# prip-lab/MSU-LatentAFIS

Measured on AMD Instinct MI355X. Metric: latent queries/sec vs 100k rolled gallery, higher is better.
Workload: dtype f32

## Files before the change

### msu-latentafis_amd/csrc/afis_api.cpp

```cpp
#include "afis_ctx.h"
#include <algorithm>
#include <vector>

using namespace afis;

namespace afis {
thread_local std::string g_create_error;
}

extern "C" {

int afis_create(afis_ctx** out, const float* codewords, int M, int K, int dsub, int device_id)
{
    if (!out || !codewords) return fail(nullptr, AFIS_EINVAL, "afis_create: null argument");
    *out = nullptr;
    if (M != kM || K != kK || dsub != kDsub) return fail(nullptr, AFIS_EINVAL, "afis_create: only the M=16, K=256, dsub=6 codebook geometry is supported");
    int n_dev = 0;
    if (hipGetDeviceCount(&n_dev) != hipSuccess || n_dev <= 0) return fail(nullptr, AFIS_EDEVICE, "afis_create: no HIP device (this library has no CPU fallback)");
    if (device_id < 0 || device_id >= n_dev) return fail(nullptr, AFIS_EINVAL, "afis_create: device_id out of range");
    hipDeviceProp_t prop;
    if (hipGetDeviceProperties(&prop, device_id) != hipSuccess) return fail(nullptr, AFIS_EDEVICE, "afis_create: hipGetDeviceProperties failed");
    if (strncmp(prop.gcnArchName, "gfx950", 6) != 0)
        return fail(nullptr, AFIS_EDEVICE, std::string("afis_create: kernels are built for gfx950 only, device is ") + prop.gcnArchName);
    afis_ctx* c = new afis_ctx();
    c->device = device_id;
    c->n_cus = prop.multiProcessorCount;
#define CRCHK(call) do { hipError_t e_ = (call); if (e_ != hipSuccess) { g_create_error = std::string(#call) + ": " + hipGetErrorString(e_); afis_destroy(c); return AFIS_EDEVICE; } } while (0)
    CRCHK(hipSetDevice(device_id));
    if (const char* cm = getenv("AFIS_CU_MASK")) {
        std::vector<uint32_t> words;
        for (const char* p = cm; *p;) { words.push_back((uint32_t)strtoul(p, nullptr, 16)); const char* q = strchr(p, ','); if (!q) break; p = q + 1; }
        CRCHK(hipExtStreamCreateWithCUMask(&c->stream, (uint32_t)words.size(), words.data()));
    } else
    CRCHK(hipStreamCreateWithFlags(&c->stream, hipStreamNonBlocking));
    std::vector<float> cw(codewords, codewords + (size_t)M * K * dsub);
    CRCHK(upload(c->codewords, cw, c->stream));
    std::vector<float> table((size_t)kDistN * kDistN);
    for (int i = 0; i < kDistN; ++i)
        for (int j = i; j < kDistN; ++j) {
            table[i * kDistN + j] = (float)sqrt((i * 16.0) * (i * 16.0) + (j * 16.0) * (j * 16.0));
            table[j * kDistN + i] = table[i * kDistN + j];
        }
    CRCHK(upload(c->table, table, c->stream));
    CRCHK(hipStreamSynchronize(c->stream));
#undef CRCHK
    *out = c;
    register_context(c);
    {
        if (const char* r = getenv("AFIS_OVERLAP_CELL_RATIO")) c->overlap_cell_ratio = atof(r);
        if (const char* r = getenv("AFIS_SEARCH_TIMEOUT_S")) c->search_timeout_s = atof(r);
        const char* e = getenv("AFIS_BOUND_CUS");
        const int64_t n = e ? atoll(e) : (c->n_cus == 256 ? 128 : 0);
        if (afis_set_option(c, "bound_cus", n) != AFIS_OK) { c->bound_cus = 0; c->err.clear(); }
    }
    return AFIS_OK;
}

int afis_device_info(int device_id, char* name, size_t name_cap, char* pci_bus_id, size_t pci_cap, char* uuid_hex, size_t uuid_cap, int* n_cus)
{
    int n_dev = 0;
    if (hipGetDeviceCount(&n_dev) != hipSuccess || device_id < 0 || device_id >= n_dev) return AFIS_EINVAL;
    hipDeviceProp_t prop;
    if (hipGetDeviceProperties(&prop, device_id) != hipSuccess) return AFIS_EDEVICE;
    if (name && name_cap) snprintf(name, name_cap, "%s (%s)", prop.name, prop.gcnArchName);
    if (pci_bus_id && pci_cap) { if (hipDeviceGetPCIBusId(pci_bus_id, (int)pci_cap, device_id) != hipSuccess) pci_bus_id[0] = 0; }
    if (uuid_hex && uuid_cap) {
        uuid_hex[0] = 0;
        hipUUID u;
        if (uuid_cap >= 33 && hipDeviceGetUuid(&u, device_id) == hipSuccess)
            for (int i = 0; i < 16; ++i) snprintf(uuid_hex + 2 * i, 3, "%02x", (unsigned)(unsigned char)u.bytes[i]);
    }
    if (n_cus) *n_cus = prop.multiProcessorCount;
    return AFIS_OK;
}

int afis_create_from_codebook(afis_ctx** out, const void* bytes, size_t len, int device_id)
{
    HostCodebook cb;
    if (!bytes || !parse_codebook(bytes, len, cb)) return fail(nullptr, AFIS_EFORMAT, "codebook is empty!");
    return afis_create(out, cb.words.data(), cb.M, cb.K, cb.dsub, device_id);
}

void afis_destroy(afis_ctx* c)
{
    if (!c) return;
    unregister_context(c);
    (void)hipSetDevice(c->device);
    static const bool trace = getenv("AFIS_DESTROY_TRACE") != nullptr;
    auto lap = [&](const char* what) { if (trace) { fprintf(stderr, "afis_destroy: %s\n", what); fflush(stderr); } };
    lap("waiting for the side streams");
    for (hipStream_t* ps : {&c->stream_lo, &c->stream_hi}) if (*ps) (void)hipStreamSynchronize(*ps);
    lap("waiting for the context's stream");
    if (c->stream) (void)hipStreamSynchronize(c->stream);
    lap("destroying the side streams");
    for (hipStream_t* ps : {&c->stream_lo, &c->stream_hi}) if (*ps) { (void)hipStreamDestroy(*ps); *ps = nullptr; }
    lap("freeing device memory");
    for (afis_queries* q : c->parked_queries) { for (QueryGroup& g : q->groups) g.release(); delete q; }
    c->parked_queries.clear();
    if (c->h_pin) { (void)hipHostFree(c->h_pin); c->h_pin = nullptr; c->h_pin_bytes = 0; }
    free_gallery_dev(c);
    c->codewords.release(); c->table.release(); c->lut.release(); c->rm_val.release(); c->rm_arg.release(); c->rm_cv.release(); c->rm_n.release();
    c->parts.release(); c->scores.release(); c->scratch.release(); c->cands.release(); c->cand_n.release(); c->minu_fb.release(); c->diag.release(); c->topk_idx.release(); c->topk_score.release(); c->lutq.release(); c->lutq_min.release(); c->lutq_rng.release(); c->lutq_rowc.release(); c->lut32.release();
    c->mf_cw16.release(); c->mf_cwn.release(); c->mf_bfrag.release(); c->mf_rowk.release(); c->mf_rec.release(); c->mf_stats.release();
    lap("destroying events and the context's stream");
    for (auto& e : c->evpool) if (e) (void)hipEventDestroy(e);
    if (c->stream) (void)hipStreamDestroy(c->stream);
    lap("joining the staging thread");
    if (c->staging_reaper.joinable()) c->staging_reaper.join();
    lap("done");
    delete c;
}

const char* afis_last_error(const afis_ctx* ctx) { return ctx ? ctx->err.c_str() : g_create_error.c_str(); }

int afis_get_timing(const afis_ctx* ctx, afis_timing* out)
{
    return afis_get_timing2(ctx, out, offsetof(afis_timing, pairs) + sizeof(int64_t));
}

int afis_get_timing2(const afis_ctx* ctx, afis_timing* out, size_t struct_size)
{
    if (!ctx || !out || struct_size < sizeof(float)) return AFIS_EINVAL;
    memcpy(out, &ctx->timing, std::min(struct_size, sizeof(afis_timing)));
    return AFIS_OK;
}

int afis_rank_list(const float* scores, int64_t n, int ref_order, int k, int64_t* idx, float* sc)
{
    if (n < 0 || k < 0 || (n > 0 && !scores) || (k > 0 && !idx)) return fail(nullptr, AFIS_EINVAL, "afis_rank_list: null argument or negative size");
    if (n > 0x7fffffff) return fail(nullptr, AFIS_EINVAL, "afis_rank_list: more than 2^31 - 1 scores");
    std::vector<int> ind((size_t)n);
    for (int64_t i = 0; i < n; ++i) ind[(size_t)i] = (int)i;
    auto by_score = [scores](const int& a, const int& b) { return scores[a] > scores[b]; };
    if (ref_order) std::sort(ind.begin(), ind.end(), by_score);
    else std::stable_sort(ind.begin(), ind.end(), by_score);
    for (int j = 0; j < k; ++j) {
        const bool in = j < n;
        idx[j] = in ? ind[(size_t)j] : -1;
        if (sc) sc[j] = in ? scores[ind[(size_t)j]] : 0.0f;
    }
    return AFIS_OK;
}


int afis_get_option(const afis_ctx* ctx, const char* name, int64_t* value)
{
    if (!ctx || !name || !value) return AFIS_EINVAL;
    const std::string n(name);
    if (n == "adc_variant") *value = ctx->adc_variant;
    else if (n == "bound_cus") *value = (ctx->stream_lo && !ctx->overlap_failed) ? ctx->bound_cus : 0;
    else if (n == "search_timeout_s") *value = ctx->search_timeout_s <= 0 ? 0 : (int64_t)std::ceil(ctx->search_timeout_s);
    else if (n == "search_timeout_ms") *value = ctx->search_timeout_s <= 0 ? 0 : (int64_t)std::llround(ctx->search_timeout_s * 1e3);
    else if (n == "mf_blocks") *value = 2;
    else if (n == "query_batch") *value = ctx->query_batch;
    else if (n == "chunk") *value = ctx->chunk;
    else if (n == "tile_share") *value = ctx->tile_share;
    else if (n == "minu_generic") *value = ctx->minu_generic;
    else if (n == "s3_tie_order") *value = ctx->s3_tie_order;
    else if (n == "ref_tie_order") *value = ctx->s3_tie_order + ctx->s89_tie_order;
    else if (n == "minu_fast_max_latent") *value = rt_class_max_latent(4);
    else if (n == "minu_fast_max_rolled") *value = rt_class_max_rolled(4);
    else if (n == "minu_fast_max_cells") *value = rt_class_simi_floats(4);
    else if (n == "mf_stats") *value = ctx->mf_collect_stats;
    else if (n == "rowmax_budget_mb") *value = ctx->rowmax_budget_bytes >> 20;
    else if (n == "lut_dtype") *value = 32;
    else return AFIS_EINVAL;
    return AFIS_OK;
}

int afis_set_option(afis_ctx* ctx, const char* name, int64_t value)
{
    if (!ctx || !name) return AFIS_EINVAL;
    const std::string n(name);
    if (n == "adc_variant") {
        if (value < 0 || value > 9 || value == 4 || value == 5 || (value < 8 && !g_direct_adc_stage))
            return fail(ctx, AFIS_EINVAL, "adc_variant must be 9 (matrix-core bound pass + exact values) or 8 (16-bit LDS-table bound pass + exact values); the direct kernels 0..3, 6, 7 "
                                          "are reference kernels built into libafis_hip_test.so only");
        ctx->adc_variant = (int)value;
    }
    else if (n == "lut_dtype") { if (value != 32) return fail(ctx, AFIS_EINVAL, "lut_dtype: only 32 (exact) exists; the 16-bit tolerance path of rounds 1-2 missed its stated tolerance and was removed (the reduced-precision pass of BASELINE.json configs[4] is adc_variant 9 / 8: a bound, followed by exact values)"); }
    else if (n == "tile_share") { if (value < 0 || value > 32) return fail(ctx, AFIS_EINVAL, "tile_share must be 0 (auto) or 1..32"); ctx->tile_share = (int)value; }
    else if (n == "query_batch") { if (value < 0 || value > 256) return fail(ctx, AFIS_EINVAL, "query_batch must be 0 (auto) or 1..256"); ctx->query_batch = (int)value; }
    else if (n == "chunk") { if (value < 0 || value > 65536) return fail(ctx, AFIS_EINVAL, "chunk must be 0 (auto) or 1..65536"); ctx->chunk = (int)value; }
    else if (n == "minu_generic") { ctx->minu_generic = value ? 1 : 0; }
    else if (n == "s3_tie_order") { if (value != 0 && value != 1) return fail(ctx, AFIS_EINVAL, "s3_tie_order must be 0 (equal candidate norms by ascending element index) or 1 (in the order libstdc++'s std::sort leaves them)"); ctx->s3_tie_order = (int)value; ctx->s89_tie_order = 0; }
    else if (n == "ref_tie_order") { if (value < 0 || value > 2) return fail(ctx, AFIS_EINVAL, "ref_tie_order must be 0 (equal sort keys by ascending index), 1 (candidate norms in the order libstdc++'s std::sort leaves them: = s3_tie_order 1) or 2 (the scores of the greedy selections of S8 and S9 as well)"); ctx->s3_tie_order = value >= 1; ctx->s89_tie_order = value >= 2; }
    else if (n == "mf_stats") { ctx->mf_collect_stats = value ? 1 : 0; }
    else if (n == "search_timeout_s") { ctx->search_timeout_s = (double)value; }
    else if (n == "search_timeout_ms") { ctx->search_timeout_s = (double)value * 1e-3; }
    else if (n == "bound_cus") {
        if (value < 0 || value > 224 || (value & 31)) return fail(ctx, AFIS_EINVAL, "bound_cus must be 0 (off), 32, 64, ... 224 (the runtime honours CU masks in steps of 32 CUs: 4 per XCD)");
        if (value > 0 && value + 32 > ctx->n_cus) return fail(ctx, AFIS_EINVAL, "bound_cus must leave at least 32 of the device's CUs to the other stream");
        if (hipSetDevice(ctx->device) != hipSuccess) return fail(ctx, AFIS_EDEVICE, "bound_cus: hipSetDevice failed");
        { const int rcd = drain_abandoned(ctx); if (rcd != AFIS_OK) return rcd; }
        for (hipStream_t* ps : {&ctx->stream_lo, &ctx->stream_hi}) if (*ps) { (void)hipStreamSynchronize(*ps); (void)hipStreamDestroy(*ps); *ps = nullptr; }
        ctx->bound_cus = (int)value;
        ctx->overlap_failed = false;
        if (value > 0) {
            uint32_t lo[8] = {0, 0, 0, 0, 0, 0, 0, 0}, hi[8] = {0, 0, 0, 0, 0, 0, 0, 0};
            for (int b = 0; b < std::min(256, ctx->n_cus); ++b) (b < (int)value ? lo : hi)[b >> 5] |= 1u << (b & 31);
            hipError_t e = hipExtStreamCreateWithCUMask(&ctx->stream_lo, 8, lo);
            if (e == hipSuccess) e = hipExtStreamCreateWithCUMask(&ctx->stream_hi, 8, hi);
            if (e != hipSuccess) {
                for (hipStream_t* ps : {&ctx->stream_lo, &ctx->stream_hi}) if (*ps) { (void)hipStreamDestroy(*ps); *ps = nullptr; }
                ctx->bound_cus = 0;
                return fail(ctx, AFIS_EDEVICE, std::string("bound_cus: hipExtStreamCreateWithCUMask: ") + hipGetErrorString(e));
            }
        }
    }
    else if (n == "mf_blocks") { if (value != 2) return fail(ctx, AFIS_EINVAL, "mf_blocks must be 2 (row blocks per wave of the bound pass; the three-row-block form measured 2 % slower in the default schedule and was removed)"); }
    else if (n == "rowmax_budget_mb") { if (value < 1) return fail(ctx, AFIS_EINVAL, "rowmax_budget_mb must be positive"); ctx->rowmax_budget_bytes = value << 20; }
    else return fail(ctx, AFIS_EINVAL, "unknown option: " + n);
    return AFIS_OK;
}

}
```

### msu-latentafis_amd/csrc/afis_ctx.h

```cpp
#pragma once
#include "../../include/afis_matcher.h"

#include <algorithm>
#include <atomic>
#include <cmath>
#include <cstddef>
#include <cstdio>
#include <cstdlib>
#include <cstring>
#include <mutex>
#include <new>
#include <numeric>
#include <string>
#include <thread>
#include <chrono>
#include <vector>
#include <sys/mman.h>

#include "afis_device.h"
#include "template_io.h"
#include <memory>

namespace afis {

struct DevBuf {
    void* p = nullptr; size_t bytes = 0;
    hipError_t ensure(size_t n)
    {
        if (n <= bytes) return hipSuccess;
        static const bool trace = getenv("AFIS_ALLOC_TRACE") != nullptr;
        const auto t0 = std::chrono::steady_clock::now();
        const size_t was = bytes;
        if (p) { hipError_t e = hipFree(p); p = nullptr; bytes = 0; if (e != hipSuccess) return e; }
        const auto t1 = std::chrono::steady_clock::now();
        hipError_t e = hipMalloc(&p, n);
        if (e == hipSuccess) bytes = n;
        if (trace && n >= ((size_t)64 << 20))
            fprintf(stderr, "alloc: %.3f GB (was %.3f): hipFree %.1f ms, hipMalloc %.1f ms\n", n / 1e9, was / 1e9, std::chrono::duration<double, std::milli>(t1 - t0).count(),
                    std::chrono::duration<double, std::milli>(std::chrono::steady_clock::now() - t1).count());
        return e;
    }
    void release() { if (p) (void)hipFree(p); p = nullptr; bytes = 0; }
    template <class T> T* as() const { return (T*)p; }
};

}

using namespace afis;

struct QueryGroup {
    QueryDev dev;
    DevBuf lm_off, lm_xy, lm_ori, lm_des, lm_frag, lm_tile_off, lt_off, lt_xy, lt_ori, lt_des, tile_off, tile16_off, tex_slot, status;
    int nq = 0; int max_nL = 0; int n_lt_rows = 0; int64_t lut_rows_x_tiles = 0;
    int64_t n_lm_points = 0;
    bool overlapped = false;
    std::vector<int32_t> h_lt_n;
    void release() { lm_off.release(); lm_xy.release(); lm_ori.release(); lm_des.release(); lm_frag.release(); lm_tile_off.release(); lt_off.release(); lt_xy.release(); lt_ori.release();
                     lt_des.release(); tile_off.release(); tile16_off.release(); tex_slot.release(); status.release(); }
};

struct afis_queries {
    std::vector<QueryGroup> groups;
    std::vector<int32_t> status;
    int n_q = 0;
};

struct afis_ctx {
    int device = 0;
    hipStream_t stream = nullptr;
    hipStream_t stream_hi = nullptr;
    hipStream_t stream_lo = nullptr;
    int bound_cus = 0;
    int n_cus = 0;
    std::vector<hipEvent_t> evpool;
    std::string err;
    DevBuf codewords, table;
    HostGallery hg;
    std::unique_ptr<GalleryMapping> pend;
    int64_t pend_first = 0, pend_count = 0;
    std::thread staging_reaper;
    bool committed = false;
    int64_t index_base = 0;
    GalleryDev gal;
    DevBuf g_minu_off, g_minu_xy, g_minu_ori, g_minu_des, g_minu_frag, g_minu_tile_off, g_tex_off, g_tex_xy, g_tex_ori, g_tex_codes, g_tex_codes_cf, g_tex_cf_blk, g_tex_codes_q, g_tex_q_blk, g_tex_t32_blk, g_empty, g_task_ctr;
    bool codes_cf_built = false;
    bool codes_q_built = false;
    int64_t q_blocks = 0;
    int64_t t32_tiles = 0;
    int max_nR = 0;
    int64_t total_tex_points = 0;
    int64_t total_minutiae = 0;
    DevBuf mf_cw16, mf_cwn, g_codes_p, g_nrm_p, g_tile_meta, mf_bfrag, mf_rowk, mf_rec, mf_stats;
    bool mf_cb_built = false, mf_gal_built = false;
    int mf_collect_stats = 0;
    DevBuf lutq, lutq_min, lutq_rng, lutq_rowc, lut32;
    DevBuf lut, rm_val, rm_arg, rm_cv, rm_n, parts, scores, scratch, cands, cand_n, minu_fb, topk_idx, topk_score;
    DevBuf diag;
    std::vector<unsigned long long> h_diag;
    void* h_pin = nullptr; size_t h_pin_bytes = 0;
    std::vector<float> h_scores, h_parts;
    int adc_variant = 9;
    int tile_share = 0;
    int query_batch = 0;
    int chunk = 0;
    int minu_generic = 0;
    int s3_tie_order = 0;
    int s89_tie_order = 0;
    double search_timeout_s = 600.0;
    int64_t planned_group_bytes = 0;
    std::vector<afis_queries*> parked_queries;
    bool search_abandoned = false;
    bool overlap_failed = false;
    double overlap_cell_ratio = 0.037;
    int64_t rowmax_budget_bytes = 0;
    afis_timing timing = {};
};

namespace afis {

extern thread_local std::string g_create_error;

inline int fail(afis_ctx* ctx, int code, const std::string& msg)
{
    if (ctx) ctx->err = msg; else g_create_error = msg;
    return code;
}
#define HIPCHK(ctx, call)                                                                                       \
    do { hipError_t e_ = (call); if (e_ != hipSuccess)                                                          \
        return fail(ctx, AFIS_EDEVICE, std::string(#call) + ": " + hipGetErrorString(e_) + (e_ == hipErrorOutOfMemory ?                                      \
            " (device memory: a launch group's buffers are sized from the memory that was free when the queries were uploaded - with several contexts or processes on one "  \
            "device lower option rowmax_budget_mb or query_batch)" : "")); } while (0)

template <class T, class A>
inline hipError_t upload(DevBuf& b, const std::vector<T, A>& v, hipStream_t s)
{
    hipError_t e = b.ensure(std::max<size_t>(v.size() * sizeof(T), 16));
    if (e != hipSuccess) return e;
    if (!v.empty()) e = hipMemcpyAsync(b.p, v.data(), v.size() * sizeof(T), hipMemcpyHostToDevice, s);
    return e;
}

template <class F>
void parallel_for(int64_t n, F body)
{
    const int64_t nt = std::min<int64_t>(std::max<int64_t>(1, (int64_t)std::thread::hardware_concurrency()), std::min<int64_t>(16, std::max<int64_t>(1, n / 256)));
    if (nt <= 1) { body((int64_t)0, n); return; }
    std::vector<std::thread> th;
    for (int64_t i = 0; i < nt; ++i) th.emplace_back(body, n * i / nt, n * (i + 1) / nt);
    for (std::thread& t : th) t.join();
}

template <class Off>
std::vector<float> fragment_tiles(const std::vector<float>& des, const std::vector<Off>& off, std::vector<int32_t>& tile_off)
{
    const int64_t T = (int64_t)off.size() - 1;
    tile_off.assign((size_t)T + 1, 0);
    for (int64_t t = 0; t < T; ++t) tile_off[(size_t)t + 1] = tile_off[(size_t)t] + (int32_t)((off[(size_t)t + 1] - off[(size_t)t] + 15) / 16);
    std::vector<float> out((size_t)tile_off[(size_t)T] * 6 * 64 * 4, 0.0f);
    parallel_for(T, [&](int64_t lo, int64_t hi) {
        for (int64_t t = lo; t < hi; ++t) {
            const int64_t r0 = (int64_t)off[(size_t)t], n = (int64_t)off[(size_t)t + 1] - r0;
            for (int64_t row = 0; row < n; ++row) {
                const float* src = &des[(size_t)(r0 + row) * kDes];
                float* tile = &out[(size_t)(tile_off[(size_t)t] + row / 16) * 6 * 64 * 4];
                const int li = (int)(row & 15);
                for (int v = 0; v < 6; ++v)
                    for (int lg = 0; lg < 4; ++lg)
                        for (int c = 0; c < 4; ++c) tile[((size_t)v * 64 + lg * 16 + li) * 4 + c] = src[4 * (4 * v + c) + lg];
            }
        }
    });
    return out;
}

constexpr int64_t kMfRecBytesPerRow = 8;
int materialise(afis_ctx* ctx);
void free_gallery_dev(afis_ctx* c);
int ensure_mf_gallery(afis_ctx* ctx, hipStream_t s);
void views_of(const HostTemplate& t, std::vector<afis_minutiae_view>& mv, std::vector<afis_texture_view>& tv, afis_template_view& out);
int build_group(afis_ctx* ctx, const afis_template_view* qs, int nq, QueryGroup& grp, std::vector<int32_t>& status_out, const int* spec = nullptr);
int adc_stage_q(afis_ctx* ctx, QueryGroup& grp, int chunk, bool exact, hipEvent_t after_lut = nullptr);
int adc_refine_mfma(afis_ctx* ctx, QueryGroup& grp, bool all_rows, bool compact);
int adc_stage_mfma(afis_ctx* ctx, QueryGroup& grp, bool all_rows, hipEvent_t after_lut = nullptr, hipEvent_t after_bound = nullptr, bool compact = false, hipStream_t sb = nullptr,
                   bool refine_now = true, unsigned long long* diag = nullptr);
typedef int (*DirectAdcStage)(afis_ctx* ctx, const QueryDev& d, int chunk, hipEvent_t after_lut);
extern DirectAdcStage g_direct_adc_stage __attribute__((visibility("hidden")));
int wait_streams(afis_ctx* ctx, std::initializer_list<hipStream_t> streams, const char* what);
void register_context(afis_ctx* ctx); void unregister_context(afis_ctx* ctx);
int drain_abandoned(afis_ctx* ctx);

}
```

### msu-latentafis_amd/csrc/afis_device.h

```cpp
#pragma once
#include <hip/hip_runtime.h>
#include <stdint.h>

namespace afis {

constexpr int kM = 16;
constexpr int kK = 256;
constexpr int kDsub = 6;
constexpr int kDes = 96;
constexpr int kTexMax = 1000;
constexpr int kTopTex = 200;
constexpr int kTopMinu = 120;
constexpr int kDistN = 50;
constexpr int kTileRows = 8;
constexpr int kTileFloats = kTileRows * kM * kK;

struct GalleryDev {
    int32_t G = 0;
    const int32_t* minu_off = nullptr;
    const short2*  minu_xy = nullptr;
    const float*   minu_ori = nullptr;
    const float*   minu_des = nullptr;
    const float4*  minu_frag = nullptr;
    const int32_t* minu_tile_off = nullptr;
    const int32_t* tex_off = nullptr;
    const short2*  tex_xy = nullptr;
    const float*   tex_ori = nullptr;
    const uint4*   tex_codes = nullptr;
    const uint4*   tex_codes_cf = nullptr;
    const int32_t* tex_cf_blk = nullptr;
    const uint8_t* empty = nullptr;
    int32_t* task_ctr = nullptr;
};

struct QueryDev {
    int32_t nq = 0;
    const int32_t* lm_off = nullptr;
    const short2*  lm_xy = nullptr;
    const float*   lm_ori = nullptr;
    const float*   lm_des = nullptr;
    const float4*  lm_frag = nullptr;
    const int32_t* lm_tile_off = nullptr;
    const int32_t* lt_off = nullptr;
    const short2*  lt_xy = nullptr;
    const float*   lt_ori = nullptr;
    const float*   lt_des = nullptr;
    const int32_t* tile_off = nullptr;
    const int32_t* tile16_off = nullptr;
    int32_t n_tiles16 = 0;
    const int32_t* tex_slot = nullptr;
    const int32_t* status = nullptr;
    int32_t n_tiles = 0;
    int32_t lt_pad = 0;
};

#ifdef __HIPCC__
__device__ __forceinline__ float sqrt_rn_pos(float x)
{
    float r = __builtin_amdgcn_sqrtf(x);
    const float dn = __int_as_float(__float_as_int(r) - 1), up = __int_as_float(__float_as_int(r) + 1);
    const float e_dn = __builtin_fmaf(-dn, r, x), e_up = __builtin_fmaf(-up, r, x);
    r = e_dn <= 0.0f ? dn : r;
    r = e_up > 0.0f ? up : r;
    return r;
}
#endif

#ifdef __HIPCC__
__device__ __forceinline__ float lut_entry(const float* __restrict__ des6, const float* __restrict__ cw6)
{
    float dist = 0.0f;
#pragma unroll
    for (int d = 0; d < kDsub; ++d) {
        float t = des6[d] - cw6[d];
        float t2 = t * t;
        dist += t2;
    }
    return dist;
}
#endif

hipError_t launch_lut_build(const QueryDev& q, const float* codewords, float* lut_tiles, int variant, hipStream_t stream);
hipError_t launch_adc_rowmax(const QueryDev& q, const GalleryDev& g, const float* lut_tiles, int chunk, int variant,
                             float* rm_val, int32_t* rm_arg, hipStream_t stream);
hipError_t launch_codes_cf(const GalleryDev& g, void* out, hipStream_t stream);
hipError_t launch_lutq_build(const QueryDev& q, int n_rows_total, const float* codewords, float* row_min, float* row_rng, void* tiles, void* rowc, hipStream_t stream);
hipError_t launch_codes_q(const GalleryDev& g, const int32_t* q_blk, void* out, hipStream_t stream);
hipError_t launch_adc_rowmax_q(const QueryDev& q, const GalleryDev& g, const void* codes_q, const int32_t* q_blk, const void* lutq_tiles, const void* rowc,
                               const float* lut32, int chunk, int share, float* rm_val, int32_t* rm_arg, hipStream_t stream);
hipError_t launch_mf_codebook(const float* codewords, void* cw16, float* cwn, hipStream_t stream);
hipError_t launch_mf_tiles(const GalleryDev& g, const int32_t* t32_blk, const float* cwn, void* codes_p, float* nrm_p, void* tile_meta, hipStream_t stream);
hipError_t launch_mf_rows(const float* lt_des, int n_rows, int n_rb, const float* codewords, const float* cwn, void* bfrag, void* rowk, hipStream_t stream);
hipError_t launch_adc_mfma(const GalleryDev& g, const void* codes_p, const float* nrm_p, const void* tile_meta, const int32_t* tile0, const void* cw16,
                           const void* bfrag, const void* rowk, int n_rows, int n_rb, int R_pad, int chunk, void* rec,
                           unsigned long long* diag , hipStream_t stream);
hipError_t launch_tex_refine(const QueryDev& q, const GalleryDev& g, const float* codewords, const void* rec, const void* rowk, int R_pad, int all_rows,
                             float* rm_val, int32_t* rm_arg, unsigned long long* stats, float* rm_cv, int32_t* rm_n, hipStream_t stream);
struct MinuCand { float sim; short li, ri; };

#ifdef __HIPCC__
#define AFIS_HOST_DEVICE __host__ __device__
#else
#define AFIS_HOST_DEVICE
#endif
AFIS_HOST_DEVICE constexpr int rt_class_max_rolled(int S) { return S == 1 ? 128 : S == 2 ? 256 : 512; }
AFIS_HOST_DEVICE constexpr int rt_class_max_latent(int S) { return S == 1 ? 64 : 256; }
AFIS_HOST_DEVICE constexpr int rt_class_simi_floats(int S) { return S == 1 ? 8192 : S == 2 ? 8192 * 2 + 256 : 38912; }
AFIS_HOST_DEVICE constexpr int rt_class_keys_per_thread(int S) { return S == 4 ? 64 : 32; }
AFIS_HOST_DEVICE inline int rt_row_stride(int S, int nR) { return S == 1 ? (((nR & 1) || nR == 128) ? nR : nR + 1) : (nR | 1); }
AFIS_HOST_DEVICE inline int rt_max_rows(int S, int nR)
{
    if (nR <= 0 || nR > rt_class_max_rolled(S)) return 0;
    int m = rt_class_keys_per_thread(S) * ((256 * S) / nR);
    const int cap = rt_class_simi_floats(S) / rt_row_stride(S, nR);
    m = m < cap ? m : cap;
    return m < rt_class_max_latent(S) ? m : rt_class_max_latent(S);
}
inline long long launch_group_latents(long long G) { if (G < 1) G = 1; const long long w = (5000000 + G / 2) / G; return w < 10 ? 10 : w > 128 ? 128 : w; }
inline void launch_group_cuts(const long long* rows_prefix, int n, int per, bool by_row_groups, int* cuts , int* n_cuts)
{
    *n_cuts = 0;
    if (n <= 0) return;
    if (per < 1) per = 1;
    if (!by_row_groups || n == 1) { for (int i = per; i < n; i += per) cuts[(*n_cuts)++] = i; cuts[(*n_cuts)++] = n; return; }
    const long long kInf = 1ll << 60, rg_rows = 768;
    long long* best = new long long[(size_t)n + 1]; int* from = new int[(size_t)n + 1]; int* cnt = new int[(size_t)n + 1];
    best[0] = 0; from[0] = 0; cnt[0] = 0;
    for (int i = 1; i <= n; ++i) {
        best[i] = kInf; from[i] = 0; cnt[i] = 0;
        for (int j = (i - per > 0 ? i - per : 0); j < i; ++j) {
            const long long c = best[j] + (rows_prefix[i] - rows_prefix[j] + rg_rows - 1) / rg_rows;
            if (c < best[i] || (c == best[i] && cnt[j] + 1 < cnt[i])) { best[i] = c; from[i] = j; cnt[i] = cnt[j] + 1; }
        }
    }
    int m = 0;
    for (int i = n; i > 0; i = from[i]) cuts[m++] = i;
    for (int a = 0, b = m - 1; a < b; ++a, --b) { const int t = cuts[a]; cuts[a] = cuts[b]; cuts[b] = t; }
    *n_cuts = m;
    delete[] best; delete[] from; delete[] cnt;
}
inline size_t minu_fb_ints(size_t n_tasks, size_t G) { return 1 + n_tasks + 8 + 3 * G; }
inline size_t minu_scratch_floats(int max_nL, int max_nR, int s3_tie_order)
{
    const size_t n = ((size_t)(max_nL > 1 ? max_nL : 1) * (size_t)(max_nR > 1 ? max_nR : 1) + 63) / 64 * 64;
    return (s3_tie_order ? 5 : 2) * n + 4096;
}
enum { kDiagFallback = 0,
       kDiagSmall = 1,
       kDiagCandsClk = 4, kDiagCandsWall = 5,
       kDiagBoundClk = 6, kDiagBoundWall = 7,
       kDiagWords = 16 };
hipError_t launch_graph_texture(const QueryDev& q, const GalleryDev& g, const float* table_dist,
                                const float* rm_val, const int32_t* rm_arg, const float* rm_cv, const int32_t* rm_n, float* parts, MinuCand* tap_out, int32_t* tap_n, int tap_stage, hipStream_t stream);
hipError_t launch_minu_cands(const QueryDev& q, const GalleryDev& g, float* scratch, size_t scratch_floats_per_wg, int n_wg,
                             int force_generic, MinuCand* cands, int32_t* cand_n, int32_t* fallback , int max_nL, int max_nR,
                             unsigned long long* diag , hipStream_t stream);
hipError_t launch_graph_minutiae(const QueryDev& q, const GalleryDev& g, const MinuCand* cands, const int32_t* cand_n,
                                 float* parts, short4* corr_out, int32_t* corr_n, MinuCand* tap_out, int32_t* tap_n, int tap_stage, hipStream_t stream, bool join = false);
hipError_t launch_fuse(const QueryDev& q, const GalleryDev& g, const float* parts, float* scores, hipStream_t stream);

hipError_t launch_topk(const float* scores, int n_q, int G, int k, long long index_base, long long* out_idx, float* out_score, hipStream_t stream);

hipError_t launch_pq_encode(const float* des, long long n, const float* codewords, uint8_t* codes, hipStream_t stream);
hipError_t launch_fragment_tiles(const float* des, const int32_t* off, const int32_t* tile_off, int n_templates, void* frag, hipStream_t stream);
hipError_t read_phase_cycles(unsigned long long* out32, bool reset);
hipError_t read_graph_phase_cycles(unsigned long long* out16, bool reset);

hipError_t launch_debug_atan2_grid(int R, float* out, hipStream_t stream);
hipError_t launch_debug_graph_arith(unsigned long long* cnt8, hipStream_t stream);
hipError_t launch_lut_reference_layout(const float* des, int n, const float* codewords, float* out, hipStream_t stream);

}
```

### msu-latentafis_amd/csrc/afis_search.cpp

```cpp
#include "afis_ctx.h"

using namespace afis;

namespace afis {

int64_t group_bytes_per_query(const afis_ctx* ctx, int64_t G)
{
    const int64_t per_pair = (int64_t)kTexMax * 8 + (ctx->adc_variant == 9 ? (int64_t)kTexMax * kMfRecBytesPerRow : 0) + 3 * (int64_t)kTopMinu * (int64_t)sizeof(MinuCand) + 3 * 4 + 16 + 8;
    return std::max<int64_t>(1, G) * per_pair;
}
int64_t group_bytes_actual(const afis_ctx* ctx, int64_t G, int64_t nq, int64_t rows_total, int64_t lt_max)
{
    const int64_t lt_pad = std::max<int64_t>(kTileRows, (lt_max + kTileRows - 1) / kTileRows * kTileRows), R_pad = (rows_total + 31) / 32 * 32;
    const int64_t per_pair = lt_pad * 8 + 3 * (int64_t)kTopMinu * (int64_t)sizeof(MinuCand) + 3 * 4 + 16 + 8;
    return std::max<int64_t>(1, G) * (nq * per_pair + (ctx->adc_variant == 9 ? R_pad * kMfRecBytesPerRow : 0));
}

namespace { std::mutex g_ctx_mutex; std::vector<afis_ctx*> g_ctx_live; }
static size_t held_group_bytes(const afis_ctx* c)
{
    return c->rm_val.bytes + c->rm_arg.bytes + c->rm_cv.bytes + c->rm_n.bytes + c->mf_rec.bytes + c->cands.bytes + c->cand_n.bytes + c->parts.bytes + c->minu_fb.bytes;
}
void register_context(afis_ctx* c) { std::lock_guard<std::mutex> lk(g_ctx_mutex); g_ctx_live.push_back(c); }
void unregister_context(afis_ctx* c) { std::lock_guard<std::mutex> lk(g_ctx_mutex); g_ctx_live.erase(std::remove(g_ctx_live.begin(), g_ctx_live.end(), c), g_ctx_live.end()); }

int64_t group_budget_bytes(const afis_ctx* ctx)
{
    if (ctx->rowmax_budget_bytes > 0) return ctx->rowmax_budget_bytes;
    size_t free_b = 0, total_b = 0;
    if (hipMemGetInfo(&free_b, &total_b) != hipSuccess) return 36ll << 30;
    int64_t pending_elsewhere = 0;
    {
        std::lock_guard<std::mutex> lk(g_ctx_mutex);
        for (const afis_ctx* c : g_ctx_live)
            if (c != ctx && c->device == ctx->device) pending_elsewhere += std::max<int64_t>(0, c->planned_group_bytes - (int64_t)held_group_bytes(c));
    }
    const int64_t avail = (int64_t)free_b + (int64_t)held_group_bytes(ctx) - pending_elsewhere;
    return std::max<int64_t>(1ll << 30, (int64_t)((double)std::max<int64_t>(0, avail) * 0.6));
}

int wait_streams(afis_ctx* ctx, std::initializer_list<hipStream_t> streams, const char* what)
{
    if (ctx->search_timeout_s <= 0) {
        for (hipStream_t st : streams) if (st) HIPCHK(ctx, hipStreamSynchronize(st));
        return AFIS_OK;
    }
    const auto t0 = std::chrono::steady_clock::now();
    for (long spins = 0;; ++spins) {
        bool all = true;
        for (hipStream_t st : streams) {
            if (!st) continue;
            const hipError_t e = hipStreamQuery(st);
            if (e == hipErrorNotReady) all = false;
            else if (e != hipSuccess) return fail(ctx, AFIS_EDEVICE, std::string(what) + ": hipStreamQuery: " + hipGetErrorString(e));
        }
        if (all) return AFIS_OK;
        if (std::chrono::duration<double>(std::chrono::steady_clock::now() - t0).count() > ctx->search_timeout_s) {
            if (streams.size() > 1) ctx->overlap_failed = true;
            ctx->search_abandoned = true;
            char msg[256];
            snprintf(msg, sizeof msg, "%s: the device did not finish within %.3g s (AFIS_SEARCH_TIMEOUT_S)%s", what, ctx->search_timeout_s,
                     streams.size() > 1 ? "; the overlapped schedule is switched off for this context (bound_cus 0)" : "");
            return fail(ctx, AFIS_EDEVICE, msg);
        }
        if (spins < 20000) std::this_thread::yield(); else std::this_thread::sleep_for(std::chrono::microseconds(50));
    }
}

int drain_abandoned(afis_ctx* ctx)
{
    if (!ctx->search_abandoned) return AFIS_OK;
    ctx->search_abandoned = false;
    const int rc = wait_streams(ctx, {ctx->stream_lo, ctx->stream_hi, ctx->stream}, "waiting for the search that timed out");
    if (rc != AFIS_OK) return rc;
    for (afis_queries* q : ctx->parked_queries) { for (QueryGroup& g : q->groups) g.release(); delete q; }
    ctx->parked_queries.clear();
    return AFIS_OK;
}

struct SideStreamGuard {
    afis_ctx* ctx; hipStream_t a = nullptr, b = nullptr; bool armed = false;
    explicit SideStreamGuard(afis_ctx* c) : ctx(c) {}
    void arm(hipStream_t x, hipStream_t y) { a = x; b = y; armed = true; }
    void disarm() { armed = false; }
    ~SideStreamGuard()
    {
        if (!armed) return;
        const std::string keep = ctx->err;
        const double full = ctx->search_timeout_s;
        if (full > 0) ctx->search_timeout_s = std::min(full, 10.0);
        const int rc = wait_streams(ctx, {a, b}, "draining the side streams after a failed launch group");
        ctx->search_timeout_s = full;
        ctx->err = rc == AFIS_OK ? keep : keep + " [and the side streams did not drain within 10 s: " + ctx->err + "]";
    }
};

}

namespace afis {

static const int kSelected[3] = {27 - 1, 3 - 1, 12 - 1};

int build_group(afis_ctx* ctx, const afis_template_view* qs, int nq, QueryGroup& grp, std::vector<int32_t>& status_out, const int* spec)
{
    std::vector<int32_t> lm_off{0}, lt_off{0}, tile_off{0}, tile16_off{0}, tex_slot, status;
    std::vector<short2> lm_xy, lt_xy; std::vector<float> lm_ori, lm_des, lt_ori, lt_des;
    int max_nL = 0, lt_max = 0;
    for (int i = 0; i < nq; ++i) {
        const afis_template_view& t = qs[i];
        if (t.n_minu < 0 || t.n_tex < 0 || (t.n_minu > 0 && !t.minu) || (t.n_tex > 0 && !t.tex)) return fail(ctx, AFIS_EINVAL, "latent template: bad view");
        const int* sel = spec ? spec + (size_t)i * 4 : kSelected;
        const int tex_ind = spec ? spec[(size_t)i * 4 + 3] : 0;
        const bool latent_empty = !spec && (t.n_minu <= sel[0] && t.n_tex <= 0);
        status.push_back(latent_empty ? AFIS_QUERY_LATENT_EMPTY : AFIS_QUERY_OK);
        for (int s = 0; s < 3; ++s) {
            if (!latent_empty && sel[s] >= 0 && t.n_minu > sel[s]) {
                const afis_minutiae_view& m = t.minu[sel[s]];
                if (m.n <= 0 || m.n > 2000 || !m.x || !m.y || !m.ori || !m.des) return fail(ctx, AFIS_EINVAL, "latent minutiae template: bad view (n must be 1..2000)");
                if (m.des_len != kDes) return fail(ctx, AFIS_EINVAL, "latent minutiae template: des_len must be 96 (the reference asserts equal descriptor lengths, matcher.cpp:433)");
                for (int k = 0; k < m.n; ++k) lm_xy.push_back(make_short2(m.x[k], m.y[k]));
                lm_ori.insert(lm_ori.end(), m.ori, m.ori + m.n);
                lm_des.insert(lm_des.end(), m.des, m.des + (size_t)m.n * kDes);
                max_nL = std::max(max_nL, m.n);
            }
            lm_off.push_back((int32_t)lm_xy.size());
        }
        int n_lt = 0;
        if (!latent_empty && tex_ind >= 0 && t.n_tex > tex_ind) {
            const afis_texture_view& x = t.tex[tex_ind];
            if (x.n <= 0 || x.n > 2000 || !x.x || !x.y || !x.ori || !x.des) return fail(ctx, AFIS_EINVAL, "latent texture template: bad view (n must be 1..2000, des required)");
            if (x.des_len != kDes) return fail(ctx, AFIS_EINVAL, "latent texture template: des_len must be 96");
            n_lt = std::min(x.n, kTexMax);
            for (int k = 0; k < n_lt; ++k) lt_xy.push_back(make_short2(x.x[k], x.y[k]));
            lt_ori.insert(lt_ori.end(), x.ori, x.ori + n_lt);
            lt_des.insert(lt_des.end(), x.des, x.des + (size_t)n_lt * kDes);
        }
        lt_off.push_back((int32_t)lt_xy.size());
        tile_off.push_back(tile_off.back() + (n_lt + kTileRows - 1) / kTileRows);
        tile16_off.push_back(tile16_off.back() + (n_lt + 15) / 16);
        tex_slot.push_back(tex_ind >= 0 && t.n_tex > tex_ind ? t.n_minu : -1);
        lt_max = std::max(lt_max, n_lt);
        grp.h_lt_n.push_back(n_lt);
    }
    hipStream_t s = ctx->stream;
    HIPCHK(ctx, upload(grp.lm_off, lm_off, s)); HIPCHK(ctx, upload(grp.lm_xy, lm_xy, s)); HIPCHK(ctx, upload(grp.lm_ori, lm_ori, s));
    HIPCHK(ctx, upload(grp.lm_des, lm_des, s)); HIPCHK(ctx, upload(grp.lt_off, lt_off, s));
    std::vector<int32_t> lm_tile_off;
    const std::vector<float> lm_frag = fragment_tiles(lm_des, lm_off, lm_tile_off);
    HIPCHK(ctx, upload(grp.lm_frag, lm_frag, s)); HIPCHK(ctx, upload(grp.lm_tile_off, lm_tile_off, s)); HIPCHK(ctx, upload(grp.lt_xy, lt_xy, s));
    HIPCHK(ctx, upload(grp.lt_ori, lt_ori, s)); HIPCHK(ctx, upload(grp.lt_des, lt_des, s)); HIPCHK(ctx, upload(grp.tile_off, tile_off, s)); HIPCHK(ctx, upload(grp.tile16_off, tile16_off, s));
    HIPCHK(ctx, upload(grp.tex_slot, tex_slot, s)); HIPCHK(ctx, upload(grp.status, status, s));
    HIPCHK(ctx, hipStreamSynchronize(s));
    QueryDev& d = grp.dev;
    d.nq = nq;
    d.lm_off = grp.lm_off.as<int32_t>(); d.lm_xy = grp.lm_xy.as<short2>(); d.lm_ori = grp.lm_ori.as<float>(); d.lm_des = grp.lm_des.as<float>(); d.lm_frag = grp.lm_frag.as<float4>(); d.lm_tile_off = grp.lm_tile_off.as<int32_t>();
    d.lt_off = grp.lt_off.as<int32_t>(); d.lt_xy = grp.lt_xy.as<short2>(); d.lt_ori = grp.lt_ori.as<float>(); d.lt_des = grp.lt_des.as<float>();
    d.tile_off = grp.tile_off.as<int32_t>(); d.tex_slot = grp.tex_slot.as<int32_t>(); d.status = grp.status.as<int32_t>();
    d.n_tiles = tile_off.back();
    d.tile16_off = grp.tile16_off.as<int32_t>(); d.n_tiles16 = tile16_off.back(); grp.n_lt_rows = lt_off.back();
    d.lt_pad = std::max(kTileRows, (lt_max + kTileRows - 1) / kTileRows * kTileRows);
    grp.nq = nq; grp.max_nL = max_nL; grp.n_lm_points = (int64_t)lm_xy.size();
    status_out.insert(status_out.end(), status.begin(), status.end());
    return AFIS_OK;
}

}

extern "C" {

int afis_queries_upload(afis_ctx* ctx, const afis_template_view* queries, int n_q, afis_queries** out)
{
    if (!ctx || !out || n_q < 0 || (n_q > 0 && !queries)) return fail(ctx, AFIS_EINVAL, "afis_queries_upload: bad argument");
    if (!ctx->committed) return fail(ctx, AFIS_ESTATE, "afis_queries_upload: commit the gallery first");
    HIPCHK(ctx, hipSetDevice(ctx->device));
    { const int rcd = drain_abandoned(ctx); if (rcd != AFIS_OK) return rcd; }
    const int64_t G = std::max<int64_t>(1, ctx->gal.G);
    const int64_t by_mem = group_budget_bytes(ctx) / group_bytes_per_query(ctx, G);
    const int64_t want = ctx->query_batch > 0 ? ctx->query_batch : launch_group_latents(G);
    int per = (int)std::max<int64_t>(1, std::min<int64_t>(want, by_mem));
    afis_queries* q = new afis_queries();
    q->n_q = n_q;
    const int64_t budget = group_budget_bytes(ctx);
    std::vector<long long> rows((size_t)n_q + 1, 0);
    for (int i = 0; i < n_q; ++i) {
        const afis_template_view& t = queries[i];
        const bool has = t.n_tex > 0 && t.tex && !(t.n_minu <= kSelected[0] && t.n_tex <= 0);
        rows[(size_t)i + 1] = rows[(size_t)i] + (has ? std::min(std::max(t.tex[0].n, 0), kTexMax) : 0);
    }
    std::vector<int> cuts((size_t)std::max(n_q, 1));
    int n_cuts = 0;
    auto largest_group_bytes = [&](int n) {
        int64_t worst = 0; int a0 = 0;
        for (int c = 0; c < n; ++c) {
            int64_t lt_max = 0;
            for (int i = a0; i < cuts[(size_t)c]; ++i) lt_max = std::max<int64_t>(lt_max, rows[(size_t)i + 1] - rows[(size_t)i]);
            worst = std::max(worst, group_bytes_actual(ctx, G, cuts[(size_t)c] - a0, rows[(size_t)cuts[(size_t)c]] - rows[(size_t)a0], lt_max));
            a0 = cuts[(size_t)c];
        }
        return worst;
    };
    for (int try_per = (int)std::max<int64_t>(per, std::min<int64_t>(want, std::max(n_q, 1)));; --try_per) {
        launch_group_cuts(rows.data(), n_q, try_per, ctx->adc_variant == 9, cuts.data(), &n_cuts);
        if (try_per <= per || largest_group_bytes(n_cuts) <= budget) { per = try_per; break; }
    }
    ctx->planned_group_bytes = std::max(ctx->planned_group_bytes, largest_group_bytes(n_cuts));
    cuts.resize((size_t)n_cuts);
    int g0 = 0;
    for (int end : cuts) {
        q->groups.emplace_back();
        int rc = build_group(ctx, queries + g0, end - g0, q->groups.back(), q->status);
        if (rc != AFIS_OK) { afis_queries_free(ctx, q); return rc; }
        g0 = end;
    }
    *out = q;
    return AFIS_OK;
}

void afis_queries_free(afis_ctx* ctx, afis_queries* q)
{
    if (!q) return;
    if (ctx) (void)hipSetDevice(ctx->device);
    if (ctx && ctx->search_abandoned) { ctx->parked_queries.push_back(q); return; }
    for (QueryGroup& g : q->groups) g.release();
    delete q;
}

}

namespace afis {

DirectAdcStage g_direct_adc_stage = nullptr;

static int tile_share_of(const afis_ctx* ctx) { return ctx->tile_share > 0 ? ctx->tile_share : 4; }

int adc_stage_q(afis_ctx* ctx, QueryGroup& grp, int chunk, bool exact, hipEvent_t after_lut)
{
    const QueryDev& d = grp.dev;
    hipStream_t s = ctx->stream;
    if (d.n_tiles16 <= 0 || ctx->gal.G <= 0) { if (after_lut) HIPCHK(ctx, hipEventRecord(after_lut, s)); return AFIS_OK; }
    if (!ctx->codes_q_built) {
        HIPCHK(ctx, ctx->g_tex_codes_q.ensure(std::max<size_t>((size_t)ctx->q_blocks * 64 * 16, 16)));
        HIPCHK(ctx, launch_codes_q(ctx->gal, ctx->g_tex_q_blk.as<int32_t>(), ctx->g_tex_codes_q.p, s));
        ctx->codes_q_built = true;
    }
    HIPCHK(ctx, ctx->lutq.ensure((size_t)d.n_tiles16 * 131072));
    HIPCHK(ctx, ctx->lutq_min.ensure(std::max<size_t>((size_t)grp.n_lt_rows * kM * 4, 16)));
    HIPCHK(ctx, ctx->lutq_rng.ensure(std::max<size_t>((size_t)grp.n_lt_rows * kM * 4, 16)));
    HIPCHK(ctx, ctx->lutq_rowc.ensure(std::max<size_t>((size_t)grp.n_lt_rows * 16, 16)));
    HIPCHK(ctx, launch_lutq_build(d, grp.n_lt_rows, ctx->codewords.as<float>(), ctx->lutq_min.as<float>(), ctx->lutq_rng.as<float>(), ctx->lutq.p, ctx->lutq_rowc.p, s));
    if (exact) {
        HIPCHK(ctx, ctx->lut32.ensure((size_t)grp.n_lt_rows * kM * kK * 4));
        HIPCHK(ctx, launch_lut_reference_layout(d.lt_des, grp.n_lt_rows, ctx->codewords.as<float>(), ctx->lut32.as<float>(), s));
    }
    if (after_lut) HIPCHK(ctx, hipEventRecord(after_lut, s));
    HIPCHK(ctx, launch_adc_rowmax_q(d, ctx->gal, ctx->g_tex_codes_q.p, ctx->g_tex_q_blk.as<int32_t>(), ctx->lutq.p, ctx->lutq_rowc.p,
                                    exact ? ctx->lut32.as<float>() : nullptr, chunk, tile_share_of(ctx), ctx->rm_val.as<float>(), ctx->rm_arg.as<int32_t>(), s));
    return AFIS_OK;
}

int ensure_mf_gallery(afis_ctx* ctx, hipStream_t s)
{
    const GalleryDev& g = ctx->gal;
    if (!ctx->mf_cb_built) {
        HIPCHK(ctx, ctx->mf_cw16.ensure((size_t)kM * kK * 16));
        HIPCHK(ctx, ctx->mf_cwn.ensure((size_t)kM * kK * 4));
        HIPCHK(ctx, launch_mf_codebook(ctx->codewords.as<float>(), ctx->mf_cw16.p, ctx->mf_cwn.as<float>(), s));
        ctx->mf_cb_built = true;
    }
    if (!ctx->mf_gal_built && g.G > 0) {
        const size_t n_ent = std::max<size_t>((size_t)ctx->t32_tiles * 32, 1);
        HIPCHK(ctx, ctx->g_codes_p.ensure(n_ent * 16));
        HIPCHK(ctx, ctx->g_nrm_p.ensure(n_ent * 4));
        HIPCHK(ctx, ctx->g_tile_meta.ensure(std::max<size_t>((size_t)ctx->t32_tiles * 8, 16)));
        HIPCHK(ctx, launch_mf_tiles(g, ctx->g_tex_t32_blk.as<int32_t>(), ctx->mf_cwn.as<float>(), ctx->g_codes_p.p, ctx->g_nrm_p.as<float>(), ctx->g_tile_meta.p, s));
        ctx->mf_gal_built = true;
    }
    return AFIS_OK;
}

int adc_stage_mfma(afis_ctx* ctx, QueryGroup& grp, bool all_rows, hipEvent_t after_lut, hipEvent_t after_bound, bool compact, hipStream_t sb, bool refine_now, unsigned long long* diag)
{
    const QueryDev& d = grp.dev;
    hipStream_t s = sb ? sb : ctx->stream;
    const GalleryDev& g = ctx->gal;
    if (grp.n_lt_rows <= 0 || g.G <= 0) { if (after_lut) HIPCHK(ctx, hipEventRecord(after_lut, s)); if (after_bound) HIPCHK(ctx, hipEventRecord(after_bound, s)); return AFIS_OK; }
    { int rcg = ensure_mf_gallery(ctx, s); if (rcg != AFIS_OK) return rcg; }
    const int n_rows = grp.n_lt_rows, n_rb = (n_rows + 31) / 32, R_pad = n_rb * 32;
    const size_t R_cap = (size_t)R_pad;
    HIPCHK(ctx, ctx->mf_bfrag.ensure(R_cap / 32 * 6 * 64 * 16));
    HIPCHK(ctx, ctx->mf_rowk.ensure(R_cap * 16));
    HIPCHK(ctx, ctx->mf_rec.ensure((size_t)g.G * R_cap * kMfRecBytesPerRow));
    if (ctx->mf_collect_stats && !ctx->mf_stats.p) { HIPCHK(ctx, ctx->mf_stats.ensure(64)); HIPCHK(ctx, hipMemsetAsync(ctx->mf_stats.p, 0, 64, s)); }
    HIPCHK(ctx, launch_mf_rows(d.lt_des, n_rows, n_rb, ctx->codewords.as<float>(), ctx->mf_cwn.as<float>(), ctx->mf_bfrag.p, ctx->mf_rowk.p, s));
    if (after_lut) HIPCHK(ctx, hipEventRecord(after_lut, s));
    const int wg_rb = 24;
    const int n_rg = (n_rb + wg_rb - 1) / wg_rb;
    const long long want_chunks = (std::max<long long>(1, (256 * 24) / n_rg) + 7) / 8 * 8;
    const int chunk = ctx->chunk > 0 ? ctx->chunk : (int)std::max<long long>(8, ((long long)g.G + want_chunks - 1) / want_chunks);
    HIPCHK(ctx, launch_adc_mfma(g, ctx->g_codes_p.p, ctx->g_nrm_p.as<float>(), ctx->g_tile_meta.p, ctx->g_tex_t32_blk.as<int32_t>(), ctx->mf_cw16.p,
                                ctx->mf_bfrag.p, ctx->mf_rowk.p, n_rows, n_rb, R_pad, chunk, ctx->mf_rec.p, diag, s));
    if (after_bound) HIPCHK(ctx, hipEventRecord(after_bound, s));
    return refine_now ? adc_refine_mfma(ctx, grp, all_rows, compact) : AFIS_OK;
}

int adc_refine_mfma(afis_ctx* ctx, QueryGroup& grp, bool all_rows, bool compact)
{
    if (grp.n_lt_rows <= 0 || ctx->gal.G <= 0) return AFIS_OK;
    const int R_pad = (grp.n_lt_rows + 31) / 32 * 32;
    HIPCHK(ctx, launch_tex_refine(grp.dev, ctx->gal, ctx->codewords.as<float>(), ctx->mf_rec.p, ctx->mf_rowk.p, R_pad, all_rows ? 1 : 0, ctx->rm_val.as<float>(),
                                  ctx->rm_arg.as<int32_t>(), ctx->mf_collect_stats ? ctx->mf_stats.as<unsigned long long>() : nullptr,
                                  compact ? ctx->rm_cv.as<float>() : nullptr, compact ? ctx->rm_n.as<int32_t>() : nullptr, ctx->stream));
    return AFIS_OK;
}

static const int kDeviceTopK = 64;

static int prepare_search_buffers(afis_ctx* ctx, const afis_queries* q, bool want_parts)
{
    const int64_t G = ctx->gal.G;
    const int nq_all = q->n_q;
    float* const parts = want_parts ? reinterpret_cast<float*>(1) : nullptr;
    if (G > 0) {
        int nq_max = 0, nL_max = 1; size_t rows_pad_max = 32, pair_rows_max = 0;
        for (const QueryGroup& grp : q->groups) {
            nq_max = std::max(nq_max, grp.nq); nL_max = std::max(nL_max, grp.max_nL);
            rows_pad_max = std::max(rows_pad_max, ((size_t)std::max(grp.n_lt_rows, 0) + 31) / 32 * 32);
            pair_rows_max = std::max(pair_rows_max, (size_t)grp.nq * (size_t)grp.dev.lt_pad);
        }
        const size_t n_pairs = (size_t)nq_max * G;
        if (n_pairs > 0) {
            const size_t rm_bytes = std::max<size_t>(pair_rows_max * (size_t)G * 4, 16);
            if (ctx->adc_variant != 9) HIPCHK(ctx, ctx->rm_val.ensure(rm_bytes));
            HIPCHK(ctx, ctx->rm_arg.ensure(rm_bytes));
            HIPCHK(ctx, ctx->parts.ensure(parts ? (size_t)nq_all * G * 16 : n_pairs * 16));
            HIPCHK(ctx, ctx->cands.ensure(n_pairs * 3 * kTopMinu * sizeof(MinuCand)));
            HIPCHK(ctx, ctx->cand_n.ensure(n_pairs * 3 * 4));
            HIPCHK(ctx, ctx->minu_fb.ensure(minu_fb_ints(n_pairs * 3, (size_t)G) * 4));
            {
                const size_t per_wg = minu_scratch_floats(nL_max, ctx->max_nR, ctx->s3_tie_order);
                int n_wg = 1024;
                while (n_wg > 64 && per_wg * 4 * n_wg > (8ull << 30)) n_wg /= 2;
                HIPCHK(ctx, ctx->scratch.ensure(per_wg * 4 * n_wg));
            }
            if (ctx->adc_variant == 9) {
                HIPCHK(ctx, ctx->rm_cv.ensure(rm_bytes)); HIPCHK(ctx, ctx->rm_n.ensure(n_pairs * 4));
                const size_t R_cap = rows_pad_max;
                HIPCHK(ctx, ctx->mf_bfrag.ensure(R_cap / 32 * 6 * 64 * 16));
                HIPCHK(ctx, ctx->mf_rowk.ensure(R_cap * 16));
                HIPCHK(ctx, ctx->mf_rec.ensure((size_t)G * R_cap * kMfRecBytesPerRow));
                if (!ctx->mf_gal_built) {
                    const size_t n_ent = std::max<size_t>((size_t)ctx->t32_tiles * 32, 1);
                    HIPCHK(ctx, ctx->g_codes_p.ensure(n_ent * 16));
                    HIPCHK(ctx, ctx->g_nrm_p.ensure(n_ent * 4));
                    HIPCHK(ctx, ctx->g_tile_meta.ensure(std::max<size_t>((size_t)ctx->t32_tiles * 8, 16)));
                }
            }
        }
    }
    return AFIS_OK;
}

static int collect_timing(afis_ctx* ctx, const afis_queries* q, afis_timing& tm, bool dev_topk, hipEvent_t* evk)
{
    const int64_t G = ctx->gal.G;
    const size_t n_groups = q->groups.size();
    {
        unsigned long long acc[kDiagWords] = {};
        for (size_t i = 0; i < n_groups; ++i) for (int w = 0; w < kDiagWords; ++w) acc[w] += ctx->h_diag[i * kDiagWords + w];
        tm.minu_fallback_tasks = (int64_t)acc[kDiagFallback];
        tm.minu_tasks_small = (int64_t)acc[kDiagSmall]; tm.minu_tasks_medium = (int64_t)acc[kDiagSmall + 1]; tm.minu_tasks_large = (int64_t)acc[kDiagSmall + 2];
        tm.minu_tasks = tm.minu_tasks_small + tm.minu_tasks_medium + tm.minu_tasks_large + tm.minu_fallback_tasks;
        tm.cands_clock_ghz = acc[kDiagCandsWall] ? (float)((double)acc[kDiagCandsClk] / (double)acc[kDiagCandsWall] * 0.1) : 0.0f;
        tm.bound_clock_ghz = acc[kDiagBoundWall] ? (float)((double)acc[kDiagBoundClk] / (double)acc[kDiagBoundWall] * 0.1) : 0.0f;
    }
    if (G > 0) {
        for (size_t i = 0; i < n_groups; ++i) {
            hipEvent_t* ev = &ctx->evpool[i * 10];
            float tot = 0;
            auto el = [&](int a, int b, float& out) -> int { out = 0; HIPCHK(ctx, hipEventElapsedTime(&out, ev[a], ev[b])); return AFIS_OK; };
            const bool ov = q->groups[i].overlapped;
            float t_lut = 0, t_adc = 0, t_tex = 0, t_minu = 0, t_fuse = 0, t_bound = 0, t_ref = 0, t_c = 0, t_g = 0;
            if (el(0, 5, tot)) return AFIS_EDEVICE;
            if (ov) {
                if (el(0, 1, t_lut) || el(1, 6, t_bound) || el(8, 2, t_ref) || el(2, 3, t_tex) || el(0, 7, t_c) || el(7, 4, t_g) || el(9, 5, t_fuse)) return AFIS_EDEVICE;
                t_adc = t_bound + t_ref; t_minu = t_c + t_g;
            } else {
                if (el(0, 1, t_lut) || el(1, 2, t_adc) || el(2, 3, t_tex) || el(3, 4, t_minu) || el(9, 5, t_fuse) || el(3, 7, t_c) || el(7, 4, t_g)) return AFIS_EDEVICE;
                if (ctx->adc_variant == 9 && q->groups[i].n_lt_rows > 0) { if (el(1, 6, t_bound) || el(6, 2, t_ref)) return AFIS_EDEVICE; }
                else t_bound = t_adc;
            }
            tm.adc_bound_ms += t_bound; tm.adc_refine_ms += t_ref; tm.cands_ms += t_c; tm.minu_graph_ms += t_g;
            tm.lut_ms += t_lut; tm.adc_ms += t_adc; tm.tex_tail_ms += t_tex; tm.minu_ms += t_minu; tm.fuse_ms += t_fuse; tm.total_ms += tot;
        }
        if (dev_topk) { float t = 0; HIPCHK(ctx, hipEventElapsedTime(&t, evk[0], evk[1])); tm.topk_ms = t; tm.total_ms += t; }
    }
    return AFIS_OK;
}

}

extern "C" {

int afis_search_resident(afis_ctx* ctx, afis_queries* q, float* scores, float* parts, int32_t* status,
                         int k, int64_t* topk_idx, float* topk_score)
{
    if (!ctx || !q) return fail(ctx, AFIS_EINVAL, "afis_search_resident: null argument");
    if (!ctx->committed) return fail(ctx, AFIS_ESTATE, "afis_search: commit the gallery first");
    if (k < 0 || (k > 0 && (!topk_idx || !topk_score))) return fail(ctx, AFIS_EINVAL, "afis_search: k > 0 needs topk_idx and topk_score");
    HIPCHK(ctx, hipSetDevice(ctx->device));
    { const int rcd = drain_abandoned(ctx); if (rcd != AFIS_OK) return rcd; }
    const GalleryDev& g = ctx->gal;
    const int64_t G = g.G;
    const int nq_all = q->n_q;
    afis_timing tm = {};
    if (status) for (int i = 0; i < nq_all; ++i) status[i] = q->status[i];
    hipStream_t s = ctx->stream;
    const size_t n_groups = q->groups.size();
    while (ctx->evpool.size() < n_groups * 10 + 2) { hipEvent_t e; HIPCHK(ctx, hipEventCreate(&e)); ctx->evpool.push_back(e); }
    if (G > 0 && nq_all > 0) HIPCHK(ctx, ctx->scores.ensure((size_t)nq_all * G * 4));
    HIPCHK(ctx, ctx->diag.ensure(std::max<size_t>(n_groups, 1) * kDiagWords * 8));
    HIPCHK(ctx, hipMemsetAsync(ctx->diag.p, 0, std::max<size_t>(n_groups, 1) * kDiagWords * 8, s));
    { const int rcp = prepare_search_buffers(ctx, q, parts != nullptr); if (rcp != AFIS_OK) return rcp; }
    static const bool alloc_trace = getenv("AFIS_ALLOC_TRACE") != nullptr;
    if (alloc_trace) { fprintf(stderr, "queue: the search starts queuing\n"); fflush(stderr); }
    int q0 = 0;
    size_t gi = 0;
    SideStreamGuard side_guard(ctx);
    bool any_overlap = false;
    for (QueryGroup& grp : q->groups) {
        const QueryDev& d = grp.dev;
        const int nq = grp.nq;
        hipEvent_t* ev = &ctx->evpool[gi * 10];
        unsigned long long* const diag_row = ctx->diag.as<unsigned long long>() + gi * kDiagWords;
        if (G > 0) {
            const size_t n_pairs = (size_t)nq * G;
            const size_t lt_cap = (size_t)d.lt_pad;
            if (ctx->adc_variant != 9) HIPCHK(ctx, ctx->rm_val.ensure(std::max<size_t>(n_pairs * lt_cap * 4, 16)));
            HIPCHK(ctx, ctx->rm_arg.ensure(std::max<size_t>(n_pairs * lt_cap * 4, 16)));
            if (ctx->adc_variant == 9) { HIPCHK(ctx, ctx->rm_cv.ensure(std::max<size_t>(n_pairs * lt_cap * 4, 16))); HIPCHK(ctx, ctx->rm_n.ensure(std::max<size_t>(n_pairs * 4, 16))); }
            HIPCHK(ctx, ctx->parts.ensure(parts ? (size_t)nq_all * G * 16 : n_pairs * 16));
            size_t per_wg = minu_scratch_floats(grp.max_nL, ctx->max_nR, ctx->s3_tie_order);
            int n_wg = 1024;
            while (n_wg > 64 && per_wg * 4 * n_wg > (8ull << 30)) n_wg /= 2;
            HIPCHK(ctx, ctx->scratch.ensure(per_wg * 4 * n_wg));
            HIPCHK(ctx, ctx->cands.ensure(n_pairs * 3 * kTopMinu * sizeof(MinuCand)));
            HIPCHK(ctx, ctx->cand_n.ensure(n_pairs * 3 * 4));
            HIPCHK(ctx, ctx->minu_fb.ensure(minu_fb_ints(n_pairs * 3, (size_t)G) * 4));
            float* grp_scores = ctx->scores.as<float>() + (size_t)q0 * G;
            float* const grp_parts = ctx->parts.as<float>() + (parts ? (size_t)q0 * G * 4 : 0);
            const long long cmul = 8ll * (ctx->adc_variant == 8 ? tile_share_of(ctx) : 1);
            const long long n_chunks_auto = ((G + 639) / 640 + cmul - 1) / cmul * cmul;
            const int chunk = ctx->chunk > 0 ? ctx->chunk : (int)((G + n_chunks_auto - 1) / n_chunks_auto);
            HIPCHK(ctx, hipEventRecord(ev[0], s));
            const double cells_m = (double)grp.n_lm_points * (double)ctx->total_minutiae, cells_t = (double)grp.n_lt_rows * (double)ctx->total_tex_points;
            const bool minutiae_light = cells_m <= ctx->overlap_cell_ratio * cells_t;
            const bool overlap = ctx->adc_variant == 9 && ctx->stream_lo != nullptr && !ctx->overlap_failed && n_pairs >= 65536 && minutiae_light;
            grp.overlapped = overlap;
            const bool compact9 = ctx->adc_variant == 9;
            auto minutiae_stage = [&]() -> int {
                HIPCHK(ctx, launch_minu_cands(d, g, ctx->scratch.as<float>(), per_wg, n_wg, ctx->minu_generic | (ctx->s3_tie_order << 1), ctx->cands.as<MinuCand>(), ctx->cand_n.as<int32_t>(), ctx->minu_fb.as<int32_t>(), grp.max_nL, ctx->max_nR, diag_row, s));
                HIPCHK(ctx, hipEventRecord(ev[7], s));
                HIPCHK(ctx, launch_graph_minutiae(d, g, ctx->cands.as<MinuCand>(), ctx->cand_n.as<int32_t>(), grp_parts, nullptr, nullptr, nullptr, nullptr, 2 | (ctx->s89_tie_order << 8), s));
                return AFIS_OK;
            };
            if (overlap) {
                hipStream_t sl = ctx->stream_lo, sh = ctx->stream_hi;
                side_guard.arm(sl, sh);
                HIPCHK(ctx, hipStreamWaitEvent(sl, ev[0], 0));
                HIPCHK(ctx, hipStreamWaitEvent(sh, ev[0], 0));
                int rc9 = adc_stage_mfma(ctx, grp, false, ev[1], ev[6], true, sl, false, diag_row);
                if (rc9 != AFIS_OK) return rc9;
                HIPCHK(ctx, launch_minu_cands(d, g, ctx->scratch.as<float>(), per_wg, n_wg, ctx->minu_generic | (ctx->s3_tie_order << 1), ctx->cands.as<MinuCand>(), ctx->cand_n.as<int32_t>(), ctx->minu_fb.as<int32_t>(), grp.max_nL, ctx->max_nR, diag_row, sh));
                HIPCHK(ctx, hipMemsetAsync(g.task_ctr + 1, 0, 4, sh));
                HIPCHK(ctx, hipEventRecord(ev[7], sh));
                HIPCHK(ctx, launch_graph_minutiae(d, g, ctx->cands.as<MinuCand>(), ctx->cand_n.as<int32_t>(), grp_parts, nullptr, nullptr, nullptr, nullptr, 2 | (ctx->s89_tie_order << 8), sh, true));
                HIPCHK(ctx, hipEventRecord(ev[4], sh));
                HIPCHK(ctx, hipStreamWaitEvent(s, ev[6], 0));
                HIPCHK(ctx, hipEventRecord(ev[8], s));
                rc9 = adc_refine_mfma(ctx, grp, false, true);
                if (rc9 != AFIS_OK) return rc9;
                HIPCHK(ctx, hipEventRecord(ev[2], s));
                HIPCHK(ctx, launch_graph_texture(d, g, ctx->table.as<float>(), ctx->rm_val.as<float>(), ctx->rm_arg.as<int32_t>(), ctx->rm_cv.as<float>(), ctx->rm_n.as<int32_t>(), grp_parts, nullptr, nullptr, 2 | (ctx->s89_tie_order << 8), s));
                HIPCHK(ctx, hipEventRecord(ev[3], s));
                HIPCHK(ctx, hipStreamWaitEvent(s, ev[7], 0));
                HIPCHK(ctx, launch_graph_minutiae(d, g, ctx->cands.as<MinuCand>(), ctx->cand_n.as<int32_t>(), grp_parts, nullptr, nullptr, nullptr, nullptr, 2 | (ctx->s89_tie_order << 8), s, true));
                HIPCHK(ctx, hipStreamWaitEvent(s, ev[4], 0));
                any_overlap = true;
            } else {
            if (ctx->adc_variant == 9) {
                int rc9 = adc_stage_mfma(ctx, grp, false, ev[1], ev[6], true, nullptr, true, diag_row);
                if (rc9 != AFIS_OK) return rc9;
            } else if (ctx->adc_variant == 8) {
                int rc16 = adc_stage_q(ctx, grp, chunk, true, ev[1]);
                if (rc16 != AFIS_OK) return rc16;
            } else {
                int rcd = g_direct_adc_stage(ctx, d, chunk, ev[1]);
                if (rcd != AFIS_OK) return rcd;
            }
            HIPCHK(ctx, hipEventRecord(ev[2], s));
            HIPCHK(ctx, launch_graph_texture(d, g, ctx->table.as<float>(), ctx->rm_val.as<float>(), ctx->rm_arg.as<int32_t>(), compact9 ? ctx->rm_cv.as<float>() : nullptr,
                                             compact9 ? ctx->rm_n.as<int32_t>() : nullptr, grp_parts, nullptr, nullptr, 2 | (ctx->s89_tie_order << 8), s));
            HIPCHK(ctx, hipEventRecord(ev[3], s));
            { int rcm = minutiae_stage(); if (rcm != AFIS_OK) return rcm; }
            HIPCHK(ctx, hipEventRecord(ev[4], s));
            }
            HIPCHK(ctx, hipEventRecord(ev[9], s));
            HIPCHK(ctx, launch_fuse(d, g, grp_parts, grp_scores, s));
            HIPCHK(ctx, hipEventRecord(ev[5], s));
            if (d.n_tiles > 0) {
                tm.adc_launches += 1;
                const int tile_rows = ctx->adc_variant == 8 ? 16 : kTileRows;
                int64_t rows = 0; for (int n : grp.h_lt_n) rows += (n + tile_rows - 1) / tile_rows * tile_rows;
                tm.adc_lookups += rows * ctx->total_tex_points * kM;
            }
            tm.pairs += (int64_t)n_pairs;
        }
        q0 += nq; ++gi;
    }
    const bool dev_topk = k > 0 && k <= kDeviceTopK && G > 0 && nq_all > 0;
    hipEvent_t* evk = &ctx->evpool[n_groups * 10];
    if (dev_topk) {
        HIPCHK(ctx, ctx->topk_idx.ensure((size_t)nq_all * k * 8));
        HIPCHK(ctx, ctx->topk_score.ensure((size_t)nq_all * k * 4));
        HIPCHK(ctx, hipEventRecord(evk[0], s));
        HIPCHK(ctx, launch_topk(ctx->scores.as<float>(), nq_all, (int)G, k, (long long)ctx->index_base, ctx->topk_idx.as<long long>(), ctx->topk_score.as<float>(), s));
        HIPCHK(ctx, hipEventRecord(evk[1], s));
    }
    const size_t pin_topk = dev_topk ? (size_t)nq_all * k * 12 : 0, pin_diag = std::max<size_t>(n_groups, 1) * kDiagWords * 8;
    if (ctx->h_pin_bytes < pin_topk + pin_diag) {
        if (ctx->h_pin) (void)hipHostFree(ctx->h_pin);
        ctx->h_pin = nullptr; ctx->h_pin_bytes = 0;
        HIPCHK(ctx, hipHostMalloc(&ctx->h_pin, pin_topk + pin_diag, hipHostMallocDefault));
        ctx->h_pin_bytes = pin_topk + pin_diag;
    }
    uint8_t* const pin = (uint8_t*)ctx->h_pin;
    if (dev_topk) {
        HIPCHK(ctx, hipMemcpyAsync(pin, ctx->topk_idx.p, (size_t)nq_all * k * 8, hipMemcpyDeviceToHost, s));
        HIPCHK(ctx, hipMemcpyAsync(pin + (size_t)nq_all * k * 8, ctx->topk_score.p, (size_t)nq_all * k * 4, hipMemcpyDeviceToHost, s));
    }
    HIPCHK(ctx, hipMemcpyAsync(pin + pin_topk, ctx->diag.p, pin_diag, hipMemcpyDeviceToHost, s));
    {
        const int rcw = any_overlap ? wait_streams(ctx, {ctx->stream_lo, ctx->stream_hi, s}, "afis_search") : wait_streams(ctx, {s}, "afis_search");
        side_guard.disarm();
        if (rcw != AFIS_OK) return rcw;
    }
    if (dev_topk) { memcpy(topk_idx, pin, (size_t)nq_all * k * 8); memcpy(topk_score, pin + (size_t)nq_all * k * 8, (size_t)nq_all * k * 4); }
    ctx->h_diag.assign(std::max<size_t>(n_groups, 1) * kDiagWords, 0ull);
    memcpy(ctx->h_diag.data(), pin + pin_topk, pin_diag);
    if (parts && G > 0 && nq_all > 0) HIPCHK(ctx, hipMemcpy(parts, ctx->parts.p, (size_t)nq_all * G * 16, hipMemcpyDeviceToHost));
    const bool host_topk = k > 0 && !dev_topk;
    float* h_sc = scores;
    if (G > 0 && nq_all > 0 && (scores || host_topk)) {
        if (!h_sc) { ctx->h_scores.resize((size_t)nq_all * G); h_sc = ctx->h_scores.data(); }
        HIPCHK(ctx, hipMemcpy(h_sc, ctx->scores.p, (size_t)nq_all * G * 4, hipMemcpyDeviceToHost));
    }
    { const int rct = collect_timing(ctx, q, tm, dev_topk, evk); if (rct != AFIS_OK) return rct; }
    if (host_topk) {
        std::vector<int32_t> ind((size_t)G);
        for (int i = 0; i < nq_all; ++i) {
            const float* sc = G > 0 ? h_sc + (size_t)i * G : nullptr;
            std::iota(ind.begin(), ind.end(), 0);
            const int kk = (int)std::min<int64_t>(k, G);
            std::partial_sort(ind.begin(), ind.begin() + kk, ind.end(), [sc](int a, int b) { return sc[a] > sc[b] || (sc[a] == sc[b] && a < b); });
            for (int r = 0; r < k; ++r) {
                const size_t o = (size_t)i * k + r;
                if (r < kk) { topk_idx[o] = ctx->index_base + ind[r]; topk_score[o] = sc[ind[r]]; }
                else { topk_idx[o] = -1; topk_score[o] = -INFINITY; }
            }
        }
    }
    tm.launch_groups = (int32_t)n_groups;
    for (const QueryGroup& grp : q->groups) tm.overlapped_groups += grp.overlapped ? 1 : 0;
    ctx->timing = tm;
    return AFIS_OK;
}

int afis_correspondences(afis_ctx* ctx, const afis_template_view* query, const int64_t* gallery_idx, int n, int32_t* counts, int16_t* xy)
{
    if (!ctx || !query || n < 0 || (n > 0 && (!gallery_idx || !counts || !xy))) return fail(ctx, AFIS_EINVAL, "afis_correspondences: bad argument");
    if (!ctx->committed) return fail(ctx, AFIS_ESTATE, "afis_correspondences: commit the gallery first");
    if (n == 0) return AFIS_OK;
    HIPCHK(ctx, hipSetDevice(ctx->device));
    { const int rcd = drain_abandoned(ctx); if (rcd != AFIS_OK) return rcd; }
    const GalleryDev& g = ctx->gal;
    for (int i = 0; i < n; ++i)
        if (gallery_idx[i] < ctx->index_base || gallery_idx[i] >= ctx->index_base + g.G) return fail(ctx, AFIS_EINVAL, "afis_correspondences: gallery index outside this shard");
    QueryGroup grp;
    std::vector<int32_t> status;
    int rc = build_group(ctx, query, 1, grp, status);
    if (rc != AFIS_OK) { grp.release(); return rc; }
    for (int i = 0; i < n * 3; ++i) counts[i] = -1;
    memset(xy, 0, (size_t)n * 3 * kTopMinu * 4 * sizeof(int16_t));
    DevBuf d_xy, d_n;
    auto body = [&]() -> int {
        if (status[0] != AFIS_QUERY_OK) return AFIS_OK;
        const size_t per_wg = minu_scratch_floats(grp.max_nL, ctx->max_nR, ctx->s3_tie_order);
        const int n_wg = 64;
        HIPCHK(ctx, ctx->scratch.ensure(per_wg * 4 * n_wg));
        HIPCHK(ctx, ctx->cands.ensure((size_t)n * 3 * kTopMinu * sizeof(MinuCand)));
        HIPCHK(ctx, ctx->cand_n.ensure((size_t)n * 3 * 4));
        HIPCHK(ctx, ctx->minu_fb.ensure(minu_fb_ints(3, 1) * 4));
        HIPCHK(ctx, ctx->parts.ensure((size_t)n * 16));
        HIPCHK(ctx, d_xy.ensure((size_t)n * 3 * kTopMinu * sizeof(short4)));
        HIPCHK(ctx, d_n.ensure((size_t)n * 3 * 4));
        hipStream_t s = ctx->stream;
        int err = AFIS_OK;
        for (int i = 0; i < n && err == AFIS_OK; ++i) {
            const int64_t gi = gallery_idx[i] - ctx->index_base;
            GalleryDev one = g;
            one.G = 1; one.minu_off += gi; one.minu_tile_off += gi; one.tex_off += gi; one.empty += gi;
            MinuCand* cands = ctx->cands.as<MinuCand>() + (size_t)i * 3 * kTopMinu;
            int32_t* cand_n = ctx->cand_n.as<int32_t>() + (size_t)i * 3;
            if (launch_minu_cands(grp.dev, one, ctx->scratch.as<float>(), per_wg, n_wg, ctx->minu_generic | (ctx->s3_tie_order << 1), cands, cand_n, ctx->minu_fb.as<int32_t>(), grp.max_nL, ctx->max_nR, nullptr, s) != hipSuccess ||
                launch_graph_minutiae(grp.dev, one, cands, cand_n, ctx->parts.as<float>() + (size_t)i * 4,
                                      d_xy.as<short4>() + (size_t)i * 3 * kTopMinu, d_n.as<int32_t>() + (size_t)i * 3, nullptr, nullptr, 2 | (ctx->s89_tie_order << 8), s) != hipSuccess)
                err = fail(ctx, AFIS_EDEVICE, "afis_correspondences: kernel launch failed");
        }
        if (err == AFIS_OK) {
            if (hipMemcpyAsync(xy, d_xy.p, (size_t)n * 3 * kTopMinu * sizeof(short4), hipMemcpyDeviceToHost, s) != hipSuccess ||
                hipMemcpyAsync(counts, d_n.p, (size_t)n * 3 * 4, hipMemcpyDeviceToHost, s) != hipSuccess ||
                hipStreamSynchronize(s) != hipSuccess)
                err = fail(ctx, AFIS_EDEVICE, "afis_correspondences: copy back failed");
            for (int i = 0; i < n && err == AFIS_OK; ++i) {
                const int64_t gi = gallery_idx[i] - ctx->index_base;
                int32_t off[2] = {0, 0};
                if (hipMemcpy(off, g.minu_off + gi, sizeof(off), hipMemcpyDeviceToHost) != hipSuccess) { err = fail(ctx, AFIS_EDEVICE, "afis_correspondences: copy back failed"); break; }
                for (int sl = 0; sl < 3; ++sl)
                    if (ctx->hg.empty[(size_t)gi] || off[1] - off[0] <= 0 || query->n_minu <= kSelected[sl]) counts[i * 3 + sl] = -1;
            }
        } else (void)hipStreamSynchronize(s);
        return err;
    };
    rc = body();
    d_xy.release(); d_n.release();
    grp.release();
    return rc;
}

int afis_match_all_templates(afis_ctx* ctx, const afis_template_view* query, float* scores, int32_t* rolled_status, int32_t* query_status)
{
    if (!ctx || !query || !scores) return fail(ctx, AFIS_EINVAL, "afis_match_all_templates: null argument");
    if (!ctx->committed) return fail(ctx, AFIS_ESTATE, "afis_match_all_templates: commit the gallery first");
    const int n_minu = query->n_minu, n_tex = query->n_tex;
    if (n_minu < 0 || n_tex < 0) return fail(ctx, AFIS_EINVAL, "afis_match_all_templates: bad view");
    const int64_t G = ctx->gal.G;
    const int width = n_minu + n_tex;
    if (query_status) *query_status = (n_minu <= 0 && n_tex <= 0) ? AFIS_QUERY_LATENT_EMPTY : AFIS_QUERY_OK;
    if (rolled_status) for (int64_t g = 0; g < G; ++g) rolled_status[g] = ctx->hg.empty[(size_t)g] ? 2 : 0;
    for (size_t i = 0; i < (size_t)G * width; ++i) scores[i] = 0.0f;
    if (width == 0 || G == 0) return AFIS_OK;
    HIPCHK(ctx, hipSetDevice(ctx->device));
    { const int rcd = drain_abandoned(ctx); if (rcd != AFIS_OK) return rcd; }
    const int n_pq = std::max((n_minu + 2) / 3, n_tex);
    const int64_t by_mem = std::max<int64_t>(1, group_budget_bytes(ctx) / group_bytes_per_query(ctx, G));
    const int per = (int)std::max<int64_t>(1, std::min<int64_t>(ctx->query_batch > 0 ? ctx->query_batch : 10, by_mem));
    std::vector<float> parts;
    for (int j0 = 0; j0 < n_pq; j0 += per) {
        const int nq = std::min(per, n_pq - j0);
        std::vector<afis_template_view> views((size_t)nq, *query);
        std::vector<int> spec((size_t)nq * 4);
        for (int j = 0; j < nq; ++j) {
            for (int s = 0; s < 3; ++s) spec[(size_t)j * 4 + s] = 3 * (j0 + j) + s < n_minu ? 3 * (j0 + j) + s : -1;
            spec[(size_t)j * 4 + 3] = j0 + j < n_tex ? j0 + j : -1;
        }
        afis_queries q; q.n_q = nq;
        q.groups.emplace_back();
        int rc = build_group(ctx, views.data(), nq, q.groups.back(), q.status, spec.data());
        if (rc == AFIS_OK) {
            parts.resize((size_t)nq * G * 4);
            rc = afis_search_resident(ctx, &q, nullptr, parts.data(), nullptr, 0, nullptr, nullptr);
        }
        if (ctx->search_abandoned) {
            afis_queries* keep = new afis_queries; keep->groups.swap(q.groups); ctx->parked_queries.push_back(keep);
        } else q.groups.back().release();
        if (rc != AFIS_OK) return rc;
        for (int j = 0; j < nq; ++j)
            for (int64_t g = 0; g < G; ++g) {
                if (ctx->hg.empty[(size_t)g]) continue;
                const float* p = &parts[((size_t)j * G + g) * 4];
                float* o = scores + (size_t)g * width;
                for (int s = 0; s < 3; ++s) if (3 * (j0 + j) + s < n_minu) o[3 * (j0 + j) + s] = p[s];
                if (j0 + j < n_tex) o[n_minu + j0 + j] = p[3];
            }
    }
    return AFIS_OK;
}

int afis_search(afis_ctx* ctx, const afis_template_view* queries, int n_q, float* scores, float* parts, int32_t* status,
                int k, int64_t* topk_idx, float* topk_score)
{
    afis_queries* q = nullptr;
    int rc = afis_queries_upload(ctx, queries, n_q, &q);
    if (rc != AFIS_OK) return rc;
    rc = afis_search_resident(ctx, q, scores, parts, status, k, topk_idx, topk_score);
    afis_queries_free(ctx, q);
    return rc;
}

int afis_search_dat(afis_ctx* ctx, const void* const* latent_bytes, const size_t* lens, int n_q, float* scores, float* parts,
                    int32_t* status, int k, int64_t* topk_idx, float* topk_score)
{
    if (!ctx || n_q < 0 || (n_q > 0 && (!latent_bytes || !lens))) return fail(ctx, AFIS_EINVAL, "afis_search_dat: bad argument");
    std::vector<HostTemplate> ts(n_q);
    std::vector<std::vector<afis_minutiae_view>> mv(n_q);
    std::vector<std::vector<afis_texture_view>> tv(n_q);
    std::vector<afis_template_view> views(n_q);
    for (int i = 0; i < n_q; ++i) {
        (void)parse_latent_dat(latent_bytes[i], lens[i], ts[i]);
        views_of(ts[i], mv[i], tv[i], views[i]);
    }
    return afis_search(ctx, views.data(), n_q, scores, parts, status, k, topk_idx, topk_score);
}

}
```

### msu-latentafis_amd/csrc/afis_taps.cpp

```cpp
#include "afis_ctx.h"
#include "../../include/afis_matcher_taps.h"

using namespace afis;

static int ensure_codes_cf(afis_ctx* ctx, int variant)
{
    if ((variant != 6 && variant != 7) || ctx->codes_cf_built) return AFIS_OK;
    const int64_t G = ctx->gal.G;
    std::vector<int32_t> to((size_t)G + 1), cfb((size_t)G + 1);
    HIPCHK(ctx, hipMemcpyAsync(to.data(), ctx->gal.tex_off, to.size() * 4, hipMemcpyDeviceToHost, ctx->stream));
    HIPCHK(ctx, hipStreamSynchronize(ctx->stream));
    int64_t nblk = 0;
    for (int64_t t = 0; t < G; ++t) { cfb[(size_t)t] = (int32_t)nblk; const int64_t n = to[(size_t)t + 1] - to[(size_t)t]; nblk += n > 0 ? (n + 63) / 64 + 1 : 0; }
    cfb[(size_t)G] = (int32_t)nblk;
    if (nblk > 0x7fffffff / 64) return fail(ctx, AFIS_EINVAL, "adc_variant 6 / 7: shard too large for the direct kernel's code stream; split the gallery into more shards");
    HIPCHK(ctx, upload(ctx->g_tex_cf_blk, cfb, ctx->stream));
    HIPCHK(ctx, ctx->g_tex_codes_cf.ensure(std::max<size_t>((size_t)nblk * 64 * 16, 16)));
    ctx->gal.tex_cf_blk = ctx->g_tex_cf_blk.as<int32_t>();
    ctx->gal.tex_codes_cf = ctx->g_tex_codes_cf.as<uint4>();
    HIPCHK(ctx, launch_codes_cf(ctx->gal, ctx->g_tex_codes_cf.p, ctx->stream));
    HIPCHK(ctx, hipStreamSynchronize(ctx->stream));
    ctx->codes_cf_built = true;
    return AFIS_OK;
}

static int direct_rowmax(afis_ctx* ctx, const QueryDev& d, const GalleryDev& g, int variant, int chunk, hipEvent_t after_lut)
{
    HIPCHK(ctx, ctx->lut.ensure(std::max<size_t>((size_t)d.n_tiles * kTileFloats * 4, 16)));
    HIPCHK(ctx, launch_lut_build(d, ctx->codewords.as<float>(), ctx->lut.as<float>(), variant, ctx->stream));
    if (after_lut) HIPCHK(ctx, hipEventRecord(after_lut, ctx->stream));
    HIPCHK(ctx, launch_adc_rowmax(d, g, ctx->lut.as<float>(), chunk, variant, ctx->rm_val.as<float>(), ctx->rm_arg.as<int32_t>(), ctx->stream));
    return AFIS_OK;
}

static int direct_adc_stage(afis_ctx* ctx, const QueryDev& d, int chunk, hipEvent_t after_lut)
{
    const int rcf = ensure_codes_cf(ctx, ctx->adc_variant);
    if (rcf != AFIS_OK) return rcf;
    return direct_rowmax(ctx, d, ctx->gal, ctx->adc_variant, chunk, after_lut);
}
__attribute__((constructor)) static void set_direct_adc_stage() { g_direct_adc_stage = direct_adc_stage; }

extern "C" {

int afis_debug_phase_cycles(afis_ctx* ctx, unsigned long long* out32, int reset)
{
    if (!ctx || !out32) return AFIS_EINVAL;
    HIPCHK(ctx, hipSetDevice(ctx->device));
    HIPCHK(ctx, hipStreamSynchronize(ctx->stream));
    HIPCHK(ctx, read_phase_cycles(out32, reset != 0));
    unsigned long long gph[16];
    HIPCHK(ctx, read_graph_phase_cycles(gph, reset != 0));
    for (int i = 0; i < 8; ++i) { out32[5 + i] = gph[i]; out32[21 + i] = gph[8 + i]; }
    return AFIS_OK;
}

int afis_debug_refine_stats(afis_ctx* ctx, unsigned long long* out8, int reset)
{
    if (!ctx || !out8) return fail(ctx, AFIS_EINVAL, "afis_debug_refine_stats: bad argument");
    HIPCHK(ctx, hipSetDevice(ctx->device));
    HIPCHK(ctx, hipStreamSynchronize(ctx->stream));
    for (int i = 0; i < 8; ++i) out8[i] = 0;
    if (!ctx->mf_stats.p) return AFIS_OK;
    HIPCHK(ctx, hipMemcpy(out8, ctx->mf_stats.p, 64, hipMemcpyDeviceToHost));
    if (reset) HIPCHK(ctx, hipMemset(ctx->mf_stats.p, 0, 64));
    return AFIS_OK;
}

int afis_debug_atan2_grid(afis_ctx* ctx, int R, float* out)
{
    if (!ctx || !out || R < 0 || R > 4096) return fail(ctx, AFIS_EINVAL, "afis_debug_atan2_grid: bad argument");
    HIPCHK(ctx, hipSetDevice(ctx->device));
    const size_t n = (size_t)(2 * R + 1) * (2 * R + 1);
    DevBuf d;
    HIPCHK(ctx, d.ensure(n * 4));
    hipError_t e = launch_debug_atan2_grid(R, d.as<float>(), ctx->stream);
    if (e == hipSuccess) e = hipMemcpyAsync(out, d.p, n * 4, hipMemcpyDeviceToHost, ctx->stream);
    if (e == hipSuccess) e = hipStreamSynchronize(ctx->stream);
    d.release();
    if (e != hipSuccess) return fail(ctx, AFIS_EDEVICE, std::string("afis_debug_atan2_grid: ") + hipGetErrorString(e));
    return AFIS_OK;
}

int afis_debug_graph_arith(afis_ctx* ctx, unsigned long long* out8)
{
    if (!ctx || !out8) return fail(ctx, AFIS_EINVAL, "afis_debug_graph_arith: bad argument");
    HIPCHK(ctx, hipSetDevice(ctx->device));
    DevBuf d;
    HIPCHK(ctx, d.ensure(64));
    hipError_t e = launch_debug_graph_arith(d.as<unsigned long long>(), ctx->stream);
    if (e == hipSuccess) e = hipMemcpyAsync(out8, d.p, 64, hipMemcpyDeviceToHost, ctx->stream);
    if (e == hipSuccess) e = hipStreamSynchronize(ctx->stream);
    d.release();
    if (e != hipSuccess) return fail(ctx, AFIS_EDEVICE, std::string("afis_debug_graph_arith: ") + hipGetErrorString(e));
    return AFIS_OK;
}

int afis_debug_lut(afis_ctx* ctx, const afis_template_view* query, float* out, int32_t* n_rows)
{
    if (!ctx || !query || !out) return fail(ctx, AFIS_EINVAL, "afis_debug_lut: null argument");
    if (query->n_tex <= 0) { if (n_rows) *n_rows = 0; return AFIS_OK; }
    const afis_texture_view& x = query->tex[0];
    if (x.des_len != kDes || !x.des) return fail(ctx, AFIS_EINVAL, "afis_debug_lut: latent texture template needs fp32 descriptors of length 96");
    HIPCHK(ctx, hipSetDevice(ctx->device));
    DevBuf des, lut;
    std::vector<float> h(x.des, x.des + (size_t)x.n * kDes);
    HIPCHK(ctx, upload(des, h, ctx->stream));
    HIPCHK(ctx, lut.ensure((size_t)x.n * kM * kK * 4));
    HIPCHK(ctx, launch_lut_reference_layout(des.as<float>(), x.n, ctx->codewords.as<float>(), lut.as<float>(), ctx->stream));
    HIPCHK(ctx, hipMemcpyAsync(out, lut.p, (size_t)x.n * kM * kK * 4, hipMemcpyDeviceToHost, ctx->stream));
    HIPCHK(ctx, hipStreamSynchronize(ctx->stream));
    des.release(); lut.release();
    if (n_rows) *n_rows = x.n;
    return AFIS_OK;
}

int afis_debug_texture_rowmax(afis_ctx* ctx, const afis_template_view* query, int64_t gidx, float* val, int32_t* arg, int32_t* n_rows)
{
    if (!ctx || !query || !val || !arg) return fail(ctx, AFIS_EINVAL, "afis_debug_texture_rowmax: null argument");
    if (!ctx->committed) return fail(ctx, AFIS_ESTATE, "afis_debug_texture_rowmax: commit the gallery first");
    if (gidx < 0 || gidx >= ctx->gal.G) return fail(ctx, AFIS_EINVAL, "afis_debug_texture_rowmax: gallery index out of range");
    HIPCHK(ctx, hipSetDevice(ctx->device));
    QueryGroup grp; std::vector<int32_t> st;
    int rc = build_group(ctx, query, 1, grp, st);
    if (rc != AFIS_OK) { grp.release(); return rc; }
    const QueryDev& d = grp.dev;
    const int n_lt = grp.h_lt_n[0];
    if (n_rows) *n_rows = n_lt;
    if (n_lt > 0) {
        const size_t n_pairs = (size_t)ctx->gal.G;
        HIPCHK(ctx, ctx->rm_val.ensure(n_pairs * d.lt_pad * 4));
        HIPCHK(ctx, ctx->rm_arg.ensure(n_pairs * d.lt_pad * 4));
        HIPCHK(ctx, hipMemsetAsync(ctx->rm_val.p, 0, n_pairs * d.lt_pad * 4, ctx->stream));
        HIPCHK(ctx, hipMemsetAsync(ctx->rm_arg.p, 0, n_pairs * d.lt_pad * 4, ctx->stream));
        if (ctx->adc_variant == 9) { int rc9 = adc_stage_mfma(ctx, grp, true); if (rc9 != AFIS_OK) { grp.release(); return rc9; } }
        else if (ctx->adc_variant == 8) { int rc16 = adc_stage_q(ctx, grp, ctx->chunk > 0 ? ctx->chunk : 32, true); if (rc16 != AFIS_OK) { grp.release(); return rc16; } }
        else { int rcd = direct_adc_stage(ctx, d, ctx->chunk > 0 ? ctx->chunk : 32, nullptr); if (rcd != AFIS_OK) { grp.release(); return rcd; } }
        HIPCHK(ctx, hipMemcpyAsync(val, ctx->rm_val.as<float>() + (size_t)gidx * d.lt_pad, (size_t)n_lt * 4, hipMemcpyDeviceToHost, ctx->stream));
        HIPCHK(ctx, hipMemcpyAsync(arg, ctx->rm_arg.as<int32_t>() + (size_t)gidx * d.lt_pad, (size_t)n_lt * 4, hipMemcpyDeviceToHost, ctx->stream));
        HIPCHK(ctx, hipStreamSynchronize(ctx->stream));
    }
    grp.release();
    return AFIS_OK;
}

int afis_debug_stage_list(afis_ctx* ctx, const afis_template_view* query, int64_t gidx, int which, int stage,
                          float* sim, int32_t* li, int32_t* ri, int32_t* n)
{
    if (!ctx || !query || !sim || !li || !ri || !n || which < 0 || which > 3 || stage < 0 || stage > 2) return fail(ctx, AFIS_EINVAL, "afis_debug_stage_list: bad argument");
    if (!ctx->committed) return fail(ctx, AFIS_ESTATE, "afis_debug_stage_list: commit the gallery first");
    if (gidx < 0 || gidx >= ctx->gal.G) return fail(ctx, AFIS_EINVAL, "afis_debug_stage_list: gallery index out of range");
    HIPCHK(ctx, hipSetDevice(ctx->device));
    QueryGroup grp; std::vector<int32_t> st;
    int rc = build_group(ctx, query, 1, grp, st);
    if (rc != AFIS_OK) { grp.release(); return rc; }
    *n = -1;
    DevBuf d_out, d_n;
    auto body = [&]() -> int {
        if (st[0] != AFIS_QUERY_OK) return AFIS_OK;
        const QueryDev& d = grp.dev;
        GalleryDev one = ctx->gal;
        one.G = 1; one.minu_off += gidx; one.minu_tile_off += gidx; one.tex_off += gidx; one.empty += gidx;
        hipStream_t s = ctx->stream;
        HIPCHK(ctx, d_out.ensure(3 * (size_t)kTopTex * sizeof(MinuCand)));
        HIPCHK(ctx, d_n.ensure(3 * 4));
        HIPCHK(ctx, hipMemsetAsync(d_n.p, 0xff, 12, s));
        HIPCHK(ctx, ctx->parts.ensure(16));
        int slot = 0, cap = kTopTex;
        if (which == 0) {
            if (d.n_tiles <= 0) return AFIS_OK;
            HIPCHK(ctx, ctx->rm_val.ensure((size_t)d.lt_pad * 4)); HIPCHK(ctx, ctx->rm_arg.ensure((size_t)d.lt_pad * 4));
            const int av = ctx->adc_variant >= 8 ? 0 : ctx->adc_variant;
            { int rcf = ensure_codes_cf(ctx, av); if (rcf != AFIS_OK) return rcf; }
            if (av == 6 || av == 7) { one.tex_codes_cf = ctx->gal.tex_codes_cf; one.tex_cf_blk = ctx->gal.tex_cf_blk + gidx; }
            { int rcd = direct_rowmax(ctx, d, one, av, 32, nullptr); if (rcd != AFIS_OK) return rcd; }
            HIPCHK(ctx, launch_graph_texture(d, one, ctx->table.as<float>(), ctx->rm_val.as<float>(), ctx->rm_arg.as<int32_t>(), nullptr, nullptr, ctx->parts.as<float>(),
                                             d_out.as<MinuCand>(), d_n.as<int32_t>(), stage | (ctx->s89_tie_order << 8), s));
        } else {
            slot = which - 1; cap = kTopMinu;
            const size_t per_wg = minu_scratch_floats(grp.max_nL, ctx->max_nR, ctx->s3_tie_order);
            HIPCHK(ctx, ctx->scratch.ensure(per_wg * 4 * 64));
            HIPCHK(ctx, ctx->cands.ensure(3 * (size_t)kTopMinu * sizeof(MinuCand))); HIPCHK(ctx, ctx->cand_n.ensure(12)); HIPCHK(ctx, ctx->minu_fb.ensure(minu_fb_ints(3, 1) * 4));
            HIPCHK(ctx, launch_minu_cands(d, one, ctx->scratch.as<float>(), per_wg, 64, ctx->minu_generic | (ctx->s3_tie_order << 1), ctx->cands.as<MinuCand>(), ctx->cand_n.as<int32_t>(), ctx->minu_fb.as<int32_t>(), grp.max_nL, ctx->max_nR, nullptr, s));
            HIPCHK(ctx, launch_graph_minutiae(d, one, ctx->cands.as<MinuCand>(), ctx->cand_n.as<int32_t>(), ctx->parts.as<float>(), nullptr, nullptr,
                                              d_out.as<MinuCand>(), d_n.as<int32_t>(), stage | (ctx->s89_tie_order << 8), s));
        }
        std::vector<MinuCand> h((size_t)3 * kTopTex); int32_t hn[3] = {-1, -1, -1};
        HIPCHK(ctx, hipMemcpyAsync(h.data(), d_out.p, h.size() * sizeof(MinuCand), hipMemcpyDeviceToHost, s));
        HIPCHK(ctx, hipMemcpyAsync(hn, d_n.p, 12, hipMemcpyDeviceToHost, s));
        HIPCHK(ctx, hipStreamSynchronize(s));
        if (ctx->hg.empty[(size_t)gidx]) return AFIS_OK;
        *n = hn[slot];
        for (int t = 0; t < hn[slot]; ++t) { const MinuCand& c = h[(size_t)slot * cap + t]; sim[t] = c.sim; li[t] = c.li; ri[t] = c.ri; }
        return AFIS_OK;
    };
    rc = body();
    d_out.release(); d_n.release(); grp.release();
    return rc;
}


}
```

### msu-latentafis_amd/csrc/graph.hip

```cpp
#include "afis_device.h"
#include <type_traits>
#include "atan2f_libm.h"
#include "graph_arith.h"
#include "stdsort_order.h"

namespace afis {

#define AFIS_PI 3.1415926
typedef unsigned long long u64;

#ifdef AFIS_PHASE_TIMING
__device__ u64 g_graph_phase[16];
#define GPH_INIT() u64 gph_t0 = __builtin_readcyclecounter()
#define GPH(i) do { if (threadIdx.x == 0) { const u64 t1_ = __builtin_readcyclecounter(); sm.ph[(i)] += t1_ - gph_t0; gph_t0 = t1_; } } while (0)
#define GPH_T0() const u64 gph_k0 = __builtin_readcyclecounter()
#define GPH_K(i) do { if (threadIdx.x == 0) sm.ph[(i)] += __builtin_readcyclecounter() - gph_k0; } while (0)
#define GPH_ZERO() do { if (threadIdx.x < 16) sm.ph[threadIdx.x] = 0; WSYNC(); } while (0)
#define GPH_FLUSH() do { WSYNC(); if (threadIdx.x < 16 && sm.ph[threadIdx.x]) atomicAdd(&g_graph_phase[threadIdx.x], sm.ph[threadIdx.x]); } while (0)
#else
#define GPH_INIT() do {} while (0)
#define GPH(i) do {} while (0)
#define GPH_T0() do {} while (0)
#define GPH_K(i) do {} while (0)
#define GPH_ZERO() do {} while (0)
#define GPH_FLUSH() do {} while (0)
#endif

__device__ __forceinline__ uint32_t g_ord_f32(float v)
{
    v = v + 0.0f;
    const uint32_t u = __float_as_uint(v);
    return (u & 0x80000000u) ? ~u : (u | 0x80000000u);
}
__device__ __forceinline__ u64 g_make_key(float v, int idx) { return ((u64)g_ord_f32(v) << 32) | (uint32_t)(~(uint32_t)idx); }
__device__ __forceinline__ int g_wave_popc(bool p) { return __popcll(__ballot(p)); }
__device__ __forceinline__ int g_lane_prefix(u64 mask) { return __builtin_amdgcn_mbcnt_hi((uint32_t)(mask >> 32), __builtin_amdgcn_mbcnt_lo((uint32_t)mask, 0)); }
#define WSYNC() __syncthreads()

__device__ __forceinline__ int g_wave_max(int x)
{
    x = max(x, __builtin_amdgcn_update_dpp(0, x, 0xB1, 0xf, 0xf, false));
    x = max(x, __builtin_amdgcn_update_dpp(0, x, 0x4E, 0xf, 0xf, false));
    x = max(x, __builtin_amdgcn_update_dpp(0, x, 0x124, 0xf, 0xf, false));
    x = max(x, __builtin_amdgcn_update_dpp(0, x, 0x128, 0xf, 0xf, false));
    x = max(x, __builtin_amdgcn_update_dpp(x, x, 0x142, 0xa, 0xf, false));
    x = max(x, __builtin_amdgcn_update_dpp(x, x, 0x143, 0xc, 0xf, false));
    return __builtin_amdgcn_readlane(x, 63);
}

__device__ __forceinline__ int g_wave_sum(int x)
{
    x += __builtin_amdgcn_update_dpp(0, x, 0xB1, 0xf, 0xf, false);
    x += __builtin_amdgcn_update_dpp(0, x, 0x4E, 0xf, 0xf, false);
    x += __builtin_amdgcn_update_dpp(0, x, 0x124, 0xf, 0xf, false);
    x += __builtin_amdgcn_update_dpp(0, x, 0x128, 0xf, 0xf, false);
    x += __builtin_amdgcn_update_dpp(0, x, 0x142, 0xa, 0xf, false);
    x += __builtin_amdgcn_update_dpp(0, x, 0x143, 0xc, 0xf, false);
    return __builtin_amdgcn_readlane(x, 63);
}

struct Pt { int lx, ly, rx, ry; };
__device__ __forceinline__ int2 pack_xy(int lx, int ly, int rx, int ry) { return make_int2((lx & 0xffff) | (ly << 16), (rx & 0xffff) | (ry << 16)); }
__device__ __forceinline__ Pt unpack_xy(int2 v) { Pt p; p.lx = (int)(short)v.x; p.ly = v.x >> 16; p.rx = (int)(short)v.y; p.ry = v.y >> 16; return p; }

template <int N, bool OWN> struct SimStore { float simv[N]; };
template <int N> struct SimStore<N, false> {};

#ifndef AFIS_MINU_ALIAS
#define AFIS_MINU_ALIAS 1
#endif
template <int NMAX_, int CACHE_, bool OWN_SIM_>
struct __attribute__((aligned(16))) WaveSmem : SimStore<NMAX_, OWN_SIM_> {
    static constexpr int NMAX = NMAX_, CACHE = CACHE_;
    static constexpr bool OWN_SIM = OWN_SIM_;
    static constexpr bool ALIAS_ORI = NMAX_ > 128 || AFIS_MINU_ALIAS;
    static constexpr int W = (NMAX + 31) / 32;
    static constexpr int N4 = (NMAX + 3) / 4 * 4;
    static constexpr int U = (NMAX + 63) / 64;
    float b[N4];
    union {
        float cc[N4];
        struct { short order[NMAX]; short sel[NMAX]; } os;
    } y;
    short li[NMAX], ri[NMAX];
    int2 xy[NMAX];
    uint32_t hb[NMAX][W];
    union {
        float stash[CACHE * NMAX];
        struct { u64 keys[N4]; float lo[ALIAS_ORI ? 1 : NMAX], ro[ALIAS_ORI ? 1 : NMAX]; } s;
        struct { uint32_t keys[N4]; short te[NMAX], targ[NMAX]; } pick;
    } x;
#ifdef AFIS_PHASE_TIMING
    u64 ph[16];
#endif
};
template <class SM> __device__ __forceinline__ int l_row(int v) { if constexpr (SM::OWN_SIM) return v; else return v & 1023; }
template <class SM> __device__ __forceinline__ int r_pt(int v) { if constexpr (SM::OWN_SIM) return v; else return v & 1023; }
__device__ __forceinline__ int tex_slot_of(int li, int ri) { return ((li >> 10) & 31) | (((ri >> 10) & 31) << 5); }
__device__ __forceinline__ short tex_pack_l(int row, int slot) { return (short)(row | ((slot & 31) << 10)); }
__device__ __forceinline__ short tex_pack_r(int pt, int slot) { return (short)(pt | ((slot >> 5) << 10)); }
template <class SM>
__device__ __forceinline__ float list_sim(const SM& sm, const float* __restrict__ ext, int t)
{
    if constexpr (SM::OWN_SIM) return sm.simv[t];
    else return ext[tex_slot_of(sm.li[t], sm.ri[t])];
}

__device__ __forceinline__ int next_task(int32_t* ctr)
{
    int t;
    unsigned long long saved;
    asm volatile("s_mov_b64 %1, exec\n\t"
                 "s_mov_b64 exec, 1\n\t"
                 "global_atomic_add %0, %2, %3, %4 sc0\n\t"
                 "s_waitcnt vmcnt(0)\n\t"
                 "s_mov_b64 exec, %1"
                 : "=&v"(t), "=&s"(saved) : "v"(0), "v"(1), "s"(ctr) : "memory");
    return __builtin_amdgcn_readfirstlane(t);
}

template <class SM, int ref_tie>
__device__ __forceinline__ void sort_scores(SM& sm, int num, double thr)
{
    const int lane = threadIdx.x;
    constexpr int U = SM::U;
    uint32_t* const s_key = reinterpret_cast<uint32_t*>(sm.x.s.keys);
    uint32_t* const s_cnt = s_key + SM::N4;
    uint32_t* const s_gkey = reinterpret_cast<uint32_t*>(sm.y.cc);
    static_assert(sizeof(sm.x) >= (size_t)(SM::N4 + 128) * 4, "sort scratch exceeds the union");
    uint32_t m32[U]; int r[U];
    if (num <= 48) {
        const u64 mine = lane < num ? g_make_key(sm.b[lane], lane) : 0ull;
        if (lane < num) sm.x.s.keys[lane] = mine;
        WSYNC();
        int rr = 0;
        for (int k = 0; k < num; ++k) rr += sm.x.s.keys[k] > mine;
        if (ref_tie && num > 16) {
            int gg = 0;
            for (int k = 0; k < num; ++k) gg += (uint32_t)(sm.x.s.keys[k] >> 32) > (uint32_t)(mine >> 32);
            const bool tied = lane < num && gg != rr && !((double)sm.b[lane] < thr);
            if (__ballot(tied) != 0ull) {
                uint32_t* const k32 = reinterpret_cast<uint32_t*>(sm.x.s.keys) + 96;
                static_assert(sizeof(sm.x.s.keys) >= (96 + 48 + 48) * 4, "no room for the keys and the stack of the std::sort restatement");
                WSYNC();
                if (lane < num) { k32[lane] = (uint32_t)(mine >> 32); sm.y.os.order[lane] = (short)lane; }
                WSYNC();
                if (lane == 0) stdsort_prefix<uint16_t>(reinterpret_cast<uint16_t*>(sm.y.os.order), num, num, k32, reinterpret_cast<int*>(k32 + 48));
                WSYNC();
                return;
            }
        }
        WSYNC();
        if (lane < num) sm.y.os.order[rr] = (short)lane;
        WSYNC();
        return;
    }
    uint32_t kmin = 0xffffffffu, kmax = 0u;
#pragma unroll
    for (int u = 0; u < U; ++u) {
        const int t = lane + 64 * u;
        m32[u] = t < num ? g_ord_f32(sm.b[t]) : 0u;
        if (t < num) { s_key[t] = m32[u]; kmin = min(kmin, m32[u]); kmax = max(kmax, m32[u]); }
    }
#pragma unroll
    for (int off = 32; off >= 1; off >>= 1) { kmin = min(kmin, (uint32_t)__shfl_xor((int)kmin, off)); kmax = max(kmax, (uint32_t)__shfl_xor((int)kmax, off)); }
    const uint32_t span = kmax - kmin;
    const int sh = max(0, 26 - __clz((int)(span | 1u)));
    int bin[U];
#pragma unroll
    for (int u = 0; u < U; ++u) bin[u] = (int)((m32[u] - kmin) >> sh) & 63;
    s_cnt[lane] = 0u;
    WSYNC();
#pragma unroll
    for (int u = 0; u < U; ++u) if (lane + 64 * u < num) atomicAdd(&s_cnt[bin[u]], 1u);
    WSYNC();
    {
        const int own = (int)s_cnt[lane];
        int suf = own;
#pragma unroll
        for (int off = 1; off < 64; off <<= 1) { const int v = __shfl_down(suf, off); if (lane + off < 64) suf += v; }
        WSYNC();
        s_cnt[lane] = (uint32_t)(suf - own); s_cnt[64 + lane] = (uint32_t)(suf - own);
    }
    WSYNC();
#pragma unroll
    for (int u = 0; u < U; ++u) if (lane + 64 * u < num) s_gkey[atomicAdd(&s_cnt[bin[u]], 1u)] = m32[u];
    WSYNC();
    int rsum = 0;
#pragma unroll
    for (int u = 0; u < U; ++u) {
        r[u] = 0;
        if (lane + 64 * u < num) {
            const int lo = (int)s_cnt[64 + bin[u]], hi = (int)s_cnt[bin[u]];
            int c = lo;
            for (int k = lo; k < hi; ++k) c += s_gkey[k] > m32[u];
            r[u] = c; rsum += c;
        }
    }
    if (g_wave_sum(rsum) != num * (num - 1) / 2) {
        u64 mine[U];
        int gg[U];
#pragma unroll
        for (int u = 0; u < U; ++u) { const int t = lane + 64 * u; mine[u] = t < num ? ((u64)m32[u] << 32) | (uint32_t)(~(uint32_t)t) : 0ull; r[u] = 0; gg[u] = 0; }
        for (int k = 0; k < num; ++k) {
            const u64 kk = ((u64)s_key[k] << 32) | (uint32_t)(~(uint32_t)k);
#pragma unroll
            for (int u = 0; u < U; ++u) { r[u] += kk > mine[u]; gg[u] += s_key[k] > m32[u]; }
        }
        if (ref_tie) {
            bool tied = false;
#pragma unroll
            for (int u = 0; u < U; ++u) { const int t = lane + 64 * u; tied |= t < num && gg[u] != r[u] && !((double)sm.b[t] < thr); }
            if (__ballot(tied) != 0ull) {
                WSYNC();
#pragma unroll
                for (int u = 0; u < U; ++u) { const int t = lane + 64 * u; if (t < num) sm.y.os.order[t] = (short)t; }
                WSYNC();
                if (lane == 0) stdsort_prefix<uint16_t>(reinterpret_cast<uint16_t*>(sm.y.os.order), num, num, s_key, reinterpret_cast<int*>(s_cnt));
                WSYNC();
                return;
            }
        }
    }
    WSYNC();
#pragma unroll
    for (int u = 0; u < U; ++u) { const int t = lane + 64 * u; if (t < num) sm.y.os.order[r[u]] = (short)t; }
    WSYNC();
}

template <class SM, class Compat>
__device__ int greedy(SM& sm, int num, double thr, Compat compatible)
{
    const int lane = threadIdx.x;
    constexpr int U = SM::U;
    int idx[U], li[U], ri[U];
    bool alive[U];
#pragma unroll
    for (int u = 0; u < U; ++u) {
        const int p = lane + 64 * u;
        idx[u] = 0; li[u] = -1; ri[u] = -1; alive[u] = false;
        if (p < num) {
            idx[u] = sm.y.os.order[p];
            li[u] = l_row<SM>(sm.li[idx[u]]); ri[u] = r_pt<SM>(sm.ri[idx[u]]);
            alive[u] = !((double)sm.b[idx[u]] < thr);
        }
    }
    int nsel = 0;
    for (;;) {
        int first = -1, cidx = 0, cli = 0, cri = 0;
#pragma unroll
        for (int u = 0; u < U; ++u) {
            const u64 m = __ballot(alive[u]);
            if (first < 0 && m) {
                const int fl = __ffsll((long long)m) - 1;
                first = 64 * u + fl;
                cidx = __shfl(idx[u], fl); cli = __shfl(li[u], fl); cri = __shfl(ri[u], fl);
            }
        }
        if (first < 0) break;
        if (lane == 0) sm.y.os.sel[nsel] = (short)cidx;
        ++nsel;
#pragma unroll
        for (int u = 0; u < U; ++u) {
            if (alive[u]) {
                const int p = lane + 64 * u;
                if (p == first || li[u] == cli || ri[u] == cri || !compatible(cidx, idx[u])) alive[u] = false;
            }
        }
    }
    WSYNC();
    return nsel;
}

template <class SM>
__device__ void compact(SM& sm, int n)
{
    const int lane = threadIdx.x;
    float sim[SM::U]; short li[SM::U], ri[SM::U]; int2 xy[SM::U];
#pragma unroll
    for (int u = 0; u < SM::U; ++u) {
        const int t = lane + 64 * u;
        sim[u] = 0.0f;
        if (t < n) { const int s = sm.y.os.sel[t]; if constexpr (SM::OWN_SIM) sim[u] = sm.simv[s]; li[u] = sm.li[s]; ri[u] = sm.ri[s]; xy[u] = sm.xy[s]; }
    }
    WSYNC();
#pragma unroll
    for (int u = 0; u < SM::U; ++u) {
        const int t = lane + 64 * u;
        if (t < n) { if constexpr (SM::OWN_SIM) sm.simv[t] = sim[u]; sm.li[t] = li[u]; sm.ri[t] = ri[u]; sm.xy[t] = xy[u]; }
    }
    WSYNC();
}

template <class SM>
__device__ __forceinline__ float seq_sum(const SM& sm, int num)
{
    float sum = 0.0f;
    const float4* c4 = reinterpret_cast<const float4*>(sm.y.cc);
#pragma unroll 4
    for (int k = 0; k < (num + 3) / 4; ++k) { const float4 v = c4[k]; sum += v.x; sum += v.y; sum += v.z; sum += v.w; }
    return sum;
}

template <bool LOOKUP>
__device__ __forceinline__ bool pair_dist(const Pt& a, const Pt& o, const float* __restrict__ table, float& dist)
{
    float d1, d2; bool ok = true;
    if (LOOKUP) {
        const int dx1 = abs(a.lx - o.lx), dx2 = abs(a.rx - o.rx), dy1 = abs(a.ly - o.ly), dy2 = abs(a.ry - o.ry);
        ok = !((dx1 >= kDistN) | (dx2 >= kDistN) | (dy1 >= kDistN) | (dy2 >= kDistN));
        d1 = sqrt_rn_pos((float)(256 * (dx1 * dx1 + dy1 * dy1)));
        d2 = sqrt_rn_pos((float)(256 * (dx2 * dx2 + dy2 * dy2)));
        (void)table;
    } else {
        const float dx1 = (float)(a.lx - o.lx), dx2 = (float)(a.rx - o.rx), dy1 = (float)(a.ly - o.ly), dy2 = (float)(a.ry - o.ry);
        const float p = dx1 * dx1, q = dy1 * dy1, r = dx2 * dx2, s = dy2 * dy2;
        d1 = sqrt_rn_pos(p + q);
        d2 = sqrt_rn_pos(r + s);
    }
    dist = fabsf(d1 - d2);
    return ok;
}
template <bool LOOKUP>
__device__ __forceinline__ bool pair_compatible(const Pt& a, const Pt& o, const float* __restrict__ table)
{
    float s1, s2; bool ok = true;
    if (LOOKUP) {
        const int dx1 = abs(a.lx - o.lx), dx2 = abs(a.rx - o.rx), dy1 = abs(a.ly - o.ly), dy2 = abs(a.ry - o.ry);
        ok = !((dx1 >= kDistN) | (dx2 >= kDistN) | (dy1 >= kDistN) | (dy2 >= kDistN));
        s1 = (float)(256 * (dx1 * dx1 + dy1 * dy1)); s2 = (float)(256 * (dx2 * dx2 + dy2 * dy2));
    } else {
        const float dx1 = (float)(a.lx - o.lx), dx2 = (float)(a.rx - o.rx), dy1 = (float)(a.ly - o.ly), dy2 = (float)(a.ry - o.ry);
        const float p = dx1 * dx1, q = dy1 * dy1, r = dx2 * dx2, s = dy2 * dy2;
        s1 = p + q; s2 = r + s;
    }
    const float d1 = __builtin_amdgcn_sqrtf(s1), d2 = __builtin_amdgcn_sqrtf(s2);
    const float dist = fabsf(d1 - d2);
    const float slack = fmaxf(d1, d2) * 4.76837158e-7f;
    if (fabsf(dist - 30.0f) > slack) return ok && dist < 30.0f;
    float exact;
    pair_dist<LOOKUP>(a, o, table, exact);
    return ok && exact < 30.0f;
}
template <bool RANGE_TEST>
__device__ __forceinline__ bool tex_pair_dist(int2 a, int2 o, float& dist)
{
    float n1, n2;
    pair_n(a, o, n1, n2);
    dist = 16.0f * fabsf(sqrt_rn_int(n1) - sqrt_rn_int(n2));
    return RANGE_TEST ? tex_in_range(a, o) : true;
}
template <bool RANGE_TEST>
__device__ __forceinline__ bool tex_pair_compatible(int2 a, int2 o)
{
    float n1, n2;
    pair_n(a, o, n1, n2);
    const bool ok = RANGE_TEST ? tex_in_range(a, o) : true;
    return pair_compatible_n<true>(n1, n2) && ok;
}

__device__ __forceinline__ float minu_pair_dist(int2 a, int2 o)
{
    float n1, n2;
    pair_n(a, o, n1, n2);
    return fabsf(sqrt_rn_int(n1) - sqrt_rn_int(n2));
}
__device__ __forceinline__ bool minu_pair_compatible(int2 a, int2 o)
{
    float n1, n2;
    pair_n(a, o, n1, n2);
    return pair_compatible_n<false>(n1, n2);
}

__device__ __forceinline__ float h_of_x(float x)
{
    const float q0 = x * 0.04f;
    const float r = fmaf(-q0, 25.0f, x);
    const float h = fmaf(r, 0.04f, q0);
    return __builtin_amdgcn_fmed3f(h, 0.0f, 1.0f);
}
__device__ __forceinline__ float h_value(float dist)
{
    const float x = 30.0f - dist;
    const float q0 = x * 0.04f;
    const float r = fmaf(-q0, 25.0f, x);
    const float h = fmaf(r, 0.04f, q0);
    return __builtin_amdgcn_fmed3f(h, 0.0f, 1.0f);
}

template <class SM, bool LOOKUP, int ITERS, int MODE, int REF_TIE>
__device__ int dist_filter(SM& sm, int num, const float* __restrict__ table, const float* __restrict__ ext)
{
    constexpr bool fast = MODE > 0;
    constexpr bool range_test = MODE == 1;
    auto compat_fast = [](int2 a, int2 o) -> bool { if (LOOKUP) return tex_pair_compatible<range_test>(a, o); return minu_pair_compatible(a, o); };
    auto dist_fast = [](int2 a, int2 o) -> float { float d; if (LOOKUP) { tex_pair_dist<range_test>(a, o, d); return d; } return minu_pair_dist(a, o); };
    constexpr int U = SM::U, W = SM::W, NMAX = SM::NMAX;
    [[maybe_unused]] constexpr int PH = LOOKUP ? 8 : 0;
    GPH_INIT();
    const int lane = threadIdx.x;
    for (int i = lane; i < num * W; i += 64) sm.hb[i / W][i % W] = 0u;
    int2 me[U];
#pragma unroll
    for (int u = 0; u < U; ++u) {
        const int t = lane + 64 * u;
        if (t < SM::N4) { sm.b[t] = t < num ? list_sim(sm, ext, t) : 0.0f; sm.y.cc[t] = 0.0f; }
        me[u] = t < num ? sm.xy[t] : make_int2(0, 0);
    }
    WSYNC();
    const int half = num >> 1;
    const bool even = !(num & 1);
    uint32_t* const hb0 = &sm.hb[0][0];
    auto pair = [&](int2 own, int t, int k, int2 other) {
        if (fast ? compat_fast(own, other) : pair_compatible<LOOKUP>(unpack_xy(own), unpack_xy(other), table)) {
            atomicOr(hb0 + (t * W + (k >> 5)), 1u << (k & 31));
            atomicOr(hb0 + (__umul24(k, W) + (t >> 5)), 1u << (t & 31));
        }
    };
    const int tail0 = num & ~63, R = num - tail0;
    const bool grouped = R > 0 && R <= 32;
    const int n_wide = grouped ? tail0 : num;
    uint32_t kb[U];
    const uint32_t num8 = (uint32_t)num * 8u;
#pragma unroll
    for (int u = 0; u < U; ++u) { const int t = lane + 64 * u; kb[u] = t < num ? (uint32_t)t * 8u : 0u; }
#ifndef AFIS_PAIR_UNROLL
#define AFIS_PAIR_UNROLL 1
#endif
    constexpr int DU = fast ? AFIS_PAIR_UNROLL : 1;
    auto pair_loop = [&](auto ua_tag) {
    constexpr int UA = decltype(ua_tag)::value;
    for (int d = 1; d <= half; d += DU) {
        int2 other[DU][UA];
        int kk[DU][UA];
#pragma unroll
        for (int s2 = 0; s2 < DU; ++s2) {
#pragma unroll
            for (int u = 0; u < UA; ++u) {
                const uint32_t a = kb[u] + 8u;
                kb[u] = min(a, a - num8);
                other[s2][u] = *reinterpret_cast<const int2*>(reinterpret_cast<const char*>(sm.xy) + kb[u]);
                kk[s2][u] = (int)(kb[u] >> 3);
            }
        }
        __builtin_amdgcn_sched_barrier(0);
        if (fast) {
            float n1[DU][UA], n2[DU][UA]; bool hit[DU][UA], near[DU][UA]; bool any_near = false;
#pragma unroll
            for (int s2 = 0; s2 < DU; ++s2) {
#pragma unroll
                for (int u = 0; u < UA; ++u) {
                    pair_n(me[u], other[s2][u], n1[s2][u], n2[s2][u]);
                    hit[s2][u] = pair_compatible_t<LOOKUP>(n1[s2][u], n2[s2][u], near[s2][u]);
                    hit[s2][u] = hit[s2][u] | near[s2][u];
                }
            }
            (void)any_near;
#pragma unroll
            for (int s2 = 0; s2 < DU; ++s2) {
                const bool last = d + s2 == half && even;
#pragma unroll
                for (int u = 0; u < UA; ++u) {
                    const int t = lane + 64 * u, k = kk[s2][u];
                    bool ok = hit[s2][u] && t < n_wide && d + s2 <= half && !(last && t >= half);
                    if (LOOKUP && range_test) ok = ok && tex_in_range(me[u], other[s2][u]);
                    if constexpr (LOOKUP) {
                        const int ts = t < num ? t : 0;
                        atomicOr(hb0 + (ts * W + (k >> 5)), ok ? 1u << (k & 31) : 0u);
                        atomicOr(hb0 + (__umul24(k, W) + (ts >> 5)), ok ? 1u << (ts & 31) : 0u);
                    } else if (ok) {
                        atomicOr(hb0 + (t * W + (k >> 5)), 1u << (k & 31));
                        atomicOr(hb0 + (__umul24(k, W) + (t >> 5)), 1u << (t & 31));
                    }
                }
            }
        } else {
            const bool last = d == half && even;
#pragma unroll
            for (int u = 0; u < UA; ++u) {
                const int t = lane + 64 * u;
                if (t < n_wide && !(last && t >= half)) pair(me[u], t, kk[0][u], other[0][u]);
            }
        }
    }
    };
    const int n_blk = (n_wide + 63) >> 6;
    if (n_blk >= U) pair_loop(std::integral_constant<int, U>{});
    else if (U > 1 && n_blk == U - 1) pair_loop(std::integral_constant<int, (U > 1 ? U - 1 : 1)>{});
    else if (n_blk > 0) pair_loop(std::integral_constant<int, U>{});
    if (grouped) {
        const int sh = R <= 8 ? 3 : R <= 16 ? 4 : 5, RG = 1 << sh, dstep = 64 >> sh;
        const int r = lane & (RG - 1), t = tail0 + r;
        const bool row = r < R;
        const int2 own = row ? sm.xy[t] : make_int2(0, 0);
        int d = 1 + (lane >> sh);
        int k = t + d; k = k >= num ? k - num : k;
        for (int d0 = 1; d0 <= half; d0 += dstep) {
            if (row && d <= half && !(d == half && even && t >= half)) pair(own, t, k, sm.xy[k]);
            d += dstep; k += dstep; k = k >= num ? k - num : k;
        }
    }
    WSYNC();
    GPH(PH + 0);
    int myrow[U], trip[U], rlen[U];
    const int Wn = (num + 31) / 32;
    {
        int cnt[U];
#pragma unroll
        for (int u = 0; u < U; ++u) {
            const int t = lane + 64 * u;
            int c = -1;
            if (t < num) {
                c = 0; for (int w = 0; w < Wn; ++w) c += __popc(sm.hb[t][w]);
                sm.y.os.sel[t] = (short)c;
                c = min(c >> 2, 15);
            }
            cnt[u] = c;
        }
        int base = 0;
        for (int bk = 15; bk >= 0; --bk) {
#pragma unroll
            for (int u = 0; u < U; ++u) {
                const bool in = cnt[u] == bk;
                const u64 m = __ballot(in);
                if (in) sm.y.os.order[base + g_lane_prefix(m)] = (short)(lane + 64 * u);
                base += __popcll(m);
            }
        }
        WSYNC();
#pragma unroll
        for (int u = 0; u < U; ++u) {
            const int p = lane + 64 * u;
            myrow[u] = p < num ? (int)sm.y.os.order[p] : -1;
            rlen[u] = myrow[u] >= 0 ? (int)sm.y.os.sel[myrow[u]] : 0;
            trip[u] = g_wave_max(rlen[u]);
        }
        WSYNC();
        for (int t = num + lane; t < SM::N4; t += 64) sm.y.cc[t] = 0.0f;
    }
    int2 mine[U];
#pragma unroll
    for (int u = 0; u < U; ++u) mine[u] = myrow[u] >= 0 ? sm.xy[myrow[u]] : make_int2(0, 0);
    constexpr bool kFlat = NMAX > 128;
#ifndef AFIS_MINU_VALN
#define AFIS_MINU_VALN 0
#endif
    constexpr int kValN = kFlat ? 0 : AFIS_MINU_VALN, kIdxN = 4 * SM::CACHE - 4 * kValN;
    static_assert(kValN * NMAX * 4 + kIdxN * NMAX <= (int)sizeof(sm.x.stash), "index lists + value stash exceed the stash space");
    float* const vst = sm.x.stash;
    unsigned char* const idx8 = reinterpret_cast<unsigned char*>(sm.x.stash + kValN * NMAX);
#ifndef AFIS_MINU_REGN
#define AFIS_MINU_REGN 0
#endif
    constexpr int kRegN = kFlat ? 0 : AFIS_MINU_REGN;
    static_assert(kRegN <= kIdxN, "cached values need their neighbour indices");
    float hreg[U][kRegN > 0 ? kRegN : 1];
    int cur_w[U]; uint32_t cur_bits[U];
#pragma unroll
    for (int u = 0; u < U; ++u) { cur_w[u] = 0; cur_bits[u] = 0u; }
    auto value = [&](int2 own, int k) -> float {
        float dist;
        if (fast && LOOKUP) {
            float n1, n2;
            pair_n(own, sm.xy[k], n1, n2);
            return h_of_x(fmaf(-16.0f, fabsf(sqrt_rn_int(n1) - sqrt_rn_int(n2)), 30.0f));
        }
        if (fast) dist = dist_fast(own, sm.xy[k]);
        else pair_dist<LOOKUP>(unpack_xy(own), unpack_xy(sm.xy[k]), table, dist);
        return h_value(dist);
    };
    for (int it = 0; it < ITERS; ++it) {
#pragma unroll
        for (int u = 0; u < U; ++u) {
            const int t = myrow[u];
            const uint32_t* hrow = sm.hb[t >= 0 ? t : 0];
            float acc = 0.0f;
            if (it == 0) {
                if (t >= 0) {
                    int w = 0;
                    uint32_t bits = hrow[0];
#pragma unroll
                    for (int r = 0; r < kRegN; ++r) {
                        if (r < trip[u]) {
                            while (bits == 0u && w + 1 < Wn) { ++w; bits = hrow[w]; }
                            const bool have = bits != 0u;
                            const int k = (w * 32 + __ffs(bits) - 1) & 255;
                            bits &= bits - 1;
                            const float h = value(mine[u], k);
                            idx8[r * NMAX + t] = (unsigned char)k;
                            hreg[u][r] = h;
                            const float p = h * sm.b[k];
                            acc += have ? p : 0.0f;
                        }
                    }
                    for (int n = kRegN; n < trip[u]; ++n) {
                        if (n == kIdxN) { cur_w[u] = w; cur_bits[u] = bits; }
                        while (bits == 0u && w + 1 < Wn) { ++w; bits = hrow[w]; }
                        const bool have = bits != 0u;
                        const int k = (w * 32 + __ffs(bits) - 1) & 255;
                        bits &= bits - 1;
                        const float h = value(mine[u], k);
                        if (n < kIdxN) idx8[n * NMAX + t] = (unsigned char)k;
                        if (n < kValN) vst[n * NMAX + t] = h;
                        const float p = h * sm.b[k];
                        acc += have ? p : 0.0f;
                    }
                }
            } else {
                const int nV = min(trip[u], kValN), nA = min(trip[u], kIdxN);
                const int tt = t >= 0 ? t : 0;
                for (int n = 0; n < nV; ++n) {
                    const int k = idx8[n * NMAX + tt];
                    const float p = vst[n * NMAX + tt] * sm.b[k];
                    acc += n < rlen[u] ? p : 0.0f;
                }
#pragma unroll
                for (int r = 0; r < kRegN; ++r) {
                    if (r < nA) {
                        const int k = idx8[r * NMAX + tt];
                        const float p = hreg[u][r] * sm.b[k];
                        acc += r < rlen[u] ? p : 0.0f;
                    }
                }
                for (int n = max(nV, kRegN); n < nA; ++n) {
                    const int k = idx8[n * NMAX + tt];
                    const float p = value(mine[u], k) * sm.b[k];
                    acc += n < rlen[u] ? p : 0.0f;
                }
                if (trip[u] > kIdxN) {
                    int w = cur_w[u];
                    uint32_t bits = cur_bits[u];
                    for (int n = kIdxN; n < trip[u]; ++n) {
                        while (bits == 0u && w + 1 < Wn) { ++w; bits = t >= 0 ? hrow[w] : 0u; }
                        const bool have = bits != 0u;
                        const int k = (w * 32 + __ffs(bits) - 1) & 255;
                        bits &= bits - 1;
                        const float p = value(mine[u], k) * sm.b[k];
                        acc += have ? p : 0.0f;
                    }
                }
            }
            if (t >= 0) sm.y.cc[t] = acc;
        }
        WSYNC();
        const float sum = seq_sum(sm, num);
        const float scale = (float)(1.0 / ((double)sum + 0.00001));
#pragma unroll
        for (int u = 0; u < U; ++u) { const int t = lane + 64 * u; if (t < num) sm.b[t] = sm.y.cc[t] * scale; }
        WSYNC();
    }
    GPH(PH + 1);
    sort_scores<SM, REF_TIE>(sm, num, 0.0001);
    GPH(PH + 2);
    const int nsel = greedy(sm, num, 0.0001, [&sm, table, dist_fast](int a, int o) {
        if (!((sm.hb[a][o >> 5] >> (o & 31)) & 1u)) return false;
        float dist;
        if (fast) dist = dist_fast(sm.xy[a], sm.xy[o]);
        else pair_dist<LOOKUP>(unpack_xy(sm.xy[a]), unpack_xy(sm.xy[o]), table, dist);
        return !((double)h_value(dist) < 0.00001);
    });
    compact(sm, nsel);
    GPH(PH + 3);
    return nsel;
}

__device__ __forceinline__ float adjust_angle(float angle)
{
    if ((double)angle > AFIS_PI) angle = (float)((double)angle - 2 * AFIS_PI);
    else if ((double)angle < -AFIS_PI) angle = (float)((double)angle + 2 * AFIS_PI);
    return angle;
}
__device__ __forceinline__ float fold_pi(float d)
{
    if ((double)d > AFIS_PI) d = (float)(2 * AFIS_PI - (double)d);
    return d;
}
__device__ __forceinline__ float atan2_f32(float y, float x) { return afis_atan2f_libm(y, x); }

__device__ __forceinline__ bool angle_compatible(const Pt& p1, float lo1, float ro1, const Pt& p2, float lo2, float ro2)
{
    float angle_1 = adjust_angle(lo1 - lo2);
    float angle_2 = adjust_angle(ro1 - ro2);
    float angle_diff = fold_pi(fabsf(angle_1 - angle_2));
    if ((double)angle_diff > AFIS_PI / 4.) return false;
    const float dx_1 = (float)(p1.lx - p2.lx), dy_1 = (float)(p1.ly - p2.ly);
    const float line_angle_1 = -atan2_f32(dy_1, dx_1);
    angle_1 = adjust_angle(lo1 - line_angle_1);
    const float dx_2 = (float)(p1.rx - p2.rx), dy_2 = (float)(p1.ry - p2.ry);
    const float line_angle_2 = -atan2_f32(dy_2, dx_2);
    angle_2 = adjust_angle(ro1 - line_angle_2);
    angle_diff = fold_pi(fabsf(angle_1 - angle_2));
    if ((double)angle_diff > AFIS_PI / 6.) return false;
    angle_1 = adjust_angle(lo2 - line_angle_1);
    angle_2 = adjust_angle(ro2 - line_angle_2);
    angle_diff = fold_pi(fabsf(angle_1 - angle_2));
    if ((double)angle_diff > AFIS_PI / 6.) return false;
    return true;
}

template <class SM, int REF_TIE>
__device__ int angle_filter(SM& sm, int num, const float* __restrict__ lori, const float* __restrict__ rori)
{
    constexpr int W = SM::W;
    [[maybe_unused]] constexpr int PH = SM::NMAX > 128 ? 8 : 0;
    GPH_INIT();
    const int lane = threadIdx.x;
    if constexpr (SM::ALIAS_ORI) {
        for (int t = lane; t < num; t += 64) { sm.b[t] = lori[l_row<SM>(sm.li[t])]; sm.y.cc[t] = rori[r_pt<SM>(sm.ri[t])]; }
        for (int i = lane; i < num * W; i += 64) sm.hb[i / W][i % W] = 0u;
    } else {
        for (int t = lane; t < num; t += 64) { sm.x.s.lo[t] = lori[l_row<SM>(sm.li[t])]; sm.x.s.ro[t] = rori[r_pt<SM>(sm.ri[t])]; }
        for (int i = lane; i < num * W; i += 64) sm.hb[i / W][i % W] = 0u;
        const float s0 = (float)(1.0 / num);
        for (int t = lane; t < SM::N4; t += 64) { sm.b[t] = t < num ? s0 : 0.0f; sm.y.cc[t] = 0.0f; }
    }
    WSYNC();
    const int half = num >> 1;
    const bool even = !(num & 1);
    auto pair = [&](int t, int k) {
        const int i = t < k ? t : k, j = t < k ? k : t;
        bool ok;
        if constexpr (SM::ALIAS_ORI) ok = angle_compatible(unpack_xy(sm.xy[i]), sm.b[i], sm.y.cc[i], unpack_xy(sm.xy[j]), sm.b[j], sm.y.cc[j]);
        else ok = angle_compatible(unpack_xy(sm.xy[i]), sm.x.s.lo[i], sm.x.s.ro[i], unpack_xy(sm.xy[j]), sm.x.s.lo[j], sm.x.s.ro[j]);
        if (ok) {
            atomicOr(&sm.hb[i][j >> 5], 1u << (j & 31));
            atomicOr(&sm.hb[j][i >> 5], 1u << (i & 31));
        }
    };
    const int tail0 = num & ~63, R = num - tail0;
    const bool grouped = R > 0 && R <= 32;
    const int n_wide = grouped ? tail0 : num;
    for (int d = 1; n_wide > 0 && d <= half; ++d) {
        for (int t = lane; t < n_wide; t += 64) {
            if (d == half && even && t >= half) continue;
            int k = t + d; if (k >= num) k -= num;
            pair(t, k);
        }
    }
    if (grouped) {
        const int sh = R <= 8 ? 3 : R <= 16 ? 4 : 5, RG = 1 << sh, dstep = 64 >> sh;
        const int r = lane & (RG - 1), t = tail0 + r;
        int d = 1 + (lane >> sh);
        int k = t + d; k = k >= num ? k - num : k;
        for (int d0 = 1; d0 <= half; d0 += dstep) {
            if (r < R && d <= half && !(d == half && even && t >= half)) pair(t, k);
            d += dstep; k += dstep; k = k >= num ? k - num : k;
        }
    }
    WSYNC();
    if constexpr (SM::ALIAS_ORI) {
        const float s0 = (float)(1.0 / num);
        for (int t = lane; t < SM::N4; t += 64) { sm.b[t] = t < num ? s0 : 0.0f; sm.y.cc[t] = 0.0f; }
        WSYNC();
    }
    GPH(PH + 4);
    for (int it = 0; it < 5; ++it) {
        for (int t = lane; t < num; t += 64) {
            float s1 = 0.0f;
            for (int w = 0; w < (num + 31) / 32; ++w) {
                uint32_t bits = sm.hb[t][w];
                while (bits) { const int k = w * 32 + __ffs(bits) - 1; bits &= bits - 1; s1 += sm.b[k]; }
            }
            sm.y.cc[t] = s1;
        }
        WSYNC();
        float sum = seq_sum(sm, num);
        sum = (float)(1.0 / ((double)sum + 0.00001));
        for (int t = lane; t < num; t += 64) sm.b[t] = sm.y.cc[t] * sum;
        WSYNC();
    }
    GPH(PH + 5);
    sort_scores<SM, REF_TIE>(sm, num, 0.001);
    const int nsel = greedy(sm, num, 0.001, [&sm](int a, int o) { return (sm.hb[a][o >> 5] >> (o & 31)) & 1u; });
    compact(sm, nsel);
    GPH(PH + 6);
    return nsel;
}

template <class SM, bool LOOKUP, int ITERS, int REF_TIE>
__device__ __forceinline__ float graph_score(SM& sm, int num, const float* __restrict__ table, const float* __restrict__ lori,
                                             const float* __restrict__ rori, const float* __restrict__ ext, int& n_survivors, int stop_after = 2, int mode = 0)
{
    n_survivors = num;
    if (stop_after == 0) return 0.0f;
    if (mode == 2 && LOOKUP) num = dist_filter<SM, LOOKUP, ITERS, 2, REF_TIE>(sm, num, table, ext);
    else if (mode >= 1) num = dist_filter<SM, LOOKUP, ITERS, 1, REF_TIE>(sm, num, table, ext);
    else num = dist_filter<SM, LOOKUP, ITERS, 0, REF_TIE>(sm, num, table, ext);
    n_survivors = num;
    if (mode >= 1) {
        for (int t = threadIdx.x; t < num; t += 64) {
            const int2 v = sm.xy[t];
            int lx, ly, rx, ry;
            unpack_h2(v.x, lx, ly); unpack_h2(v.y, rx, ry);
            sm.xy[t] = pack_xy(lx, ly, rx, ry);
        }
        WSYNC();
    }
    if (stop_after == 1) return 0.0f;
    n_survivors = 0;
    if (num < 2) return 0.0f;
    num = angle_filter<SM, REF_TIE>(sm, num, lori, rori);
    n_survivors = num;
    for (int t = threadIdx.x; t < num; t += 64) sm.b[t] = list_sim(sm, ext, t);
    WSYNC();
    float score = 0.0f;
    for (int i = 0; i < num; ++i) score += sm.b[i];
    return score;
}

struct GraphTap { MinuCand* out; int32_t* n; int stage; };
template <class SM>
__device__ __forceinline__ void tap_write(const GraphTap& tap, const SM& sm, const float* __restrict__ ext, long long task, int n, int cap)
{
    for (int t = threadIdx.x; t < n; t += 64) { MinuCand c; c.sim = list_sim(sm, ext, t); c.li = l_row<SM>(sm.li[t]); c.ri = r_pt<SM>(sm.ri[t]); tap.out[(size_t)task * cap + t] = c; }
    if (threadIdx.x == 0) tap.n[task] = n;
}

#ifndef AFIS_TEX_CACHE
#define AFIS_TEX_CACHE 2
#endif
#ifndef AFIS_TEX_WAVES
#define AFIS_TEX_WAVES 4
#endif
typedef WaveSmem<kTopTex, AFIS_TEX_CACHE, false> TexSmem;
constexpr int kTexRegs = (kTexMax + 63) / 64;

template <int REF_TIE>
__global__ __launch_bounds__(64) __attribute__((amdgpu_waves_per_eu(AFIS_TEX_WAVES, AFIS_TEX_WAVES))) void k_graph_texture(QueryDev q, GalleryDev g, const float* __restrict__ table_dist,
                                                      const float* __restrict__ rm_val, const int32_t* __restrict__ rm_arg,
                                                      const float* __restrict__ rm_cv, const int32_t* __restrict__ rm_n,
                                                      float* __restrict__ parts, GraphTap tap)
{
    __shared__ TexSmem sm;
    const int lane = threadIdx.x;
    GPH_ZERO();
    const int n_tasks = q.nq * g.G;
    for (;;) {
        const int task = next_task(g.task_ctr + 0);
        if (task >= n_tasks) break;
        GPH_T0();
        const int qi = task / g.G, gi = task - qi * g.G;
        const int l0 = q.lt_off[qi], n_lt = q.lt_off[qi + 1] - l0;
        const int r0 = g.tex_off[gi], n_rt = g.tex_off[gi + 1] - r0;
        float* out = parts + (size_t)task * 4 + 3;
        if (n_lt <= 0 || n_rt <= 0) { if (lane == 0) { *out = 0.0f; if (tap.out) tap.n[task] = -1; } continue; }
        const size_t o = (size_t)task * q.lt_pad;
        int num;
        if (n_lt > kTopTex) {
            const bool compact = rm_n != nullptr;
            const int n_in = compact ? rm_n[task] : n_lt;
            const int n_regs = (n_in + 63) >> 6;
            uint32_t key[kTexRegs]; int arg[kTexRegs];
#pragma unroll
            for (int u = 0; u < kTexRegs; ++u) {
                const int e = u * 64 + lane;
                const bool in = e < n_in;
                key[u] = 0u; arg[u] = 0;
                if (u < n_regs) {
                    key[u] = in ? g_ord_f32(compact ? rm_cv[o + e] : rm_val[o + e]) : 0u;
                    arg[u] = in ? rm_arg[o + e] : 0;
                }
            }
            uint32_t T = 0;
            for (int bit = 31; bit >= 0; --bit) {
                const uint32_t cand = T | (1u << bit);
                int c = 0;
#pragma unroll
                for (int u = 0; u < kTexRegs; ++u) if (u < n_regs) c += g_wave_popc(key[u] >= cand);
                if (c >= kTopTex) { T = cand; if (c == kTopTex) break; }
            }
            int n_gt = 0;
#pragma unroll
            for (int u = 0; u < kTexRegs; ++u) if (u < n_regs) n_gt += g_wave_popc(key[u] > T);
            const int need = kTopTex - n_gt;
            int base_gt = 0, base_eq = 0;
            uint32_t* const key32 = sm.x.pick.keys;
#pragma unroll
            for (int u = 0; u < kTexRegs; ++u) {
                if (u < n_regs) {
                    const int e = u * 64 + lane;
                    const bool gt = key[u] > T, eq = key[u] == T;
                    const u64 mg = __ballot(gt), me = __ballot(eq);
                    int pos = -1;
                    if (gt) pos = base_gt + g_lane_prefix(mg);
                    else if (eq) { const int r = base_eq + g_lane_prefix(me); if (r < need) pos = n_gt + r; }
                    if (pos >= 0) { key32[pos] = key[u]; sm.x.pick.te[pos] = tex_pack_l(compact ? arg[u] & 0xffff : e, e); sm.x.pick.targ[pos] = tex_pack_r(compact ? arg[u] >> 16 : arg[u], e); }
                    base_gt += __popcll(mg); base_eq += __popcll(me);
                }
            }
            WSYNC();
            num = kTopTex;
            uint32_t m32[TexSmem::U]; int r[TexSmem::U];
            uint32_t* const s_cnt = reinterpret_cast<uint32_t*>(sm.b);
            uint32_t* const s_gkey = reinterpret_cast<uint32_t*>(sm.y.cc);
            int dmax = 0;
#pragma unroll
            for (int u = 0; u < TexSmem::U; ++u) {
                const int t = lane + 64 * u;
                m32[u] = t < num ? key32[t] : T;
                dmax = max(dmax, (int)((m32[u] - T) >> 1));
            }
            dmax = g_wave_max(dmax);
            const int shift = max(0, 27 - __clz(dmax | 1));
            int bin[TexSmem::U];
#pragma unroll
            for (int u = 0; u < TexSmem::U; ++u) bin[u] = min((int)((m32[u] - T) >> shift), 63);
            s_cnt[lane] = 0u;
            WSYNC();
#pragma unroll
            for (int u = 0; u < TexSmem::U; ++u) if (lane + 64 * u < num) atomicAdd(&s_cnt[bin[u]], 1u);
            WSYNC();
            {
                const int own = (int)s_cnt[lane];
                int suf = own;
#pragma unroll
                for (int off = 1; off < 64; off <<= 1) { const int v = __shfl_down(suf, off); if (lane + off < 64) suf += v; }
                WSYNC();
                s_cnt[lane] = (uint32_t)(suf - own); s_cnt[64 + lane] = (uint32_t)(suf - own);
            }
            WSYNC();
#pragma unroll
            for (int u = 0; u < TexSmem::U; ++u) if (lane + 64 * u < num) s_gkey[atomicAdd(&s_cnt[bin[u]], 1u)] = m32[u];
            WSYNC();
#pragma unroll
            for (int u = 0; u < TexSmem::U; ++u) {
                r[u] = 0;
                if (lane + 64 * u < num) {
                    const int lo = (int)s_cnt[64 + bin[u]], hi = (int)s_cnt[bin[u]];
                    int c = lo;
                    for (int k = lo; k < hi; ++k) c += s_gkey[k] > m32[u];
                    r[u] = c;
                }
            }
            int rsum = 0;
#pragma unroll
            for (int u = 0; u < TexSmem::U; ++u) rsum += r[u];
            if (g_wave_sum(rsum) != kTopTex * (kTopTex - 1) / 2) {
                u64 mine[TexSmem::U];
#pragma unroll
                for (int u = 0; u < TexSmem::U; ++u) { const int t = lane + 64 * u; mine[u] = t < num ? ((u64)key32[t] << 32) | (uint32_t)(~(uint32_t)(sm.x.pick.te[t] & 1023)) : 0ull; r[u] = 0; }
                for (int k = 0; k < num; ++k) {
                    const u64 kk = ((u64)key32[k] << 32) | (uint32_t)(~(uint32_t)(sm.x.pick.te[k] & 1023));
#pragma unroll
                    for (int u = 0; u < TexSmem::U; ++u) r[u] += kk > mine[u];
                }
            }
#pragma unroll
            for (int u = 0; u < TexSmem::U; ++u) {
                const int t = lane + 64 * u;
                if (t < num) { sm.li[r[u]] = sm.x.pick.te[t]; sm.ri[r[u]] = sm.x.pick.targ[t]; }
            }
        } else {
            num = n_lt;
            for (int t = lane; t < num; t += 64) { sm.li[t] = tex_pack_l(t, t); sm.ri[t] = tex_pack_r(rm_n ? rm_arg[o + t] >> 16 : rm_arg[o + t], t); }
        }
        WSYNC();
        int out_of_range = 0, not_small = 0;
        short2 lp4[TexSmem::U], rp4[TexSmem::U];
#pragma unroll
        for (int u = 0; u < TexSmem::U; ++u) {
            const int t = lane + 64 * u;
            lp4[u] = make_short2(0, 0); rp4[u] = make_short2(0, 0);
            if (t < num) {
                lp4[u] = q.lt_xy[l0 + (sm.li[t] & 1023)]; rp4[u] = g.tex_xy[r0 + (sm.ri[t] & 1023)];
                out_of_range |= (lp4[u].x | lp4[u].y | rp4[u].x | rp4[u].y) & ~2047;
                not_small |= ((unsigned)lp4[u].x > 49u) | ((unsigned)lp4[u].y > 49u) | ((unsigned)rp4[u].x > 49u) | ((unsigned)rp4[u].y > 49u);
            }
        }
        const int mode = __ballot(out_of_range != 0) != 0ull ? 0 : (__ballot(not_small != 0) == 0ull ? 2 : 1);
#pragma unroll
        for (int u = 0; u < TexSmem::U; ++u) {
            const int t = lane + 64 * u;
            if (t < num) sm.xy[t] = mode ? make_int2(pack_h2(lp4[u].x, lp4[u].y), pack_h2(rp4[u].x, rp4[u].y)) : pack_xy(lp4[u].x, lp4[u].y, rp4[u].x, rp4[u].y);
        }
        WSYNC();
        GPH_K(15);
        int n_surv;
        const float* const row_max = (rm_n ? rm_cv : rm_val) + o;
        const float score = graph_score<TexSmem, true, 3, REF_TIE>(sm, num, table_dist, q.lt_ori + l0, g.tex_ori + r0, row_max, n_surv, tap.out ? tap.stage : 2, mode);
        if (lane == 0) *out = score;
        if (tap.out) tap_write(tap, sm, row_max, task, n_surv, kTopTex);
        WSYNC();
    }
    GPH_FLUSH();
}

hipError_t launch_graph_texture(const QueryDev& q, const GalleryDev& g, const float* table_dist,
                                const float* rm_val, const int32_t* rm_arg, const float* rm_cv, const int32_t* rm_n, float* parts, MinuCand* tap_out, int32_t* tap_n, int tap_stage, hipStream_t stream)
{
    const long long n_tasks = (long long)q.nq * g.G;
    if (n_tasks <= 0) return hipSuccess;
    if (n_tasks > 0x7ffffff0LL || !g.task_ctr) return hipErrorInvalidValue;
    const int grid = (int)(n_tasks < 16384 ? n_tasks : 16384);
    hipError_t e0 = hipMemsetAsync(g.task_ctr + 0, 0, 4, stream);
    if (e0 != hipSuccess) return e0;
    const GraphTap tap{tap_out, tap_n, tap_stage & 255};
    if ((tap_stage >> 8) & 1) hipLaunchKernelGGL(k_graph_texture<1>, dim3(grid), dim3(64), 0, stream, q, g, table_dist, rm_val, rm_arg, rm_cv, rm_n, parts, tap);
    else hipLaunchKernelGGL(k_graph_texture<0>, dim3(grid), dim3(64), 0, stream, q, g, table_dist, rm_val, rm_arg, rm_cv, rm_n, parts, tap);
    return hipGetLastError();
}

#ifndef AFIS_MINU_CACHE
#define AFIS_MINU_CACHE 3
#endif
typedef WaveSmem<kTopMinu, AFIS_MINU_CACHE, true> MinuGraphSmem;

#ifndef AFIS_MINU_WAVES
#define AFIS_MINU_WAVES 6
#endif
template <int REF_TIE>
__global__ __launch_bounds__(64) __attribute__((amdgpu_waves_per_eu(AFIS_MINU_WAVES, AFIS_MINU_WAVES))) void k_graph_minutiae(QueryDev q, GalleryDev g, const MinuCand* __restrict__ cands,
                                                       const int32_t* __restrict__ cand_n, float* __restrict__ parts,
                                                       short4* __restrict__ corr_out, int32_t* __restrict__ corr_n, GraphTap tap)
{
    __shared__ MinuGraphSmem sm;
    const int lane = threadIdx.x;
    GPH_ZERO();
    const int n_tasks = q.nq * 3 * g.G;
    for (;;) {
        const int task = next_task(g.task_ctr + 1);
        if (task >= n_tasks) break;
        GPH_T0();
        const int gi = task % g.G;
        const int qs = task / g.G;
        const int qi = qs / 3, s = qs - qi * 3;
        float* out = parts + ((size_t)qi * g.G + gi) * 4 + s;
        const int num = cand_n[task];
        if (num <= 0) { if (lane == 0) { *out = 0.0f; if (corr_n) corr_n[task] = 0; if (tap.out) tap.n[task] = -1; } continue; }
        const int l0 = q.lm_off[qs], r0 = g.minu_off[gi];
        const MinuCand* c = cands + (size_t)task * kTopMinu;
        int out_of_range = 0;
        short2 lp2[MinuGraphSmem::U], rp2[MinuGraphSmem::U];
#pragma unroll
        for (int u = 0; u < MinuGraphSmem::U; ++u) {
            const int t = lane + 64 * u;
            lp2[u] = make_short2(0, 0); rp2[u] = make_short2(0, 0);
            if (t < num) {
                const MinuCand cd = c[t];
                sm.simv[t] = cd.sim; sm.li[t] = cd.li; sm.ri[t] = cd.ri;
                lp2[u] = q.lm_xy[l0 + cd.li]; rp2[u] = g.minu_xy[r0 + cd.ri];
                out_of_range |= (lp2[u].x | lp2[u].y | rp2[u].x | rp2[u].y) & ~2047;
            }
        }
        const int mode = __ballot(out_of_range != 0) == 0ull ? 1 : 0;
#pragma unroll
        for (int u = 0; u < MinuGraphSmem::U; ++u) {
            const int t = lane + 64 * u;
            if (t < num) sm.xy[t] = mode ? make_int2(pack_h2(lp2[u].x, lp2[u].y), pack_h2(rp2[u].x, rp2[u].y)) : pack_xy(lp2[u].x, lp2[u].y, rp2[u].x, rp2[u].y);
        }
        WSYNC();
        GPH_K(7);
        int n_surv;
        const float score = graph_score<MinuGraphSmem, false, 5, REF_TIE>(sm, num, nullptr, q.lm_ori + l0, g.minu_ori + r0, nullptr, n_surv, tap.out ? tap.stage : 2, mode);
        if (lane == 0) *out = score;
        if (tap.out) tap_write(tap, sm, nullptr, task, n_surv, kTopMinu);
        if (corr_out) {
            for (int t = lane; t < n_surv; t += 64) {
                const Pt p = unpack_xy(sm.xy[t]);
                corr_out[(size_t)task * kTopMinu + t] = make_short4((short)p.lx, (short)p.ly, (short)p.rx, (short)p.ry);
            }
            if (lane == 0) corr_n[task] = n_surv;
        }
        WSYNC();
    }
    GPH_FLUSH();
}

hipError_t launch_graph_minutiae(const QueryDev& q, const GalleryDev& g, const MinuCand* cands, const int32_t* cand_n,
                                 float* parts, short4* corr_out, int32_t* corr_n, MinuCand* tap_out, int32_t* tap_n, int tap_stage, hipStream_t stream, bool join)
{
    const long long n_tasks = (long long)q.nq * 3 * g.G;
    if (n_tasks <= 0) return hipSuccess;
    if (n_tasks > 0x7ffffff0LL || !g.task_ctr) return hipErrorInvalidValue;
    const int grid = (int)(n_tasks < 32768 ? n_tasks : 32768);
    hipError_t e0 = join ? hipSuccess : hipMemsetAsync(g.task_ctr + 1, 0, 4, stream);
    if (e0 != hipSuccess) return e0;
    const GraphTap tap{tap_out, tap_n, tap_stage & 255};
    if ((tap_stage >> 8) & 1) hipLaunchKernelGGL(k_graph_minutiae<1>, dim3(grid), dim3(64), 0, stream, q, g, cands, cand_n, parts, corr_out, corr_n, tap);
    else hipLaunchKernelGGL(k_graph_minutiae<0>, dim3(grid), dim3(64), 0, stream, q, g, cands, cand_n, parts, corr_out, corr_n, tap);
    return hipGetLastError();
}

__global__ __launch_bounds__(256) void k_debug_atan2_grid(int R, float* __restrict__ out)
{
    const int W = 2 * R + 1;
    const long long idx = (long long)blockIdx.x * 256 + threadIdx.x;
    if (idx >= (long long)W * W) return;
    const int dy = (int)(idx / W) - R, dx = (int)(idx % W) - R;
    out[idx] = atan2_f32((float)dy, (float)dx);
}
hipError_t launch_debug_atan2_grid(int R, float* out, hipStream_t stream)
{
    const long long n = (long long)(2 * R + 1) * (2 * R + 1);
    hipLaunchKernelGGL(k_debug_atan2_grid, dim3((unsigned)((n + 255) / 256)), dim3(256), 0, stream, R, out);
    return hipGetLastError();
}

__device__ __forceinline__ void arith_check(bool tex, float f1, float f2, unsigned long long* cnt)
{
    const float d = fabsf(sqrt_rn_pos(f1) - sqrt_rn_pos(f2));
    const bool ref = tex ? 16.0f * d < 30.0f : d < 30.0f;
    const int a = tex ? pair_compatible_alg<true>(f1, f2) : pair_compatible_alg<false>(f1, f2);
    const bool full = tex ? pair_compatible_n<true>(f1, f2) : pair_compatible_n<false>(f1, f2);
    atomicAdd(cnt + 0, 1ull);
    if (a == 2) atomicAdd(cnt + 1, 1ull);
    if ((a != 2 && (a == 1) != ref) || full != ref) atomicAdd(cnt + 2, 1ull);
}
__global__ __launch_bounds__(256) void k_debug_graph_arith(int part, unsigned long long* __restrict__ cnt)
{
    constexpr unsigned kMaxN = 2u * 2047u * 2047u;
    if (part == 0) {
        const unsigned n = blockIdx.x * 256u + threadIdx.x;
        if (n <= kMaxN && __float_as_uint(sqrt_rn_int((float)n)) != __float_as_uint(sqrt_rn_pos((float)n))) atomicAdd(cnt, 1ull);
    } else if (part == 3) {
        const int dx = (int)blockIdx.x - 2047, dy = (int)(blockIdx.y * 256u + threadIdx.x) - 2047;
        if (dy > 2047) return;
        const int ax = dx > 0 ? dx : 0, ox = dx > 0 ? 0 : -dx, ay = dy > 0 ? dy : 0, oy = dy > 0 ? 0 : -dy;
        const float n = diff_n(pack_h2(ax, ay), pack_h2(ox, oy));
        int bx, by; unpack_h2(pack_h2(ax, ay), bx, by);
        if (__float_as_uint(n) != __float_as_uint((float)(dx * dx + dy * dy)) || bx != ax || by != ay) atomicAdd(cnt, 1ull);
    } else if (part == 1) {
        const unsigned n1 = blockIdx.x, n2 = blockIdx.y * 256u + threadIdx.x;
        if (n1 <= 4802u && n2 <= 4802u) arith_check(true, (float)n1, (float)n2, cnt + 1);
    } else {
        const unsigned n1 = blockIdx.x * 256u + threadIdx.x;
        if (n1 > kMaxN) return;
        const double a = sqrt((double)n1);
        for (int sg = -1; sg <= 1; sg += 2) {
            const double b = a + 30.0 * sg;
            if (b < 0) continue;
            const long long c = (long long)(b * b + 0.5);
            for (int j = -12; j <= 12; ++j) { const long long n2 = c + j; if (n2 >= 0 && n2 <= (long long)kMaxN) arith_check(false, (float)n1, (float)n2, cnt + 4); }
        }
    }
}
hipError_t launch_debug_graph_arith(unsigned long long* cnt8, hipStream_t stream)
{
    constexpr unsigned kMaxN = 2u * 2047u * 2047u;
    hipError_t e = hipMemsetAsync(cnt8, 0, 64, stream);
    if (e != hipSuccess) return e;
    hipLaunchKernelGGL(k_debug_graph_arith, dim3((kMaxN + 256) / 256), dim3(256), 0, stream, 0, cnt8);
    hipLaunchKernelGGL(k_debug_graph_arith, dim3(4803, 19), dim3(256), 0, stream, 1, cnt8);
    hipLaunchKernelGGL(k_debug_graph_arith, dim3((kMaxN + 256) / 256), dim3(256), 0, stream, 2, cnt8);
    hipLaunchKernelGGL(k_debug_graph_arith, dim3(4095, 16), dim3(256), 0, stream, 3, cnt8 + 7);
    return hipGetLastError();
}

hipError_t read_graph_phase_cycles(unsigned long long* out16, bool reset)
{
#ifdef AFIS_PHASE_TIMING
    hipError_t e = hipMemcpyFromSymbol(out16, HIP_SYMBOL(g_graph_phase), 16 * sizeof(u64));
    if (e != hipSuccess) return e;
    if (reset) { u64 z[16] = {}; e = hipMemcpyToSymbol(HIP_SYMBOL(g_graph_phase), z, sizeof(z)); }
    return e;
#else
    for (int i = 0; i < 16; ++i) out16[i] = 0;
    return hipSuccess;
#endif
}

}
```

Measured before the change: 49.04.

## Move graph-filter per-candidate step cache from LDS to per-workgroup global slabs

Replaces the small LDS-resident cache used by the distance filter in the texture and minutiae graph kernels (AFIS_TEX_CACHE/AFIS_MINU_CACHE) with per-workgroup global-memory slabs holding 48 or 32 steps per candidate. The slabs are sized from the persistent grid sizes and charged against the group memory budget. The aim is to cut LDS footprint and recomputation in dist_filter by caching more steps. In exchange it adds global-memory traffic and device allocations, and reduces the memory left for query batching.

```diff
diff --git a/msu-latentafis_amd/csrc/afis_api.cpp b/msu-latentafis_amd/csrc/afis_api.cpp
--- a/msu-latentafis_amd/csrc/afis_api.cpp
+++ b/msu-latentafis_amd/csrc/afis_api.cpp
@@ -101,7 +101,7 @@
     free_gallery_dev(c);
     c->codewords.release(); c->table.release(); c->lut.release(); c->rm_val.release(); c->rm_arg.release(); c->rm_cv.release(); c->rm_n.release();
     c->parts.release(); c->scores.release(); c->scratch.release(); c->cands.release(); c->cand_n.release(); c->minu_fb.release(); c->diag.release(); c->topk_idx.release(); c->topk_score.release(); c->lutq.release(); c->lutq_min.release(); c->lutq_rng.release(); c->lutq_rowc.release(); c->lut32.release();
-    c->mf_cw16.release(); c->mf_cwn.release(); c->mf_bfrag.release(); c->mf_rowk.release(); c->mf_rec.release(); c->mf_stats.release();
+    c->mf_cw16.release(); c->mf_cwn.release(); c->mf_bfrag.release(); c->mf_rowk.release(); c->mf_rec.release(); c->mf_stats.release(); c->tex_slab.release(); c->minu_slab.release();
     lap("destroying events and the context's stream");
     for (auto& e : c->evpool) if (e) (void)hipEventDestroy(e);
     if (c->stream) (void)hipStreamDestroy(c->stream);
@@ -161,6 +161,8 @@
     else if (n == "minu_fast_max_latent") *value = rt_class_max_latent(4);
     else if (n == "minu_fast_max_rolled") *value = rt_class_max_rolled(4);
     else if (n == "minu_fast_max_cells") *value = rt_class_simi_floats(4);
+    else if (n == "graph_slab_steps_texture") *value = kTexSlabSteps;
+    else if (n == "graph_slab_steps_minutiae") *value = kMinuSlabSteps;
     else if (n == "mf_stats") *value = ctx->mf_collect_stats;
     else if (n == "rowmax_budget_mb") *value = ctx->rowmax_budget_bytes >> 20;
     else if (n == "lut_dtype") *value = 32;
diff --git a/msu-latentafis_amd/csrc/afis_ctx.h b/msu-latentafis_amd/csrc/afis_ctx.h
--- a/msu-latentafis_amd/csrc/afis_ctx.h
+++ b/msu-latentafis_amd/csrc/afis_ctx.h
@@ -95,6 +95,7 @@
     int mf_collect_stats = 0;
     DevBuf lutq, lutq_min, lutq_rng, lutq_rowc, lut32;
     DevBuf lut, rm_val, rm_arg, rm_cv, rm_n, parts, scores, scratch, cands, cand_n, minu_fb, topk_idx, topk_score;
+    DevBuf tex_slab, minu_slab;
     DevBuf diag;
     std::vector<unsigned long long> h_diag;
     void* h_pin = nullptr; size_t h_pin_bytes = 0;
@@ -185,6 +186,7 @@
                    bool refine_now = true, unsigned long long* diag = nullptr);
 typedef int (*DirectAdcStage)(afis_ctx* ctx, const QueryDev& d, int chunk, hipEvent_t after_lut);
 extern DirectAdcStage g_direct_adc_stage __attribute__((visibility("hidden")));
+int64_t graph_slab_bytes(int64_t n_pairs);
 int wait_streams(afis_ctx* ctx, std::initializer_list<hipStream_t> streams, const char* what);
 void register_context(afis_ctx* ctx); void unregister_context(afis_ctx* ctx);
 int drain_abandoned(afis_ctx* ctx);
diff --git a/msu-latentafis_amd/csrc/afis_device.h b/msu-latentafis_amd/csrc/afis_device.h
--- a/msu-latentafis_amd/csrc/afis_device.h
+++ b/msu-latentafis_amd/csrc/afis_device.h
@@ -150,13 +150,20 @@
        kDiagCandsClk = 4, kDiagCandsWall = 5,
        kDiagBoundClk = 6, kDiagBoundWall = 7,
        kDiagWords = 16 };
+constexpr int kTexSlabSteps = 48, kMinuSlabSteps = 32;
+constexpr size_t kTexSlabWgBytes = (size_t)((kTopTex + 63) / 64) * kTexSlabSteps * 64 * 5;
+constexpr size_t kMinuSlabWgBytes = (size_t)((kTopMinu + 63) / 64) * kMinuSlabSteps * 64 * 5;
+inline int graph_texture_grid(long long n_tasks) { return (int)(n_tasks < 16384 ? n_tasks : 16384); }
+inline int graph_minutiae_grid(long long n_tasks) { return (int)(n_tasks < 32768 ? n_tasks : 32768); }
+inline size_t graph_texture_slab_bytes(long long n_tasks) { return n_tasks > 0 ? (size_t)graph_texture_grid(n_tasks) * kTexSlabWgBytes : 0; }
+inline size_t graph_minutiae_slab_bytes(long long n_tasks) { return n_tasks > 0 ? (size_t)graph_minutiae_grid(n_tasks) * kMinuSlabWgBytes : 0; }
 hipError_t launch_graph_texture(const QueryDev& q, const GalleryDev& g, const float* table_dist,
-                                const float* rm_val, const int32_t* rm_arg, const float* rm_cv, const int32_t* rm_n, float* parts, MinuCand* tap_out, int32_t* tap_n, int tap_stage, hipStream_t stream);
+                                const float* rm_val, const int32_t* rm_arg, const float* rm_cv, const int32_t* rm_n, float* parts, void* slab, size_t slab_bytes, MinuCand* tap_out, int32_t* tap_n, int tap_stage, hipStream_t stream);
 hipError_t launch_minu_cands(const QueryDev& q, const GalleryDev& g, float* scratch, size_t scratch_floats_per_wg, int n_wg,
                              int force_generic, MinuCand* cands, int32_t* cand_n, int32_t* fallback , int max_nL, int max_nR,
                              unsigned long long* diag , hipStream_t stream);
 hipError_t launch_graph_minutiae(const QueryDev& q, const GalleryDev& g, const MinuCand* cands, const int32_t* cand_n,
-                                 float* parts, short4* corr_out, int32_t* corr_n, MinuCand* tap_out, int32_t* tap_n, int tap_stage, hipStream_t stream, bool join = false);
+                                 float* parts, short4* corr_out, int32_t* corr_n, void* slab, size_t slab_bytes, MinuCand* tap_out, int32_t* tap_n, int tap_stage, hipStream_t stream, bool join = false);
 hipError_t launch_fuse(const QueryDev& q, const GalleryDev& g, const float* parts, float* scores, hipStream_t stream);
 
 hipError_t launch_topk(const float* scores, int n_q, int G, int k, long long index_base, long long* out_idx, float* out_score, hipStream_t stream);
diff --git a/msu-latentafis_amd/csrc/afis_search.cpp b/msu-latentafis_amd/csrc/afis_search.cpp
--- a/msu-latentafis_amd/csrc/afis_search.cpp
+++ b/msu-latentafis_amd/csrc/afis_search.cpp
@@ -4,6 +4,10 @@
 
 namespace afis {
 
+int64_t graph_slab_bytes(int64_t n_pairs)
+{
+    return (int64_t)graph_texture_slab_bytes(n_pairs) + 2 * (int64_t)graph_minutiae_slab_bytes(3 * n_pairs);
+}
 int64_t group_bytes_per_query(const afis_ctx* ctx, int64_t G)
 {
     const int64_t per_pair = (int64_t)kTexMax * 8 + (ctx->adc_variant == 9 ? (int64_t)kTexMax * kMfRecBytesPerRow : 0) + 3 * (int64_t)kTopMinu * (int64_t)sizeof(MinuCand) + 3 * 4 + 16 + 8;
@@ -13,13 +17,13 @@
 {
     const int64_t lt_pad = std::max<int64_t>(kTileRows, (lt_max + kTileRows - 1) / kTileRows * kTileRows), R_pad = (rows_total + 31) / 32 * 32;
     const int64_t per_pair = lt_pad * 8 + 3 * (int64_t)kTopMinu * (int64_t)sizeof(MinuCand) + 3 * 4 + 16 + 8;
-    return std::max<int64_t>(1, G) * (nq * per_pair + (ctx->adc_variant == 9 ? R_pad * kMfRecBytesPerRow : 0));
+    return std::max<int64_t>(1, G) * (nq * per_pair + (ctx->adc_variant == 9 ? R_pad * kMfRecBytesPerRow : 0)) + graph_slab_bytes(nq * std::max<int64_t>(1, G));
 }
 
 namespace { std::mutex g_ctx_mutex; std::vector<afis_ctx*> g_ctx_live; }
 static size_t held_group_bytes(const afis_ctx* c)
 {
-    return c->rm_val.bytes + c->rm_arg.bytes + c->rm_cv.bytes + c->rm_n.bytes + c->mf_rec.bytes + c->cands.bytes + c->cand_n.bytes + c->parts.bytes + c->minu_fb.bytes;
+    return c->rm_val.bytes + c->rm_arg.bytes + c->rm_cv.bytes + c->rm_n.bytes + c->mf_rec.bytes + c->cands.bytes + c->cand_n.bytes + c->parts.bytes + c->minu_fb.bytes + c->tex_slab.bytes + c->minu_slab.bytes;
 }
 void register_context(afis_ctx* c) { std::lock_guard<std::mutex> lk(g_ctx_mutex); g_ctx_live.push_back(c); }
 void unregister_context(afis_ctx* c) { std::lock_guard<std::mutex> lk(g_ctx_mutex); g_ctx_live.erase(std::remove(g_ctx_live.begin(), g_ctx_live.end(), c), g_ctx_live.end()); }
@@ -175,7 +179,7 @@
     HIPCHK(ctx, hipSetDevice(ctx->device));
     { const int rcd = drain_abandoned(ctx); if (rcd != AFIS_OK) return rcd; }
     const int64_t G = std::max<int64_t>(1, ctx->gal.G);
-    const int64_t by_mem = group_budget_bytes(ctx) / group_bytes_per_query(ctx, G);
+    const int64_t by_mem = std::max<int64_t>(0, group_budget_bytes(ctx) - graph_slab_bytes(INT64_C(1) << 40)) / group_bytes_per_query(ctx, G);
     const int64_t want = ctx->query_batch > 0 ? ctx->query_batch : launch_group_latents(G);
     int per = (int)std::max<int64_t>(1, std::min<int64_t>(want, by_mem));
     afis_queries* q = new afis_queries();
@@ -336,6 +340,8 @@
             HIPCHK(ctx, ctx->cands.ensure(n_pairs * 3 * kTopMinu * sizeof(MinuCand)));
             HIPCHK(ctx, ctx->cand_n.ensure(n_pairs * 3 * 4));
             HIPCHK(ctx, ctx->minu_fb.ensure(minu_fb_ints(n_pairs * 3, (size_t)G) * 4));
+            HIPCHK(ctx, ctx->tex_slab.ensure(graph_texture_slab_bytes((long long)n_pairs)));
+            HIPCHK(ctx, ctx->minu_slab.ensure(2 * graph_minutiae_slab_bytes(3 * (long long)n_pairs)));
             {
                 const size_t per_wg = minu_scratch_floats(nL_max, ctx->max_nR, ctx->s3_tie_order);
                 int n_wg = 1024;
@@ -456,11 +462,13 @@
             const bool minutiae_light = cells_m <= ctx->overlap_cell_ratio * cells_t;
             const bool overlap = ctx->adc_variant == 9 && ctx->stream_lo != nullptr && !ctx->overlap_failed && n_pairs >= 65536 && minutiae_light;
             grp.overlapped = overlap;
+            const size_t minu_slab_1 = graph_minutiae_slab_bytes(3 * (long long)n_pairs);
+            HIPCHK(ctx, ctx->tex_slab.ensure(graph_texture_slab_bytes((long long)n_pairs))); HIPCHK(ctx, ctx->minu_slab.ensure(2 * minu_slab_1));
             const bool compact9 = ctx->adc_variant == 9;
             auto minutiae_stage = [&]() -> int {
                 HIPCHK(ctx, launch_minu_cands(d, g, ctx->scratch.as<float>(), per_wg, n_wg, ctx->minu_generic | (ctx->s3_tie_order << 1), ctx->cands.as<MinuCand>(), ctx->cand_n.as<int32_t>(), ctx->minu_fb.as<int32_t>(), grp.max_nL, ctx->max_nR, diag_row, s));
                 HIPCHK(ctx, hipEventRecord(ev[7], s));
-                HIPCHK(ctx, launch_graph_minutiae(d, g, ctx->cands.as<MinuCand>(), ctx->cand_n.as<int32_t>(), grp_parts, nullptr, nullptr, nullptr, nullptr, 2 | (ctx->s89_tie_order << 8), s));
+                HIPCHK(ctx, launch_graph_minutiae(d, g, ctx->cands.as<MinuCand>(), ctx->cand_n.as<int32_t>(), grp_parts, nullptr, nullptr, ctx->minu_slab.p, minu_slab_1, nullptr, nullptr, 2 | (ctx->s89_tie_order << 8), s));
                 return AFIS_OK;
             };
             if (overlap) {
@@ -473,17 +481,17 @@
                 HIPCHK(ctx, launch_minu_cands(d, g, ctx->scratch.as<float>(), per_wg, n_wg, ctx->minu_generic | (ctx->s3_tie_order << 1), ctx->cands.as<MinuCand>(), ctx->cand_n.as<int32_t>(), ctx->minu_fb.as<int32_t>(), grp.max_nL, ctx->max_nR, diag_row, sh));
                 HIPCHK(ctx, hipMemsetAsync(g.task_ctr + 1, 0, 4, sh));
                 HIPCHK(ctx, hipEventRecord(ev[7], sh));
-                HIPCHK(ctx, launch_graph_minutiae(d, g, ctx->cands.as<MinuCand>(), ctx->cand_n.as<int32_t>(), grp_parts, nullptr, nullptr, nullptr, nullptr, 2 | (ctx->s89_tie_order << 8), sh, true));
+                HIPCHK(ctx, launch_graph_minutiae(d, g, ctx->cands.as<MinuCand>(), ctx->cand_n.as<int32_t>(), grp_parts, nullptr, nullptr, ctx->minu_slab.p, minu_slab_1, nullptr, nullptr, 2 | (ctx->s89_tie_order << 8), sh, true));
                 HIPCHK(ctx, hipEventRecord(ev[4], sh));
                 HIPCHK(ctx, hipStreamWaitEvent(s, ev[6], 0));
                 HIPCHK(ctx, hipEventRecord(ev[8], s));
                 rc9 = adc_refine_mfma(ctx, grp, false, true);
                 if (rc9 != AFIS_OK) return rc9;
                 HIPCHK(ctx, hipEventRecord(ev[2], s));
-                HIPCHK(ctx, launch_graph_texture(d, g, ctx->table.as<float>(), ctx->rm_val.as<float>(), ctx->rm_arg.as<int32_t>(), ctx->rm_cv.as<float>(), ctx->rm_n.as<int32_t>(), grp_parts, nullptr, nullptr, 2 | (ctx->s89_tie_order << 8), s));
+                HIPCHK(ctx, launch_graph_texture(d, g, ctx->table.as<float>(), ctx->rm_val.as<float>(), ctx->rm_arg.as<int32_t>(), ctx->rm_cv.as<float>(), ctx->rm_n.as<int32_t>(), grp_parts, ctx->tex_slab.p, ctx->tex_slab.bytes, nullptr, nullptr, 2 | (ctx->s89_tie_order << 8), s));
                 HIPCHK(ctx, hipEventRecord(ev[3], s));
                 HIPCHK(ctx, hipStreamWaitEvent(s, ev[7], 0));
-                HIPCHK(ctx, launch_graph_minutiae(d, g, ctx->cands.as<MinuCand>(), ctx->cand_n.as<int32_t>(), grp_parts, nullptr, nullptr, nullptr, nullptr, 2 | (ctx->s89_tie_order << 8), s, true));
+                HIPCHK(ctx, launch_graph_minutiae(d, g, ctx->cands.as<MinuCand>(), ctx->cand_n.as<int32_t>(), grp_parts, nullptr, nullptr, ctx->minu_slab.as<unsigned char>() + minu_slab_1, minu_slab_1, nullptr, nullptr, 2 | (ctx->s89_tie_order << 8), s, true));
                 HIPCHK(ctx, hipStreamWaitEvent(s, ev[4], 0));
                 any_overlap = true;
             } else {
@@ -499,7 +507,7 @@
             }
             HIPCHK(ctx, hipEventRecord(ev[2], s));
             HIPCHK(ctx, launch_graph_texture(d, g, ctx->table.as<float>(), ctx->rm_val.as<float>(), ctx->rm_arg.as<int32_t>(), compact9 ? ctx->rm_cv.as<float>() : nullptr,
-                                             compact9 ? ctx->rm_n.as<int32_t>() : nullptr, grp_parts, nullptr, nullptr, 2 | (ctx->s89_tie_order << 8), s));
+                                             compact9 ? ctx->rm_n.as<int32_t>() : nullptr, grp_parts, ctx->tex_slab.p, ctx->tex_slab.bytes, nullptr, nullptr, 2 | (ctx->s89_tie_order << 8), s));
             HIPCHK(ctx, hipEventRecord(ev[3], s));
             { int rcm = minutiae_stage(); if (rcm != AFIS_OK) return rcm; }
             HIPCHK(ctx, hipEventRecord(ev[4], s));
@@ -601,6 +609,7 @@
         HIPCHK(ctx, ctx->cand_n.ensure((size_t)n * 3 * 4));
         HIPCHK(ctx, ctx->minu_fb.ensure(minu_fb_ints(3, 1) * 4));
         HIPCHK(ctx, ctx->parts.ensure((size_t)n * 16));
+        HIPCHK(ctx, ctx->minu_slab.ensure(graph_minutiae_slab_bytes(3)));
         HIPCHK(ctx, d_xy.ensure((size_t)n * 3 * kTopMinu * sizeof(short4)));
         HIPCHK(ctx, d_n.ensure((size_t)n * 3 * 4));
         hipStream_t s = ctx->stream;
@@ -613,7 +622,7 @@
             int32_t* cand_n = ctx->cand_n.as<int32_t>() + (size_t)i * 3;
             if (launch_minu_cands(grp.dev, one, ctx->scratch.as<float>(), per_wg, n_wg, ctx->minu_generic | (ctx->s3_tie_order << 1), cands, cand_n, ctx->minu_fb.as<int32_t>(), grp.max_nL, ctx->max_nR, nullptr, s) != hipSuccess ||
                 launch_graph_minutiae(grp.dev, one, cands, cand_n, ctx->parts.as<float>() + (size_t)i * 4,
-                                      d_xy.as<short4>() + (size_t)i * 3 * kTopMinu, d_n.as<int32_t>() + (size_t)i * 3, nullptr, nullptr, 2 | (ctx->s89_tie_order << 8), s) != hipSuccess)
+                                      d_xy.as<short4>() + (size_t)i * 3 * kTopMinu, d_n.as<int32_t>() + (size_t)i * 3, ctx->minu_slab.p, ctx->minu_slab.bytes, nullptr, nullptr, 2 | (ctx->s89_tie_order << 8), s) != hipSuccess)
                 err = fail(ctx, AFIS_EDEVICE, "afis_correspondences: kernel launch failed");
         }
         if (err == AFIS_OK) {
@@ -652,7 +661,7 @@
     HIPCHK(ctx, hipSetDevice(ctx->device));
     { const int rcd = drain_abandoned(ctx); if (rcd != AFIS_OK) return rcd; }
     const int n_pq = std::max((n_minu + 2) / 3, n_tex);
-    const int64_t by_mem = std::max<int64_t>(1, group_budget_bytes(ctx) / group_bytes_per_query(ctx, G));
+    const int64_t by_mem = std::max<int64_t>(1, std::max<int64_t>(0, group_budget_bytes(ctx) - graph_slab_bytes(INT64_C(1) << 40)) / group_bytes_per_query(ctx, G));
     const int per = (int)std::max<int64_t>(1, std::min<int64_t>(ctx->query_batch > 0 ? ctx->query_batch : 10, by_mem));
     std::vector<float> parts;
     for (int j0 = 0; j0 < n_pq; j0 += per) {
diff --git a/msu-latentafis_amd/csrc/afis_taps.cpp b/msu-latentafis_amd/csrc/afis_taps.cpp
--- a/msu-latentafis_amd/csrc/afis_taps.cpp
+++ b/msu-latentafis_amd/csrc/afis_taps.cpp
@@ -174,7 +174,8 @@
             { int rcf = ensure_codes_cf(ctx, av); if (rcf != AFIS_OK) return rcf; }
             if (av == 6 || av == 7) { one.tex_codes_cf = ctx->gal.tex_codes_cf; one.tex_cf_blk = ctx->gal.tex_cf_blk + gidx; }
             { int rcd = direct_rowmax(ctx, d, one, av, 32, nullptr); if (rcd != AFIS_OK) return rcd; }
-            HIPCHK(ctx, launch_graph_texture(d, one, ctx->table.as<float>(), ctx->rm_val.as<float>(), ctx->rm_arg.as<int32_t>(), nullptr, nullptr, ctx->parts.as<float>(),
+            HIPCHK(ctx, ctx->tex_slab.ensure(graph_texture_slab_bytes(d.nq)));
+            HIPCHK(ctx, launch_graph_texture(d, one, ctx->table.as<float>(), ctx->rm_val.as<float>(), ctx->rm_arg.as<int32_t>(), nullptr, nullptr, ctx->parts.as<float>(), ctx->tex_slab.p, ctx->tex_slab.bytes,
                                              d_out.as<MinuCand>(), d_n.as<int32_t>(), stage | (ctx->s89_tie_order << 8), s));
         } else {
             slot = which - 1; cap = kTopMinu;
@@ -182,7 +183,8 @@
             HIPCHK(ctx, ctx->scratch.ensure(per_wg * 4 * 64));
             HIPCHK(ctx, ctx->cands.ensure(3 * (size_t)kTopMinu * sizeof(MinuCand))); HIPCHK(ctx, ctx->cand_n.ensure(12)); HIPCHK(ctx, ctx->minu_fb.ensure(minu_fb_ints(3, 1) * 4));
             HIPCHK(ctx, launch_minu_cands(d, one, ctx->scratch.as<float>(), per_wg, 64, ctx->minu_generic | (ctx->s3_tie_order << 1), ctx->cands.as<MinuCand>(), ctx->cand_n.as<int32_t>(), ctx->minu_fb.as<int32_t>(), grp.max_nL, ctx->max_nR, nullptr, s));
-            HIPCHK(ctx, launch_graph_minutiae(d, one, ctx->cands.as<MinuCand>(), ctx->cand_n.as<int32_t>(), ctx->parts.as<float>(), nullptr, nullptr,
+            HIPCHK(ctx, ctx->minu_slab.ensure(graph_minutiae_slab_bytes(3ll * d.nq)));
+            HIPCHK(ctx, launch_graph_minutiae(d, one, ctx->cands.as<MinuCand>(), ctx->cand_n.as<int32_t>(), ctx->parts.as<float>(), nullptr, nullptr, ctx->minu_slab.p, ctx->minu_slab.bytes,
                                               d_out.as<MinuCand>(), d_n.as<int32_t>(), stage | (ctx->s89_tie_order << 8), s));
         }
         std::vector<MinuCand> h((size_t)3 * kTopTex); int32_t hn[3] = {-1, -1, -1};
diff --git a/msu-latentafis_amd/csrc/graph.hip b/msu-latentafis_amd/csrc/graph.hip
--- a/msu-latentafis_amd/csrc/graph.hip
+++ b/msu-latentafis_amd/csrc/graph.hip
@@ -59,6 +59,10 @@
     return __builtin_amdgcn_readlane(x, 63);
 }
 
+typedef __amdgpu_buffer_rsrc_t SlabBuf;
+typedef uint32_t v4u __attribute__((ext_vector_type(4)));
+__device__ __forceinline__ SlabBuf g_slab_buf(unsigned char* base, uint32_t bytes) { return __builtin_amdgcn_make_buffer_rsrc(base, 0, (int)bytes, 0x00020000); }
+
 struct Pt { int lx, ly, rx, ry; };
 __device__ __forceinline__ int2 pack_xy(int lx, int ly, int rx, int ry) { return make_int2((lx & 0xffff) | (ly << 16), (rx & 0xffff) | (ry << 16)); }
 __device__ __forceinline__ Pt unpack_xy(int2 v) { Pt p; p.lx = (int)(short)v.x; p.ly = v.x >> 16; p.rx = (int)(short)v.y; p.ry = v.y >> 16; return p; }
@@ -69,9 +73,9 @@
 #ifndef AFIS_MINU_ALIAS
 #define AFIS_MINU_ALIAS 1
 #endif
-template <int NMAX_, int CACHE_, bool OWN_SIM_>
+template <int NMAX_, bool OWN_SIM_>
 struct __attribute__((aligned(16))) WaveSmem : SimStore<NMAX_, OWN_SIM_> {
-    static constexpr int NMAX = NMAX_, CACHE = CACHE_;
+    static constexpr int NMAX = NMAX_;
     static constexpr bool OWN_SIM = OWN_SIM_;
     static constexpr bool ALIAS_ORI = NMAX_ > 128 || AFIS_MINU_ALIAS;
     static constexpr int W = (NMAX + 31) / 32;
@@ -86,7 +90,7 @@
     int2 xy[NMAX];
     uint32_t hb[NMAX][W];
     union {
-        float stash[CACHE * NMAX];
+        uint32_t sortbuf[N4 + 128];
         struct { u64 keys[N4]; float lo[ALIAS_ORI ? 1 : NMAX], ro[ALIAS_ORI ? 1 : NMAX]; } s;
         struct { uint32_t keys[N4]; short te[NMAX], targ[NMAX]; } pick;
     } x;
@@ -389,7 +393,7 @@
 }
 
 template <class SM, bool LOOKUP, int ITERS, int MODE, int REF_TIE>
-__device__ int dist_filter(SM& sm, int num, const float* __restrict__ table, const float* __restrict__ ext)
+__device__ int dist_filter(SM& sm, int num, const float* __restrict__ table, const float* __restrict__ ext, SlabBuf slab)
 {
     constexpr bool fast = MODE > 0;
     constexpr bool range_test = MODE == 1;
@@ -542,19 +546,20 @@
 #pragma unroll
     for (int u = 0; u < U; ++u) mine[u] = myrow[u] >= 0 ? sm.xy[myrow[u]] : make_int2(0, 0);
     constexpr bool kFlat = NMAX > 128;
-#ifndef AFIS_MINU_VALN
-#define AFIS_MINU_VALN 0
-#endif
-    constexpr int kValN = kFlat ? 0 : AFIS_MINU_VALN, kIdxN = 4 * SM::CACHE - 4 * kValN;
-    static_assert(kValN * NMAX * 4 + kIdxN * NMAX <= (int)sizeof(sm.x.stash), "index lists + value stash exceed the stash space");
-    float* const vst = sm.x.stash;
-    unsigned char* const idx8 = reinterpret_cast<unsigned char*>(sm.x.stash + kValN * NMAX);
-#ifndef AFIS_MINU_REGN
-#define AFIS_MINU_REGN 0
-#endif
-    constexpr int kRegN = kFlat ? 0 : AFIS_MINU_REGN;
-    static_assert(kRegN <= kIdxN, "cached values need their neighbour indices");
-    float hreg[U][kRegN > 0 ? kRegN : 1];
+    constexpr int kSlabN = kFlat ? kTexSlabSteps : kMinuSlabSteps;
+    static_assert(kSlabN % 4 == 0, "the read loop takes blocks of four steps");
+    static_assert((size_t)U * kSlabN * 64 * 5 == (kFlat ? kTexSlabWgBytes : kMinuSlabWgBytes), "slab layout and the size the host allocates differ");
+    constexpr int kSlabBlk = kSlabN / 4;
+    constexpr uint32_t kSlabIdx0 = (uint32_t)U * kSlabN * 64 * 4;
+    const uint32_t lane16 = (uint32_t)lane * 16u, lane4 = (uint32_t)lane * 4u;
+    auto put_block = [&](int e, const float (&h)[4], uint32_t k4) {
+        __builtin_amdgcn_raw_buffer_store_b128(v4u{__float_as_uint(h[0]), __float_as_uint(h[1]), __float_as_uint(h[2]), __float_as_uint(h[3])}, slab, lane16, e * 1024, 0);
+        __builtin_amdgcn_raw_buffer_store_b32(k4, slab, lane4, (int)kSlabIdx0 + e * 256, 0);
+    };
+    auto get_block = [&](int e, v4u& h, uint32_t& k4) {
+        h = __builtin_amdgcn_raw_buffer_load_b128(slab, lane16, e * 1024, 0);
+        k4 = __builtin_amdgcn_raw_buffer_load_b32(slab, lane4, (int)kSlabIdx0 + e * 256, 0);
+    };
     int cur_w[U]; uint32_t cur_bits[U];
 #pragma unroll
     for (int u = 0; u < U; ++u) { cur_w[u] = 0; cur_bits[u] = 0u; }
@@ -579,58 +584,44 @@
                 if (t >= 0) {
                     int w = 0;
                     uint32_t bits = hrow[0];
-#pragma unroll
-                    for (int r = 0; r < kRegN; ++r) {
-                        if (r < trip[u]) {
-                            while (bits == 0u && w + 1 < Wn) { ++w; bits = hrow[w]; }
-                            const bool have = bits != 0u;
-                            const int k = (w * 32 + __ffs(bits) - 1) & 255;
-                            bits &= bits - 1;
-                            const float h = value(mine[u], k);
-                            idx8[r * NMAX + t] = (unsigned char)k;
-                            hreg[u][r] = h;
-                            const float p = h * sm.b[k];
-                            acc += have ? p : 0.0f;
+                    for (int n0 = 0; n0 < trip[u]; n0 += 4) {
+                        if (n0 == kSlabN) { cur_w[u] = w; cur_bits[u] = bits; }
+                        float h4[4] = {0.0f, 0.0f, 0.0f, 0.0f};
+                        uint32_t k4 = 0u;
+#pragma unroll
+                        for (int j = 0; j < 4; ++j) {
+                            if (n0 + j < trip[u]) {
+                                while (bits == 0u && w + 1 < Wn) { ++w; bits = hrow[w]; }
+                                const bool have = bits != 0u;
+                                const int k = (w * 32 + __ffs(bits) - 1) & 255;
+                                bits &= bits - 1;
+                                const float h = value(mine[u], k);
+                                h4[j] = h; k4 |= (uint32_t)k << (8 * j);
+                                const float p = h * sm.b[k];
+                                acc += have ? p : 0.0f;
+                            }
                         }
-                    }
-                    for (int n = kRegN; n < trip[u]; ++n) {
-                        if (n == kIdxN) { cur_w[u] = w; cur_bits[u] = bits; }
-                        while (bits == 0u && w + 1 < Wn) { ++w; bits = hrow[w]; }
-                        const bool have = bits != 0u;
-                        const int k = (w * 32 + __ffs(bits) - 1) & 255;
-                        bits &= bits - 1;
-                        const float h = value(mine[u], k);
-                        if (n < kIdxN) idx8[n * NMAX + t] = (unsigned char)k;
-                        if (n < kValN) vst[n * NMAX + t] = h;
-                        const float p = h * sm.b[k];
-                        acc += have ? p : 0.0f;
+                        if (n0 < kSlabN) put_block(u * kSlabBlk + (n0 >> 2), h4, k4);
                     }
                 }
             } else {
-                const int nV = min(trip[u], kValN), nA = min(trip[u], kIdxN);
-                const int tt = t >= 0 ? t : 0;
-                for (int n = 0; n < nV; ++n) {
-                    const int k = idx8[n * NMAX + tt];
-                    const float p = vst[n * NMAX + tt] * sm.b[k];
-                    acc += n < rlen[u] ? p : 0.0f;
-                }
-#pragma unroll
-                for (int r = 0; r < kRegN; ++r) {
-                    if (r < nA) {
-                        const int k = idx8[r * NMAX + tt];
-                        const float p = hreg[u][r] * sm.b[k];
-                        acc += r < rlen[u] ? p : 0.0f;
+                const int nS = min(trip[u], kSlabN);
+                v4u hc = {0u, 0u, 0u, 0u}; uint32_t kc = 0u;
+                if (nS > 0) get_block(u * kSlabBlk, hc, kc);
+                for (int n0 = 0; n0 < nS; n0 += 4) {
+                    const float hn[4] = {__uint_as_float(hc.x), __uint_as_float(hc.y), __uint_as_float(hc.z), __uint_as_float(hc.w)};
+                    const uint32_t kn = kc;
+                    if (n0 + 4 < nS) get_block(u * kSlabBlk + (n0 >> 2) + 1, hc, kc);
+#pragma unroll
+                    for (int j = 0; j < 4; ++j) {
+                        const float p = hn[j] * sm.b[(kn >> (8 * j)) & 255u];
+                        acc += n0 + j < rlen[u] ? p : 0.0f;
                     }
                 }
-                for (int n = max(nV, kRegN); n < nA; ++n) {
-                    const int k = idx8[n * NMAX + tt];
-                    const float p = value(mine[u], k) * sm.b[k];
-                    acc += n < rlen[u] ? p : 0.0f;
-                }
-                if (trip[u] > kIdxN) {
+                if (trip[u] > kSlabN) {
                     int w = cur_w[u];
                     uint32_t bits = cur_bits[u];
-                    for (int n = kIdxN; n < trip[u]; ++n) {
+                    for (int n = kSlabN; n < trip[u]; ++n) {
                         while (bits == 0u && w + 1 < Wn) { ++w; bits = t >= 0 ? hrow[w] : 0u; }
                         const bool have = bits != 0u;
                         const int k = (w * 32 + __ffs(bits) - 1) & 255;
@@ -779,13 +770,13 @@
 
 template <class SM, bool LOOKUP, int ITERS, int REF_TIE>
 __device__ __forceinline__ float graph_score(SM& sm, int num, const float* __restrict__ table, const float* __restrict__ lori,
-                                             const float* __restrict__ rori, const float* __restrict__ ext, int& n_survivors, int stop_after = 2, int mode = 0)
+                                             const float* __restrict__ rori, const float* __restrict__ ext, SlabBuf slab, int& n_survivors, int stop_after = 2, int mode = 0)
 {
     n_survivors = num;
     if (stop_after == 0) return 0.0f;
-    if (mode == 2 && LOOKUP) num = dist_filter<SM, LOOKUP, ITERS, 2, REF_TIE>(sm, num, table, ext);
-    else if (mode >= 1) num = dist_filter<SM, LOOKUP, ITERS, 1, REF_TIE>(sm, num, table, ext);
-    else num = dist_filter<SM, LOOKUP, ITERS, 0, REF_TIE>(sm, num, table, ext);
+    if (mode == 2 && LOOKUP) num = dist_filter<SM, LOOKUP, ITERS, 2, REF_TIE>(sm, num, table, ext, slab);
+    else if (mode >= 1) num = dist_filter<SM, LOOKUP, ITERS, 1, REF_TIE>(sm, num, table, ext, slab);
+    else num = dist_filter<SM, LOOKUP, ITERS, 0, REF_TIE>(sm, num, table, ext, slab);
     n_survivors = num;
     if (mode >= 1) {
         for (int t = threadIdx.x; t < num; t += 64) {
@@ -816,22 +807,20 @@
     if (threadIdx.x == 0) tap.n[task] = n;
 }
 
-#ifndef AFIS_TEX_CACHE
-#define AFIS_TEX_CACHE 2
-#endif
 #ifndef AFIS_TEX_WAVES
 #define AFIS_TEX_WAVES 4
 #endif
-typedef WaveSmem<kTopTex, AFIS_TEX_CACHE, false> TexSmem;
+typedef WaveSmem<kTopTex, false> TexSmem;
 constexpr int kTexRegs = (kTexMax + 63) / 64;
 
 template <int REF_TIE>
 __global__ __launch_bounds__(64) __attribute__((amdgpu_waves_per_eu(AFIS_TEX_WAVES, AFIS_TEX_WAVES))) void k_graph_texture(QueryDev q, GalleryDev g, const float* __restrict__ table_dist,
                                                       const float* __restrict__ rm_val, const int32_t* __restrict__ rm_arg,
                                                       const float* __restrict__ rm_cv, const int32_t* __restrict__ rm_n,
-                                                      float* __restrict__ parts, GraphTap tap)
+                                                      float* __restrict__ parts, unsigned char* slab_all, GraphTap tap)
 {
     __shared__ TexSmem sm;
+    const SlabBuf slab = g_slab_buf(slab_all + (size_t)blockIdx.x * kTexSlabWgBytes, (uint32_t)kTexSlabWgBytes);
     const int lane = threadIdx.x;
     GPH_ZERO();
     const int n_tasks = q.nq * g.G;
@@ -977,7 +966,7 @@
         GPH_K(15);
         int n_surv;
         const float* const row_max = (rm_n ? rm_cv : rm_val) + o;
-        const float score = graph_score<TexSmem, true, 3, REF_TIE>(sm, num, table_dist, q.lt_ori + l0, g.tex_ori + r0, row_max, n_surv, tap.out ? tap.stage : 2, mode);
+        const float score = graph_score<TexSmem, true, 3, REF_TIE>(sm, num, table_dist, q.lt_ori + l0, g.tex_ori + r0, row_max, slab, n_surv, tap.out ? tap.stage : 2, mode);
         if (lane == 0) *out = score;
         if (tap.out) tap_write(tap, sm, row_max, task, n_surv, kTopTex);
         WSYNC();
@@ -986,24 +975,22 @@
 }
 
 hipError_t launch_graph_texture(const QueryDev& q, const GalleryDev& g, const float* table_dist,
-                                const float* rm_val, const int32_t* rm_arg, const float* rm_cv, const int32_t* rm_n, float* parts, MinuCand* tap_out, int32_t* tap_n, int tap_stage, hipStream_t stream)
+                                const float* rm_val, const int32_t* rm_arg, const float* rm_cv, const int32_t* rm_n, float* parts, void* slab, size_t slab_bytes, MinuCand* tap_out, int32_t* tap_n, int tap_stage, hipStream_t stream)
 {
     const long long n_tasks = (long long)q.nq * g.G;
     if (n_tasks <= 0) return hipSuccess;
     if (n_tasks > 0x7ffffff0LL || !g.task_ctr) return hipErrorInvalidValue;
-    const int grid = (int)(n_tasks < 16384 ? n_tasks : 16384);
+    const int grid = graph_texture_grid(n_tasks);
+    if (!slab || slab_bytes < (size_t)grid * kTexSlabWgBytes) return hipErrorInvalidValue;
     hipError_t e0 = hipMemsetAsync(g.task_ctr + 0, 0, 4, stream);
     if (e0 != hipSuccess) return e0;
     const GraphTap tap{tap_out, tap_n, tap_stage & 255};
-    if ((tap_stage >> 8) & 1) hipLaunchKernelGGL(k_graph_texture<1>, dim3(grid), dim3(64), 0, stream, q, g, table_dist, rm_val, rm_arg, rm_cv, rm_n, parts, tap);
-    else hipLaunchKernelGGL(k_graph_texture<0>, dim3(grid), dim3(64), 0, stream, q, g, table_dist, rm_val, rm_arg, rm_cv, rm_n, parts, tap);
+    if ((tap_stage >> 8) & 1) hipLaunchKernelGGL(k_graph_texture<1>, dim3(grid), dim3(64), 0, stream, q, g, table_dist, rm_val, rm_arg, rm_cv, rm_n, parts, (unsigned char*)slab, tap);
+    else hipLaunchKernelGGL(k_graph_texture<0>, dim3(grid), dim3(64), 0, stream, q, g, table_dist, rm_val, rm_arg, rm_cv, rm_n, parts, (unsigned char*)slab, tap);
     return hipGetLastError();
 }
 
-#ifndef AFIS_MINU_CACHE
-#define AFIS_MINU_CACHE 3
-#endif
-typedef WaveSmem<kTopMinu, AFIS_MINU_CACHE, true> MinuGraphSmem;
+typedef WaveSmem<kTopMinu, true> MinuGraphSmem;
 
 #ifndef AFIS_MINU_WAVES
 #define AFIS_MINU_WAVES 6
@@ -1011,9 +998,10 @@
 template <int REF_TIE>
 __global__ __launch_bounds__(64) __attribute__((amdgpu_waves_per_eu(AFIS_MINU_WAVES, AFIS_MINU_WAVES))) void k_graph_minutiae(QueryDev q, GalleryDev g, const MinuCand* __restrict__ cands,
                                                        const int32_t* __restrict__ cand_n, float* __restrict__ parts,
-                                                       short4* __restrict__ corr_out, int32_t* __restrict__ corr_n, GraphTap tap)
+                                                       short4* __restrict__ corr_out, int32_t* __restrict__ corr_n, unsigned char* slab_all, GraphTap tap)
 {
     __shared__ MinuGraphSmem sm;
+    const SlabBuf slab = g_slab_buf(slab_all + (size_t)blockIdx.x * kMinuSlabWgBytes, (uint32_t)kMinuSlabWgBytes);
     const int lane = threadIdx.x;
     GPH_ZERO();
     const int n_tasks = q.nq * 3 * g.G;
@@ -1051,7 +1039,7 @@
         WSYNC();
         GPH_K(7);
         int n_surv;
-        const float score = graph_score<MinuGraphSmem, false, 5, REF_TIE>(sm, num, nullptr, q.lm_ori + l0, g.minu_ori + r0, nullptr, n_surv, tap.out ? tap.stage : 2, mode);
+        const float score = graph_score<MinuGraphSmem, false, 5, REF_TIE>(sm, num, nullptr, q.lm_ori + l0, g.minu_ori + r0, nullptr, slab, n_surv, tap.out ? tap.stage : 2, mode);
         if (lane == 0) *out = score;
         if (tap.out) tap_write(tap, sm, nullptr, task, n_surv, kTopMinu);
         if (corr_out) {
@@ -1067,17 +1055,18 @@
 }
 
 hipError_t launch_graph_minutiae(const QueryDev& q, const GalleryDev& g, const MinuCand* cands, const int32_t* cand_n,
-                                 float* parts, short4* corr_out, int32_t* corr_n, MinuCand* tap_out, int32_t* tap_n, int tap_stage, hipStream_t stream, bool join)
+                                 float* parts, short4* corr_out, int32_t* corr_n, void* slab, size_t slab_bytes, MinuCand* tap_out, int32_t* tap_n, int tap_stage, hipStream_t stream, bool join)
 {
     const long long n_tasks = (long long)q.nq * 3 * g.G;
     if (n_tasks <= 0) return hipSuccess;
     if (n_tasks > 0x7ffffff0LL || !g.task_ctr) return hipErrorInvalidValue;
-    const int grid = (int)(n_tasks < 32768 ? n_tasks : 32768);
+    const int grid = graph_minutiae_grid(n_tasks);
+    if (!slab || slab_bytes < (size_t)grid * kMinuSlabWgBytes) return hipErrorInvalidValue;
     hipError_t e0 = join ? hipSuccess : hipMemsetAsync(g.task_ctr + 1, 0, 4, stream);
     if (e0 != hipSuccess) return e0;
     const GraphTap tap{tap_out, tap_n, tap_stage & 255};
-    if ((tap_stage >> 8) & 1) hipLaunchKernelGGL(k_graph_minutiae<1>, dim3(grid), dim3(64), 0, stream, q, g, cands, cand_n, parts, corr_out, corr_n, tap);
-    else hipLaunchKernelGGL(k_graph_minutiae<0>, dim3(grid), dim3(64), 0, stream, q, g, cands, cand_n, parts, corr_out, corr_n, tap);
+    if ((tap_stage >> 8) & 1) hipLaunchKernelGGL(k_graph_minutiae<1>, dim3(grid), dim3(64), 0, stream, q, g, cands, cand_n, parts, corr_out, corr_n, (unsigned char*)slab, tap);
+    else hipLaunchKernelGGL(k_graph_minutiae<0>, dim3(grid), dim3(64), 0, stream, q, g, cands, cand_n, parts, corr_out, corr_n, (unsigned char*)slab, tap);
     return hipGetLastError();
 }
 
```

Result: faster. 52.37 (median of 6 runs) (+6.8%).
